# hku-mars/BALM

Hardware: AMD Instinct MI355X
Metric: BA iterations/sec (W poses x F plane features) (higher is better)
Workload: dtype f64

## Files before the change

balm_amd/capi.py:

```python
import ctypes as C
import os

import numpy as np

_HERE = os.path.dirname(os.path.abspath(__file__))
LIB_PATH = os.environ.get("BALM_HIP_LIB") or os.path.join(_HERE, "lib", "libbalm_hip.so")

FORM_LEFT, FORM_RIGHT = 0, 1
OK, ERR_ARG, ERR_HIP, ERR_STATE, ERR_TOO_FEW_PLANES, ERR_NUMERIC = range(6)
ABI_VERSION = 6
FLAG_TIMING = 1
FLAG_LOOPBACK_SHARDS = 2
FLAG_SYRK_INT8 = 4
T_MOMENTS, T_FACTORS, T_SYRK, T_ASSEMBLE, T_SOLVE, T_UPDATE, T_BUILD, T_VOXEL, T_COV, T_COMM, T_UPLOAD, T_COUNT = range(12)
TIMING_NAMES = ["moments", "factors", "syrk", "assemble", "solve", "update", "build", "voxel", "cov", "comm", "upload"]

EXPORTS = ["balm_create", "balm_prewarm", "balm_create_multi", "balm_destroy", "balm_set_features", "balm_set_features_cb", "balm_evaluate", "balm_only_residual",
           "balm_solve_damped", "balm_damping_iter", "balm_build_clusters", "balm_build_clusters_planes", "balm_voxel_defaults", "balm_associate", "balm_associate_scans", "balm_get_features", "balm_get_association", "balm_pose_covariance",
           "balm_window_open", "balm_window_add_scan", "balm_window_add_scan_strided", "balm_window_recut", "balm_window_get_points", "balm_window_features", "balm_window_marginalize", "balm_window_info", "balm_window_close",
           "balm_set_allreduce", "balm_comm_unique_id", "balm_comm_init_rank", "balm_comm_info",
           "balm_get_timing", "balm_get_shard_timing", "balm_get_solve_trace", "balm_chain_macro_plan", "balm_reset_timing", "balm_work_model", "balm_last_error", "balm_version", "balm_abi_version"]


class IterLog(C.Structure):
    _fields_ = [("r1", C.c_double), ("r2", C.c_double), ("u", C.c_double), ("v", C.c_double),
                ("q", C.c_double), ("q1", C.c_double), ("accepted", C.c_int), ("hess_evaluated", C.c_int)]


class LMOpts(C.Structure):
    _fields_ = [("form", C.c_int), ("u0", C.c_double), ("max_iter", C.c_int), ("rel_tol", C.c_double),
                ("min_planes_per_pose", C.c_int), ("force_hess", C.c_int), ("no_stop", C.c_int),
                ("verbose", C.c_int), ("reanchor", C.c_int), ("abs_tol", C.c_double)]


class VoxelOpts(C.Structure):
    _fields_ = [("voxel_size", C.c_double), ("eigen_thr", C.c_float * 3), ("min_ps", C.c_int), ("layer_limit", C.c_int),
                ("min_observers", C.c_int), ("fix_frames", C.c_int), ("max_plane_dist", C.c_double),
                ("max_lambda21", C.c_double), ("max_lambda0", C.c_double), ("want_point_features", C.c_int),
                ("fix_point_limit", C.c_int), ("defer_recut", C.c_int)]


ALLREDUCE_FN = C.CFUNCTYPE(C.c_int, C.c_void_p, C.c_long, C.c_void_p)
FILL_CLUSTERS_FN = C.CFUNCTYPE(None, C.c_void_p, C.c_int, C.c_int, C.POINTER(C.c_double))

_LIB = None


class BalmError(RuntimeError):
    def __init__(self, code, msg):
        super().__init__("balm_hip error %d: %s" % (code, msg))
        self.code = code


def lib():
    global _LIB
    if _LIB is None:
        if not os.path.exists(LIB_PATH):
            raise ImportError("libbalm_hip.so is not built (%s missing): run `python -m balm_amd.build`. "
                              "There is no CPU fallback for the HIP path." % LIB_PATH)
        L = C.CDLL(LIB_PATH)
        abi = getattr(L, "balm_abi_version", None)
        abi = abi() if abi is not None else 0
        if abi != ABI_VERSION:
            raise ImportError("libbalm_hip.so has ABI revision %d, this binding was written for %d: rebuild (python -m balm_amd.build)"
                              % (abi, ABI_VERSION))
        L.balm_create.restype = C.c_void_p
        L.balm_create.argtypes = [C.c_int, C.c_int, C.c_int]
        L.balm_create_multi.restype = C.c_void_p
        L.balm_create_multi.argtypes = [C.c_int, C.c_int, C.c_int, C.c_int]
        L.balm_prewarm.argtypes = [C.c_int]
        L.balm_destroy.restype = None
        L.balm_destroy.argtypes = [C.c_void_p]
        L.balm_set_features.argtypes = [C.c_void_p, C.c_int, C.c_void_p, C.c_void_p, C.c_void_p]
        L.balm_set_features_cb.argtypes = [C.c_void_p, C.c_int, FILL_CLUSTERS_FN, C.c_void_p, C.c_void_p, C.c_void_p]
        L.balm_evaluate.argtypes = [C.c_void_p, C.c_int, C.c_void_p, C.c_int, C.c_int, C.c_void_p, C.c_void_p,
                                    C.POINTER(C.c_double)]
        L.balm_only_residual.argtypes = [C.c_void_p, C.c_void_p, C.POINTER(C.c_double)]
        L.balm_solve_damped.argtypes = [C.c_void_p, C.c_void_p, C.c_void_p, C.c_double, C.c_void_p,
                                        C.POINTER(C.c_double)]
        L.balm_damping_iter.argtypes = [C.c_void_p, C.POINTER(LMOpts), C.c_void_p, C.POINTER(IterLog),
                                        C.POINTER(C.c_int)]
        L.balm_build_clusters.argtypes = [C.c_void_p, C.c_int, C.c_void_p, C.c_void_p, C.c_void_p, C.c_long,
                                          C.c_void_p, C.c_void_p, C.c_void_p]
        L.balm_build_clusters_planes.argtypes = [C.c_void_p, C.c_int, C.c_void_p, C.c_void_p, C.c_size_t, C.c_size_t, C.c_void_p,
                                                 C.c_void_p, C.c_void_p]
        L.balm_associate_scans.argtypes = [C.c_void_p, C.POINTER(VoxelOpts), C.c_int, C.c_void_p, C.c_void_p, C.c_size_t,
                                           C.c_void_p, C.POINTER(C.c_int), C.POINTER(C.c_long)]
        L.balm_window_add_scan_strided.argtypes = [C.c_void_p, C.c_void_p, C.c_long, C.c_size_t, C.c_void_p]
        L.balm_window_open.argtypes = [C.c_void_p, C.POINTER(VoxelOpts)]
        L.balm_window_add_scan.argtypes = [C.c_void_p, C.c_void_p, C.c_long, C.c_void_p]
        L.balm_window_recut.argtypes = [C.c_void_p]
        L.balm_window_get_points.argtypes = [C.c_void_p, C.c_void_p, C.c_void_p, C.c_void_p, C.c_long, C.c_void_p]
        L.balm_window_features.argtypes = [C.c_void_p, C.POINTER(C.c_int)]
        L.balm_window_marginalize.argtypes = [C.c_void_p, C.c_int, C.c_void_p]
        L.balm_window_info.argtypes = [C.c_void_p, C.POINTER(C.c_int), C.POINTER(C.c_long), C.POINTER(C.c_long)]
        L.balm_window_close.argtypes = [C.c_void_p]
        L.balm_associate.argtypes = [C.c_void_p, C.POINTER(VoxelOpts), C.c_void_p, C.c_void_p, C.c_long, C.c_void_p,
                                     C.POINTER(C.c_int), C.POINTER(C.c_long)]
        L.balm_get_features.argtypes = [C.c_void_p, C.c_void_p, C.c_void_p, C.c_void_p]
        L.balm_get_association.argtypes = [C.c_void_p, C.c_void_p, C.c_void_p]
        L.balm_voxel_defaults.restype = None
        L.balm_voxel_defaults.argtypes = [C.POINTER(VoxelOpts)]
        L.balm_pose_covariance.argtypes = [C.c_void_p, C.c_void_p, C.c_void_p, C.c_double, C.c_void_p, C.c_void_p]
        L.balm_set_allreduce.argtypes = [C.c_void_p, ALLREDUCE_FN, C.c_void_p]
        L.balm_comm_unique_id.argtypes = [C.c_void_p]
        L.balm_comm_init_rank.argtypes = [C.c_void_p, C.c_int, C.c_int, C.c_void_p]
        L.balm_comm_info.argtypes = [C.c_void_p, C.c_void_p]
        L.balm_get_timing.argtypes = [C.c_void_p, C.c_void_p, C.c_void_p]
        L.balm_get_shard_timing.argtypes = [C.c_void_p, C.c_int, C.c_void_p, C.c_void_p]
        L.balm_get_solve_trace.argtypes = [C.c_void_p, C.c_void_p, C.c_long, C.c_void_p]
        L.balm_chain_macro_plan.argtypes = [C.c_int, C.c_int, C.c_void_p, C.c_long]
        L.balm_reset_timing.argtypes = [C.c_void_p]
        L.balm_work_model.argtypes = [C.c_void_p, C.c_void_p]
        L.balm_last_error.restype = C.c_char_p
        L.balm_last_error.argtypes = [C.c_void_p]
        L.balm_version.restype = C.c_char_p
        _LIB = L
    return _LIB


def chain_macro_plan(panels, helpers):
    tab = np.empty(helpers * 64, np.int32)
    rc = lib().balm_chain_macro_plan(int(panels), int(helpers), tab.ctypes.data_as(C.c_void_p), tab.size)
    if rc != OK:
        raise BalmError(rc, "balm_chain_macro_plan(%d, %d)" % (panels, helpers))
    tab = tab.reshape(helpers, 64)
    return [[(int(e) & 0xffff, int(e) >> 16) for e in row if e >= 0] for row in tab]


def _p(a):
    return None if a is None else a.ctypes.data_as(C.c_void_p)


def _c(a, dtype=np.float64):
    return None if a is None else np.ascontiguousarray(a, dtype=dtype)


class Context:

    def __init__(self, win_size, device=0, flags=0, n_devices=None):
        self.L = lib()
        self.W = int(win_size)
        self.n = 6 * self.W
        if n_devices is None:
            self.h = self.L.balm_create(self.W, int(device), int(flags))
        else:
            self.h = self.L.balm_create_multi(self.W, int(device), int(n_devices), int(flags))
        if not self.h:
            raise BalmError(ERR_HIP, "balm_create(win_size=%d, device=%d, n_devices=%s) failed (no GPU, bad device, or "
                                     "win_size out of range)" % (win_size, device, n_devices))
        self.F = 0
        self._cb = None

    def close(self):
        if getattr(self, "h", None):
            self.L.balm_destroy(self.h)
            self.h = None

    def __del__(self):
        try:
            self.close()
        except Exception:
            pass

    def _check(self, rc):
        if rc != OK:
            raise BalmError(rc, self.L.balm_last_error(self.h).decode())

    def set_features(self, clusters, fix, coeffs):
        clusters, fix, coeffs = _c(clusters), _c(fix), _c(coeffs)
        F = clusters.shape[0]
        assert clusters.shape == (F, self.W, 10), clusters.shape
        assert coeffs.shape == (F,)
        assert fix is None or fix.shape == (F, 10)
        self._check(self.L.balm_set_features(self.h, F, _p(clusters), _p(fix), _p(coeffs)))
        self.F = F

    def set_features_cb(self, per_feature, fix, coeffs):
        tabs = [_c(t) for t in per_feature]
        F = len(tabs)
        assert all(t.shape == (self.W, 10) for t in tabs)
        fix, coeffs = _c(fix), _c(coeffs)
        row = self.W * 10

        failed = []

        def fill(_user, f0, f1, dst):
            out = np.ctypeslib.as_array(dst, shape=((f1 - f0) * row,))
            try:
                for a in range(f0, f1):
                    out[(a - f0) * row:(a - f0 + 1) * row] = tabs[a].reshape(-1)
            except BaseException as exc:
                out[:] = 0.0
                failed.append(exc)

        cb = FILL_CLUSTERS_FN(fill)
        rc = self.L.balm_set_features_cb(self.h, F, cb, None, _p(fix), _p(coeffs))
        if failed:
            self.F = 0
            raise failed[0]
        self._check(rc)
        self.F = F

    def build_clusters(self, F, xyz, feat_id, pose_id, fix, coeffs, want_clusters=True):
        xyz = _c(xyz, np.float32).reshape(-1, 3)
        feat_id, pose_id = _c(feat_id, np.int32), _c(pose_id, np.int32)
        fix, coeffs = _c(fix), _c(coeffs)
        out = np.zeros((F, self.W, 10)) if want_clusters else None
        self._check(self.L.balm_build_clusters(self.h, F, _p(xyz), _p(feat_id), _p(pose_id), xyz.shape[0],
                                               _p(fix), _p(coeffs), _p(out)))
        self.F = F
        return out

    @staticmethod
    def _containers(arrays):
        keep = [np.ascontiguousarray(a, dtype=np.float32) for a in arrays]
        keep = [a.reshape(-1, 3) if a.ndim == 1 else a for a in keep]
        cols = {a.shape[1] for a in keep}
        assert len(cols) == 1 and min(cols) >= 3, "every container: [n, c] float32 with the same c >= 3"
        ptrs = (C.c_void_p * len(keep))(*[a.ctypes.data if a.shape[0] else None for a in keep])
        cnt = (C.c_long * len(keep))(*[a.shape[0] for a in keep])
        return ptrs, cnt, 4 * cols.pop(), keep

    def build_clusters_planes(self, planes, pose_col, fix, coeffs, want_clusters=True):
        ptrs, cnt, stride, keep = self._containers(planes)
        F = len(keep)
        fix, coeffs = _c(fix), _c(coeffs)
        out = np.zeros((F, self.W, 10)) if want_clusters else None
        self._check(self.L.balm_build_clusters_planes(self.h, F, ptrs, cnt, stride, 4 * int(pose_col), _p(fix), _p(coeffs), _p(out)))
        self.F = F
        return out

    def associate_scans(self, scans, poses, voxel_size=2.0, eigen_thresholds=(1.0 / 16, 1.0 / 16, 1.0 / 9), min_ps=15,
                        want_features=True, layer_limit=2, min_observers=2, fix_frames=0, strict=None, want_points=False):
        ptrs, cnt, stride, keep = self._containers(scans)
        poses = _c(poses)
        assert poses.shape[0] == self.W + fix_frames == len(keep), "one scan and one pose per window slot"
        o = self._voxel_opts(voxel_size, eigen_thresholds, min_ps, layer_limit, min_observers, fix_frames, strict, want_points)
        F, nr = C.c_int(0), C.c_long(0)
        self._check(self.L.balm_associate_scans(self.h, C.byref(o), len(keep), ptrs, cnt, stride, _p(poses), C.byref(F), C.byref(nr)))
        self.F = F.value
        return self.F, nr.value, self._association_result(want_features, fix_frames, want_points, sum(a.shape[0] for a in keep))

    def _voxel_opts(self, voxel_size, eigen_thresholds, min_ps, layer_limit, min_observers, fix_frames, strict, want_points):
        o = VoxelOpts()
        self.L.balm_voxel_defaults(C.byref(o))
        o.voxel_size = voxel_size
        o.eigen_thr = (C.c_float * 3)(*[float(t) for t in eigen_thresholds])
        o.min_ps, o.layer_limit, o.min_observers, o.fix_frames = min_ps, layer_limit, min_observers, fix_frames
        if strict is not None:
            o.max_plane_dist, o.max_lambda21, o.max_lambda0 = strict
        o.want_point_features = int(want_points)
        return o

    def _association_result(self, want_features, fix_frames, want_points, n_pts):
        feats = None
        if want_features and self.F > 0:
            cl, co = np.zeros((self.F, self.W, 10)), np.zeros(self.F)
            layer = np.zeros(self.F, dtype=np.int32)
            self._check(self.L.balm_get_features(self.h, _p(cl), _p(co), _p(layer)))
            feats = (cl, co, layer)
            if fix_frames or want_points:
                fix = np.zeros((self.F, 10))
                pf = np.zeros(n_pts, dtype=np.int32) if want_points else None
                self._check(self.L.balm_get_association(self.h, _p(fix), _p(pf)))
                feats = (cl, co, layer, fix, pf)
        return feats

    def associate(self, xyz, frame_id, poses, voxel_size=2.0, eigen_thresholds=(1.0 / 16, 1.0 / 16, 1.0 / 9),
                  min_ps=15, want_features=True, layer_limit=2, min_observers=2, fix_frames=0, strict=None,
                  want_points=False):
        xyz = _c(xyz, np.float32).reshape(-1, 3)
        frame_id, poses = _c(frame_id, np.int32), _c(poses)
        assert poses.shape[0] == self.W + fix_frames, "poses for the marginalised scans too"
        o = self._voxel_opts(voxel_size, eigen_thresholds, min_ps, layer_limit, min_observers, fix_frames, strict, want_points)
        F, nr = C.c_int(0), C.c_long(0)
        self._check(self.L.balm_associate(self.h, C.byref(o), _p(xyz), _p(frame_id), xyz.shape[0], _p(poses),
                                          C.byref(F), C.byref(nr)))
        self.F = F.value
        return self.F, nr.value, self._association_result(want_features, fix_frames, want_points, xyz.shape[0])

    def window_open(self, voxel_size=2.0, eigen_thresholds=(1.0 / 16, 1.0 / 16, 1.0 / 9), min_ps=15, layer_limit=2,
                    min_observers=2, fix_frames=0, strict=None, fix_point_limit=50, defer_recut=False):
        o = VoxelOpts()
        self.L.balm_voxel_defaults(C.byref(o))
        o.voxel_size = voxel_size
        o.eigen_thr = (C.c_float * 3)(*[float(t) for t in eigen_thresholds])
        o.min_ps, o.layer_limit, o.min_observers = min_ps, layer_limit, min_observers
        o.fix_frames, o.fix_point_limit, o.defer_recut = int(fix_frames), int(fix_point_limit), int(bool(defer_recut))
        if strict is not None:
            o.max_plane_dist, o.max_lambda21, o.max_lambda0 = [float(v) for v in strict]
        self._check(self.L.balm_window_open(self.h, C.byref(o)))

    def window_points(self):
        n = self.window_info()[1]
        xyz, slot, feat = np.zeros((n, 3), np.float32), np.zeros(n, np.int32), np.zeros(n, np.int32)
# ... 154 lines not shown
```

balm_amd/csrc/balm_capi.hip:

```cpp
#include <algorithm>
#include <array>
#include <atomic>
#include <chrono>
#include <cmath>
#include <cstdio>
#include <cstdlib>
#include <cstring>

#include "balm_internal.h"

using namespace balm;

#define HIP_TRY(expr)                                                                              \
  do {                                                                                             \
    hipError_t e_ = (expr);                                                                        \
    if (e_ != hipSuccess) {                                                                        \
      ctx->err = std::string(#expr) + ": " + hipGetErrorString(e_);                                \
      return BALM_ERR_HIP;                                                                         \
    }                                                                                              \
  } while (0)

namespace {

#ifdef BALM_COLD_TRACE
static void cold_mark(const char *what) {
  static const auto t0 = std::chrono::steady_clock::now();
  static double last = 0;
  const double now = std::chrono::duration<double, std::milli>(std::chrono::steady_clock::now() - t0).count();
  fprintf(stderr, "[cold] %9.3f ms (+%8.3f)  %s\n", now, now - last, what);
  last = now;
}
#else
#define cold_mark(what) ((void)0)
#endif

struct DeviceWarm {
  std::mutex mu;
  std::thread th;
  bool started = false;
  PinnedRing ring;
  std::atomic<bool> ring_ready{false};
  ~DeviceWarm() { if (th.joinable()) th.join(); }
};
static DeviceWarm g_warm[64];

static void warm_body(int device) {
  DeviceWarm &w = g_warm[device];
  if (hipSetDevice(device) != hipSuccess) { hipGetLastError(); return; }
  std::thread ring_th([&w, device] {
    if (hipSetDevice(device) == hipSuccess && w.ring.init(device) == hipSuccess) w.ring_ready.store(true, std::memory_order_release);
    else hipGetLastError();
  });
  (void)preload_voxel(); (void)preload_build(); (void)prepare_device_accum(); (void)preload_solve(); (void)prepare_device_cov();
  hipGetLastError();
  ring_th.join();
}

static int warm_start(int device) {
  if (device < 0 || device >= 64) return BALM_ERR_ARG;
  DeviceWarm &w = g_warm[device];
  std::lock_guard<std::mutex> lk(w.mu);
  if (!w.started) { w.started = true; w.th = std::thread(warm_body, device); }
  return BALM_OK;
}

static void adopt_warm_ring(balm_ctx *ctx) {
  if (ctx->ring.buf[0] || ctx->device < 0 || ctx->device >= 64) return;
  DeviceWarm &w = g_warm[ctx->device];
  std::lock_guard<std::mutex> lk(w.mu);
  if (!w.started) return;
  if (w.th.joinable()) w.th.join();
  if (w.ring_ready.load(std::memory_order_acquire)) {
    const int key = ctx->ring.pool_key;
    ctx->ring = w.ring; ctx->ring.pool_key = key;
    w.ring = PinnedRing(); w.ring_ready.store(false);
  }
}

struct Span {
  balm_ctx *c; int slot; hipEvent_t a = nullptr, b = nullptr;
  Span(balm_ctx *ctx, int s) : c(ctx), slot(s) {
    if (!c->timer.on) return;
    a = take(); b = take();
    hipEventRecord(a, c->stream);
  }
  ~Span() {
    if (!c->timer.on) return;
    hipEventRecord(b, c->stream);
    c->timer.pending.push_back({a, b, slot});
  }
  hipEvent_t take() {
    if (!c->timer.pool.empty()) { hipEvent_t e = c->timer.pool.back(); c->timer.pool.pop_back(); return e; }
    hipEvent_t e; hipEventCreate(&e); return e;
  }
};

void collect_timing(balm_ctx *c) {
  for (auto &sp : c->timer.pending) {
    float ms = 0;
    if (hipEventElapsedTime(&ms, sp.a, sp.b) == hipSuccess) { c->timer.ms[sp.slot] += ms; c->timer.cnt[sp.slot]++; }
    c->timer.pool.push_back(sp.a); c->timer.pool.push_back(sp.b);
  }
  c->timer.pending.clear();
}

template <class T>
int dalloc(balm_ctx *ctx, T **p, size_t count) {
  if (*p) { hipFree(*p); *p = nullptr; }
  if (count == 0) count = 1;
  HIP_TRY(hipMalloc((void **)p, count * sizeof(T)));
  return BALM_OK;
}

template <class T>
int keep(balm_ctx *ctx, T **p, size_t *cap, size_t count) {
  if (*p && *cap >= count) return BALM_OK;
  for (int k = 0; k < balm_ctx::LM_GRAPHS; k++)
    if (ctx->lm_graph[k]) { hipGraphExecDestroy(ctx->lm_graph[k]); ctx->lm_graph[k] = nullptr; ctx->lm_graph_form[k] = -1; }
  int rc = dalloc(ctx, p, count + count / 4);
  *cap = rc ? 0 : count + count / 4;
  return rc;
}

template <class T>
int ensure(balm_ctx *ctx, T **p, size_t *cap, size_t count) {
  if (*p && *cap >= count) return BALM_OK;
  for (int k = 0; k < balm_ctx::LM_GRAPHS; k++)
    if (ctx->lm_graph[k]) { hipGraphExecDestroy(ctx->lm_graph[k]); ctx->lm_graph[k] = nullptr; ctx->lm_graph_form[k] = -1; }
  int rc = dalloc(ctx, p, count);
  if (rc) return rc;
  *cap = count;
  return BALM_OK;
}

int stage_begin(balm_ctx *ctx, size_t total_bytes) {
  total_bytes += 16 * 256;
  ctx->stage_off = 0;
  if (ctx->stage_cap >= total_bytes) return BALM_OK;
  if (ctx->d_stage) { hipStreamSynchronize(ctx->stream); hipFree(ctx->d_stage); ctx->d_stage = nullptr; ctx->stage_cap = 0; }
  const size_t want = total_bytes + total_bytes / 8;
  HIP_TRY(hipMalloc((void **)&ctx->d_stage, want));
  ctx->stage_cap = want;
  return BALM_OK;
}

template <class T>
T *stage_take(balm_ctx *ctx, size_t count) {
  const size_t off = (ctx->stage_off + 255) & ~(size_t)255;
  ctx->stage_off = off + count * sizeof(T);
  return reinterpret_cast<T *>(ctx->d_stage + off);
}

int sync_stream(balm_ctx *ctx) {
  HIP_TRY(hipStreamSynchronize(ctx->stream));
  HIP_TRY(hipGetLastError());
  collect_timing(ctx);
  return BALM_OK;
}

long red_dacc_off(const balm_ctx *c) { return (long)c->ntiles * TILE_ELEMS; }
long red_r_off(const balm_ctx *c) { return red_dacc_off(c) + (long)DACC_MAX * c->W; }

bool has_transport(const balm_ctx *ctx) { return ctx->comm || multi_is_loopback(ctx) || ctx->allreduce; }

int hook_allreduce(balm_ctx *ctx, double *buf, long n) {
  if (ctx->comm) { Span sp(ctx, BALM_T_COMM); return comm_allreduce(ctx, buf, n); }
  if (multi_is_loopback(ctx)) { Span sp(ctx, BALM_T_COMM); return loopback_allreduce(ctx, buf, n); }
  if (!ctx->allreduce) return BALM_OK;
  int rc = sync_stream(ctx);
  if (rc) return rc;
  if (ctx->allreduce((void *)buf, n, ctx->allreduce_user) != 0) {
    ctx->err = "all-reduce hook failed";
    return BALM_ERR_STATE;
  }
  return BALM_OK;
}

int set_damping(balm_ctx *ctx, double u) {
  ctx->u_value = u;
  ctx->u_on_device = false;
  return BALM_OK;
}
int push_damping(balm_ctx *ctx) {
  double *slot = ctx->h_scal + 16 + (ctx->u_ring++ & 63);
  *slot = ctx->u_value;
  HIP_TRY(hipMemcpyAsync(ctx->d_scal + SCAL_U, slot, sizeof(double), hipMemcpyHostToDevice, ctx->stream));
  ctx->u_on_device = true;
  return BALM_OK;
}

static void collect_timing_if_idle(balm_ctx *ctx) {
  if (!ctx->timer.on || ctx->timer.pending.empty()) return;
  if (hipStreamSynchronize(ctx->stream) == hipSuccess) collect_timing(ctx);
}

int wait_scalars(balm_ctx *ctx) {
  volatile double *stamp = ctx->h_scal + SCAL_STAMP;
  const double want = (double)ctx->mail_seq;
  const auto t0 = std::chrono::steady_clock::now();
  for (int spin = 0;; spin++) {
    if (*stamp == want) { std::atomic_thread_fence(std::memory_order_acquire); collect_timing_if_idle(ctx); return BALM_OK; }
    if ((spin & 255) == 255 && std::chrono::steady_clock::now() - t0 > std::chrono::microseconds(300)) break;
  }
  int rc = sync_stream(ctx);
  if (rc) return rc;
  if (*stamp != want) { ctx->err = "balm_damping_iter: the iteration's scalars did not arrive"; return BALM_ERR_HIP; }
  return BALM_OK;
}

void drop_lm_graphs(balm_ctx *ctx) {
  for (int k = 0; k < balm_ctx::LM_GRAPHS; k++) {
    if (ctx->lm_graph[k]) hipGraphExecDestroy(ctx->lm_graph[k]);
    ctx->lm_graph[k] = nullptr; ctx->lm_graph_form[k] = -1;
  }
}

int residual_device(balm_ctx *ctx, const double *d_poses, int f0, int f1, int slot, bool defer_sum = false, bool send_mail = false) {
  if (f1 <= f0) {
    HIP_TRY(hipMemsetAsync(ctx->d_scal + slot, 0, sizeof(double), ctx->stream));
    ctx->nr_tmp = 0;
  } else {
    Span sp(ctx, BALM_T_MOMENTS);
    launch_world_moments(ctx->stream, ctx->d_cl, d_poses, ctx->W, f0, f1, ctx->d_C);
    const EigenMail mail{ctx->d_scal, ctx->d_hscal, send_mail ? (double)++ctx->mail_seq : 0.0, slot};
    ctx->nr_tmp = launch_feature_eigen(ctx->stream, ctx->d_C, ctx->has_fix ? ctx->d_fix : nullptr, ctx->d_coe, f0, f1, ctx->d_feat_tmp,
                                       ctx->d_rpart_tmp, send_mail ? &mail : nullptr);
    if (!defer_sum) launch_sum_scalar(ctx->stream, ctx->d_rpart_tmp, ctx->nr_tmp, ctx->d_scal + slot);
  }
  HIP_TRY(hipGetLastError());
  if (defer_sum) return BALM_OK;
  return hook_allreduce(ctx, ctx->d_scal + slot, 1);
}

bool fuse_trial(const balm_ctx *ctx) {
  const char *e = getenv("BALM_FUSE_TRIAL");
  return ctx->W <= 256 && ctx->F > 0 && e && e[0] == '1';
}

static bool syrk_int8_mode(const balm_ctx *ctx) {
  if (ctx->flags & BALM_FLAG_SYRK_INT8) return true;
  const char *m = getenv("BALM_SYRK");
  return m && !strcmp(m, "int8");
}
static bool syrk_int8_for(const balm_ctx *ctx, long K) {
  if (!syrk_int8_mode(ctx)) return false;
  if (const char *m = getenv("BALM_SYRK_INT8_MIN_COLS")) return K >= atol(m);
  return K >= 12288L && ctx->W >= 96;
}

int prepare_evaluate(balm_ctx *ctx, int form, int nf) {
  if (nf <= 0) return BALM_OK;
  const SyrkPlan plan = plan_syrk(ctx->ntiles, 3L * nf);
  int rc;
  size_t gcols = (size_t)plan.Kpad + 64, parts = (size_t)plan.SG * ctx->ntiles;
  if (ctx->sparse && nf == ctx->F) {
    gcols = (size_t)ctx->sp_nchunks * ctx->sp_nsteps * 4 + 64;
    parts = (size_t)ctx->sp_nitems;
  }
  {
    const double *before = ctx->d_Gt;
    if ((rc = ensure(ctx, &ctx->d_Gt, &ctx->cap_Gt, gcols * ctx->npad))) return rc;
    if (ctx->d_Gt != before) ctx->gt_dirty_cols = ~(size_t)0;
  }
  if ((rc = ensure(ctx, &ctx->d_part, &ctx->cap_part, parts * TILE_ELEMS))) return rc;
  if (syrk_int8_for(ctx, 3L * nf) && !(ctx->sparse && nf == ctx->F)) {
    if ((rc = ensure(ctx, &ctx->d_i8, &ctx->cap_i8, syrk_i8_scratch_bytes(ctx->n, 3L * nf, nullptr)))) return rc;
    if (!ctx->d_rowmax) ctx->rowmax_cur_valid = false;
    if (!ctx->d_rowmax2) ctx->rowmax_trial_valid = false;
    if ((rc = ensure(ctx, &ctx->d_rowmax, &ctx->cap_rowmax, (size_t)ctx->npad + 128))) return rc;
    if ((rc = ensure(ctx, &ctx->d_rowmax2, &ctx->cap_rowmax2, (size_t)ctx->npad + 128))) return rc;
    if ((rc = ensure(ctx, &ctx->d_rowmax_part, &ctx->cap_rowmax_part, (size_t)factors_grid(ctx->W, nf, form) * 6 * ctx->W))) return rc;
    HIP_TRY(prepare_device_syrk_i8());
  }
  if ((rc = ensure(ctx, &ctx->d_dpart, &ctx->cap_dpart, (size_t)factors_grid(ctx->W, nf, form) * DACC_MAX * ctx->W))) return rc;
  if (nf == ctx->F && fuse_trial(ctx)) {
    if (ctx->cap_Gt2 < gcols * ctx->npad || ctx->cap_dpart2 < (size_t)factors_grid(ctx->W, nf, form) * DACC_MAX * ctx->W) ctx->gt_trial_valid = false;
    if ((rc = ensure(ctx, &ctx->d_Gt2, &ctx->cap_Gt2, gcols * ctx->npad))) return rc;
    if ((rc = ensure(ctx, &ctx->d_dpart2, &ctx->cap_dpart2, (size_t)factors_grid(ctx->W, nf, form) * DACC_MAX * ctx->W))) return rc;
  }
  return BALM_OK;
}

int evaluate_device(balm_ctx *ctx, int form, const double *d_poses, int f0, int f1, int slot) {
  const int W = ctx->W, nf = f1 - f0;
  const int dacc = form == 0 ? DACC_LEFT : DACC_RIGHT;
  int rc;
  if (nf <= 0) {
    HIP_TRY(hipMemsetAsync(ctx->d_red, 0, ctx->red_len * sizeof(double), ctx->stream));
    if ((rc = hook_allreduce(ctx, ctx->d_red, (long)ctx->red_len))) return rc;
    Span sp(ctx, BALM_T_ASSEMBLE);
    launch_assemble(ctx->stream, form, ctx->d_red, red_dacc_off(ctx), ctx->d_sub, ctx->ntiles, W, ctx->d_H, ctx->d_g,
                    ctx->d_red + red_r_off(ctx), ctx->d_scal + slot);
    return BALM_OK;
  }
  SyrkPlan plan = plan_syrk(ctx->ntiles, 3L * nf);
  if ((rc = prepare_evaluate(ctx, form, nf))) return rc;
  const int nblk = factors_grid(W, nf, form);
  hipStream_t s = ctx->stream;
  if (!(ctx->feat_cur_valid && f0 == 0 && f1 == ctx->F)) {
    Span sp(ctx, BALM_T_MOMENTS);
    launch_world_moments(s, ctx->d_cl, d_poses, W, f0, f1, ctx->d_C);
    ctx->nr_cur = launch_feature_eigen(s, ctx->d_C, ctx->has_fix ? ctx->d_fix : nullptr, ctx->d_coe, f0, f1, ctx->d_feat, ctx->d_rpart);
    ctx->feat_cur_valid = (f0 == 0 && f1 == ctx->F);
  }
  const int nr = ctx->nr_cur;
  const bool sparse = ctx->sparse && f0 == 0 && f1 == ctx->F;
  const size_t kpad = sparse ? (size_t)ctx->sp_nchunks * ctx->sp_nsteps * 4 : (size_t)plan.Kpad;
  if (!(ctx->gt_cur_valid && ctx->feat_cur_valid && f0 == 0 && f1 == ctx->F)) {
    Span sp(ctx, BALM_T_FACTORS);
    const size_t k0 = (size_t)3 * nf, k1 = kpad + 64;
    if (ctx->gt_dirty_cols == ~(size_t)0) {
      HIP_TRY(hipMemsetAsync(ctx->d_Gt, 0, ctx->cap_Gt * sizeof(double), s));
      ctx->gt_dirty_cols = 0;
    } else if (ctx->gt_dirty_cols > k0) {
      HIP_TRY(hipMemsetAsync(ctx->d_Gt + k0 * ctx->npad, 0, (std::max(ctx->gt_dirty_cols, k1) - k0) * ctx->npad * sizeof(double), s));
    }
    ctx->gt_dirty_cols = k0;
    ctx->rowmax_cur_valid = launch_factors(s, form, ctx->d_cl, d_poses, ctx->d_feat, W, ctx->npad, f0, f1, ctx->d_Gt, ctx->d_dpart, nblk,
                                           sparse ? ctx->d_slot : nullptr, (!sparse && syrk_int8_for(ctx, 3L * nf)) ? ctx->d_rowmax : nullptr, ctx->d_rowmax_part);
    ctx->gt_cur_valid = false;
  }
  HIP_TRY(hipGetLastError());
  const bool int8 = !sparse && syrk_int8_for(ctx, 3L * nf);
  {
    Span sp(ctx, BALM_T_SYRK);
    if (sparse) launch_syrk_sparse(s, ctx->d_Gt, ctx->npad, ctx->d_jobs, ctx->d_items, ctx->d_chunk_ids, ctx->sp_nsteps, ctx->sp_nitems, ctx->d_part);
    else if (int8) {
      if (launch_syrk_i8(s, ctx->d_Gt, ctx->npad, ctx->n, 3L * nf, ctx->d_sub, ctx->ntiles, ctx->d_i8, ctx->d_part,
                         ctx->rowmax_cur_valid ? ctx->d_rowmax : nullptr)) { ctx->err = "INT8 SYRK: unsupported size"; return BALM_ERR_ARG; }
      plan.SG = 1;
    }
    else launch_syrk(s, ctx->d_Gt, ctx->npad, ctx->ntiles, ctx->d_jobs, plan, ctx->d_part);
  }
  {
    Span sp(ctx, BALM_T_ASSEMBLE);
    launch_reduce(s, ctx->d_part, plan.SG, (long)ctx->ntiles * TILE_ELEMS, ctx->d_dpart, nblk, dacc * W,
                  ctx->d_rpart, nr, ctx->d_red, red_dacc_off(ctx), red_r_off(ctx), sparse ? ctx->d_csr : nullptr);
  }
  if ((rc = hook_allreduce(ctx, ctx->d_red, (long)ctx->red_len))) return rc;
  {
    Span sp(ctx, BALM_T_ASSEMBLE);
    launch_assemble(s, form, ctx->d_red, red_dacc_off(ctx), ctx->d_sub, ctx->ntiles, W, ctx->d_H, ctx->d_g, ctx->d_red + red_r_off(ctx),
                    ctx->d_scal + slot);
  }
  return BALM_OK;
}

int trial_device(balm_ctx *ctx, int form, const double *d_poses, int slot) {
  const int W = ctx->W, F = ctx->F;
  hipStream_t s = ctx->stream;
  const SyrkPlan plan = plan_syrk(ctx->ntiles, 3L * F);
  const bool sparse = ctx->sparse;
  const size_t kpad = sparse ? (size_t)ctx->sp_nchunks * ctx->sp_nsteps * 4 : (size_t)plan.Kpad;
  const int nblk = factors_grid(W, F, form);
  {
    Span sp(ctx, BALM_T_FACTORS);
    const size_t k0 = (size_t)3 * F, k1 = kpad + 64;
    HIP_TRY(hipMemsetAsync(ctx->d_Gt2 + k0 * ctx->npad, 0, (k1 - k0) * ctx->npad * sizeof(double), s));
    if (ctx->npad > ctx->n)
      HIP_TRY(hipMemset2DAsync(ctx->d_Gt2 + ctx->n, (size_t)ctx->npad * sizeof(double), 0,
                               (size_t)(ctx->npad - ctx->n) * sizeof(double), k0, s));
    ctx->nr_tmp = launch_moments_factors(s, form, ctx->d_cl, d_poses, ctx->has_fix ? ctx->d_fix : nullptr, ctx->d_coe, W, ctx->npad, F,
                                         ctx->d_Gt2, ctx->d_dpart2, nblk, sparse ? ctx->d_slot : nullptr, ctx->d_feat_tmp, ctx->d_rpart_tmp,
                                         (!sparse && syrk_int8_for(ctx, 3L * F) && ctx->d_rowmax2) ? ctx->d_rowmax2 : nullptr, ctx->d_rowmax_part);
    ctx->rowmax_trial_valid = !sparse && syrk_int8_for(ctx, 3L * F) && ctx->d_rowmax2;
  }
  HIP_TRY(hipGetLastError());
  {
    Span sp(ctx, BALM_T_MOMENTS);
    launch_sum_scalar(s, ctx->d_rpart_tmp, ctx->nr_tmp, ctx->d_scal + slot);
  }
  ctx->gt_trial_valid = true;
  return hook_allreduce(ctx, ctx->d_scal + slot, 1);
}

int read_scalars(balm_ctx *ctx) {
  HIP_TRY(hipMemcpyAsync(ctx->h_scal, ctx->d_scal, 16 * sizeof(double), hipMemcpyDeviceToHost, ctx->stream));
  return sync_stream(ctx);
}

std::vector<unsigned char> obs_of(const double *clusters, int F, int W) {
  std::vector<unsigned char> obs((size_t)F * W);
  parallel_ranges(obs.size(), (size_t)1 << 16, [&](size_t lo, size_t hi) {
    for (size_t t = lo; t < hi; t++) obs[t] = clusters[t * 10 + 9] != 0 ? 1 : 0;
  });
  return obs;
}

int feature_bookkeeping(balm_ctx *ctx, int F, const unsigned char *obs, const double *fix, const double *coeffs) {
  const int W = ctx->W;
  ctx->planes_per_pose.assign(W, 0);
  double S = 0, B = 0;
  int bad_a = F, bad_rc = BALM_OK;
  std::mutex mu;
  parallel_ranges((size_t)F, (size_t)(65536 / W + 1), [&](size_t lo, size_t hi) {
    std::vector<int> ppp((size_t)W, 0);
    double s = 0, b = 0;
    int my_bad = F, my_rc = BALM_OK;
    for (size_t a = lo; a < hi; a++) {
      int na = 0;
      const unsigned char *oa = obs + a * W;
      for (int i = 0; i < W; i++)
        if (oa[i]) { ppp[(size_t)i]++; na++; }
      if (my_rc == BALM_OK) {
        if (na == 0 && !(fix && fix[a * 10 + 9] != 0)) { my_bad = (int)a; my_rc = BALM_ERR_NUMERIC; }
        else if (!(coeffs[a] >= 0) || !std::isfinite(coeffs[a])) { my_bad = (int)a; my_rc = BALM_ERR_ARG; }
      }
      s += na; b += 0.5 * na * (na + 1.0);
    }
    std::lock_guard<std::mutex> lk(mu);
    for (int i = 0; i < W; i++) ctx->planes_per_pose[(size_t)i] += ppp[(size_t)i];
    S += s; B += b;
    if (my_rc != BALM_OK && my_bad < bad_a) { bad_a = my_bad; bad_rc = my_rc; }
  });
  if (bad_rc == BALM_ERR_NUMERIC) {
    ctx->err = "feature " + std::to_string(bad_a) + " has no observation and no fix cluster (zero point count)";
    return BALM_ERR_NUMERIC;
  }
  if (bad_rc == BALM_ERR_ARG) {
    ctx->err = "feature " + std::to_string(bad_a) + " has a negative or non-finite weight";
    return BALM_ERR_ARG;
  }
  ctx->work_S = S; ctx->work_B = B;
  return BALM_OK;
}

}

extern "C" {

const char *balm_version(void) { return "balm_hip 0.6.0 (gfx950)"; }
int balm_abi_version(void) { return BALM_ABI_VERSION; }

const char *balm_last_error(balm_ctx *ctx) { return ctx ? ctx->err.c_str() : "null context"; }

static void one_destroy(balm_ctx *ctx);

balm_ctx *balm_create(int win_size, int device, int flags) {
  if (win_size < 1 || win_size > MAX_W) return nullptr;
  cold_mark("balm_create: enter");
  int ndev = 0;
  if (hipGetDeviceCount(&ndev) != hipSuccess || ndev < 1 || device < 0 || device >= ndev) return nullptr;
  if (hipSetDevice(device) != hipSuccess) return nullptr;
  cold_mark("balm_create: hipGetDeviceCount + hipSetDevice");
  warm_start(device);
  if (prepare_device_accum() != hipSuccess || prepare_device_cov() != hipSuccess) return nullptr;
  cold_mark("balm_create: prepare_device (function attributes -> code objects)");
  balm_ctx *ctx = new balm_ctx();
  ctx->W = win_size;
  ctx->n = 6 * win_size;
  ctx->npad = (ctx->n + TILE - 1) / TILE * TILE;
  ctx->T = ctx->npad / TILE;
  ctx->nA = (ctx->n + NB - 1) / NB * NB;
  ctx->device = device;
  ctx->flags = flags;
  ctx->timer.on = (flags & BALM_FLAG_TIMING) != 0;
  auto fail = [&]() -> balm_ctx * { one_destroy(ctx); return nullptr; };
  std::vector<int> jobs, sub;
  {
    const int T = ctx->T, ngroups = T / 5;
    std::vector<std::array<int, 3>> mixed[4];
    std::vector<std::array<int, 2>> pairs;
    for (int r = 0; r < TM; r++) for (int c = r; c < TM; c++) pairs.push_back({r, c});
    for (int k = 0; k < 15; k++) mixed[1].push_back({0, pairs[k][0], pairs[k][1]});
    for (int k = 0; k < 10; k++) mixed[1].push_back({1, pairs[k][0], pairs[k][1]});
    for (int k = 10; k < 15; k++) mixed[2].push_back({1, pairs[k][0], pairs[k][1]});
    for (int k = 0; k < 15; k++) mixed[2].push_back({2, pairs[k][0], pairs[k][1]});
    for (int k = 0; k < 5; k++) mixed[2].push_back({3, pairs[k][0], pairs[k][1]});
    for (int k = 5; k < 15; k++) mixed[3].push_back({3, pairs[k][0], pairs[k][1]});
    for (int k = 0; k < 15; k++) mixed[3].push_back({4, pairs[k][0], pairs[k][1]});
    auto regular = [&](int I, int J) {
      jobs.insert(jobs.end(), {0, I, J, 0});
      for (int t = 0; t < 25; t++) sub.push_back(((TM * I + t / TM) << 16) | (TM * J + t % TM));
    };
    for (int m = 0; m < T; m++) {
      for (int i = 0; i < m; i++) regular(i, m);
      if (m >= TM * ngroups) regular(m, m);
      else if (m % TM == TM - 1) {
        const int b = m - (TM - 1);
        for (int v = 1; v <= 3; v++) {
          jobs.insert(jobs.end(), {v, b, b, 0});
          for (const auto &e : mixed[v]) sub.push_back(((TM * (b + e[0]) + e[1]) << 16) | (TM * (b + e[0]) + e[2]));
        }
      }
    }
  }
  ctx->ntiles = (int)(jobs.size() / 4);
  ctx->h_jobs = jobs;
  if (hipStreamCreateWithFlags(&ctx->stream, hipStreamNonBlocking) != hipSuccess) return fail();
  cold_mark("balm_create: job tables + stream");
  const int W = ctx->W, n = ctx->n, nA = ctx->nA;
  ctx->red_len = (size_t)ctx->ntiles * TILE_ELEMS + (size_t)DACC_MAX * W + 2;
  if (dalloc(ctx, &ctx->d_poses, (size_t)12 * W) || dalloc(ctx, &ctx->d_poses_tmp, (size_t)12 * W) ||
      dalloc(ctx, &ctx->d_red, ctx->red_len) || dalloc(ctx, &ctx->d_jobs, jobs.size()) || dalloc(ctx, &ctx->d_sub, sub.size()) ||
      dalloc(ctx, &ctx->d_H, (size_t)n * n) || dalloc(ctx, &ctx->d_g, (size_t)n) ||
      dalloc(ctx, &ctx->d_A, (size_t)(2 * nA + NB) * nA) || dalloc(ctx, &ctx->d_Wp, (size_t)2 * NB * (2 * nA + NB)) ||
      dalloc(ctx, &ctx->d_dvec, (size_t)nA) || dalloc(ctx, &ctx->d_z, (size_t)nA) || dalloc(ctx, &ctx->d_x, (size_t)16 * nA) ||
      dalloc(ctx, &ctx->d_perm, (size_t)nA) || dalloc(ctx, &ctx->d_flags, (size_t)2 * (2 * (nA / NB) + 1) * (nA / NB) + (nA / NB) + 8) || dalloc(ctx, &ctx->d_minv, (size_t)2 * (nA / NB) * NB * NB) || dalloc(ctx, &ctx->d_dx, (size_t)n) ||
      dalloc(ctx, &ctx->d_scal, (size_t)16) || dalloc(ctx, &ctx->d_pre, (size_t)W + 2))
    return fail();
  if (hipHostMalloc((void **)&ctx->h_scal, (16 + 64 + 8) * sizeof(double), hipHostMallocMapped | hipHostMallocCoherent) != hipSuccess) return fail();
  if (hipHostGetDevicePointer((void **)&ctx->d_hscal, ctx->h_scal, 0) != hipSuccess) return fail();
  ctx->h_scal[SCAL_STAMP] = 0.0;
  if (hipMemcpy(ctx->d_jobs, jobs.data(), jobs.size() * sizeof(int), hipMemcpyHostToDevice) != hipSuccess ||
      hipMemcpy(ctx->d_sub, sub.data(), sub.size() * sizeof(int), hipMemcpyHostToDevice) != hipSuccess)
    return fail();
  if (getenv("BALM_SOLVE_TRACE")) {
    const size_t cnt = (size_t)(2 * (nA / NB) + 1) * (nA / NB) * 6 + (size_t)(nA / NB) * 6;
    if (hipMalloc((void **)&ctx->d_trace, cnt * sizeof(long long)) != hipSuccess) return fail();
    hipMemset(ctx->d_trace, 0, cnt * sizeof(long long));
  }
  {
    std::vector<int> ident(nA);
    for (int i = 0; i < nA; i++) ident[i] = i;
    if (hipMemcpy(ctx->d_perm, ident.data(), (size_t)nA * sizeof(int), hipMemcpyHostToDevice) != hipSuccess) return fail();
  }
  if (hipMemset(ctx->d_scal, 0, 16 * sizeof(double)) != hipSuccess) return fail();
  if (hipMemset(ctx->d_red, 0, ctx->red_len * sizeof(double)) != hipSuccess) return fail();
  if (hipMemset(ctx->d_minv, 0, (size_t)2 * (nA / NB) * NB * NB * sizeof(double)) != hipSuccess) return fail();
  cold_mark("balm_create: device buffers + small copies");
  context_born(device); ctx->counted_live = true;
  return ctx;
}

static void one_destroy(balm_ctx *ctx) {
  if (!ctx) return;
  if (ctx->counted_live) { context_gone(ctx->device); ctx->counted_live = false; }
  comm_destroy(ctx);
  drop_lm_graphs(ctx);
  hipSetDevice(ctx->device);
  if (ctx->stream) hipStreamSynchronize(ctx->stream);
  if (ctx->window) { window_close(ctx->window); ctx->window = nullptr; }
  void *ptrs[] = {ctx->d_cl, ctx->d_fix, ctx->d_coe, ctx->d_poses, ctx->d_poses_tmp, ctx->d_C, ctx->d_feat,
                  ctx->d_Gt, ctx->d_Gt2, ctx->d_dpart2, ctx->d_part, ctx->d_dpart, ctx->d_rpart, ctx->d_feat_tmp, ctx->d_rpart_tmp, ctx->d_red, ctx->d_jobs, ctx->d_sub, ctx->d_H,
                  ctx->d_g, ctx->d_A, ctx->d_Wp, ctx->d_dvec, ctx->d_z, ctx->d_x, ctx->d_perm, ctx->d_dx, ctx->d_scal, ctx->d_arena, ctx->d_pre, ctx->d_flags, ctx->d_minv, ctx->d_macro_tab, ctx->d_trace, ctx->d_slot, ctx->d_items, ctx->d_csr, ctx->d_chunk_ids, ctx->d_stage, ctx->d_i8, ctx->d_rowmax, ctx->d_rowmax2, ctx->d_rowmax_part};
  for (void *p : ptrs) if (p) hipFree(p);
  if (ctx->h_scal) hipHostFree(ctx->h_scal);
  ctx->ring.release();
  if (ctx->amail.host) hipHostFree((void *)ctx->amail.host);
  if (ctx->amail.scan_state) hipFree(ctx->amail.scan_state);
  for (auto &sp : ctx->timer.pending) { hipEventDestroy(sp.a); hipEventDestroy(sp.b); }
  for (auto e : ctx->timer.pool) hipEventDestroy(e);
  if (ctx->stream) hipStreamDestroy(ctx->stream);
  delete ctx;
}

static int build_sparse_plan(balm_ctx *ctx, int F, const unsigned char *obs) {
  ctx->sparse = false;
  const char *mode = getenv("BALM_SYRK");
  if (mode && !strcmp(mode, "dense")) return BALM_OK;
  if (syrk_int8_for(ctx, 3L * F)) return BALM_OK;
  const int W = ctx->W, T = ctx->T, ntiles = ctx->ntiles;
  if (T > 128 || T <= 2 || F < 64) return BALM_OK;
  struct Key { uint64_t hi, lo; int a; };
  std::vector<Key> keys((size_t)F);
  parallel_ranges((size_t)F, (size_t)(65536 / W + 1), [&](size_t a0, size_t a1) {
    for (size_t a = a0; a < a1; a++) {
      uint64_t hi = 0, lo = 0;
      const unsigned char *oa = obs + a * W;
      for (int i = 0; i < W; i++)
        if (oa[i])
          for (int b = (6 * i) / TILE; b <= (6 * i + 5) / TILE; b++) {
            if (b < 64) hi |= 1ull << (63 - b); else lo |= 1ull << (127 - b);
          }
      keys[a] = {hi, lo, (int)a};
    }
  });
  auto first_of = [&](const Key &k) { for (int b = 0; b < T; b++) if (b < 64 ? (k.hi >> (63 - b)) & 1 : (k.lo >> (127 - b)) & 1) return b; return T; };
  auto last_of = [&](const Key &k) { for (int b = T - 1; b >= 0; b--) if (b < 64 ? (k.hi >> (63 - b)) & 1 : (k.lo >> (127 - b)) & 1) return b; return -1; };
  std::vector<int> fb((size_t)F), lb((size_t)F);
  for (int a = 0; a < F; a++) { fb[(size_t)a] = first_of(keys[(size_t)a]); lb[(size_t)a] = last_of(keys[(size_t)a]); }
  std::sort(keys.begin(), keys.end(), [&](const Key &x, const Key &y) {
    if (fb[(size_t)x.a] != fb[(size_t)y.a]) return fb[(size_t)x.a] < fb[(size_t)y.a];
    if (lb[(size_t)x.a] != lb[(size_t)y.a]) return lb[(size_t)x.a] < lb[(size_t)y.a];
    return x.hi != y.hi ? x.hi > y.hi : (x.lo != y.lo ? x.lo > y.lo : x.a < y.a);
  });
  const int C = 16, nsteps = 3 * C / 4, nchunks = (F + C - 1) / C;
  auto touched = [](const Key &k, int b) { return b < 64 ? (k.hi >> (63 - b)) & 1 : (k.lo >> (127 - b)) & 1; };
  std::vector<int> slot((size_t)F);
  std::vector<std::vector<int>> chunks_of((size_t)ntiles);
  long total = 0;
  for (int c = 0; c < nchunks; c++) {
    Key cm{0, 0, 0};
    for (int k = c * C; k < F && k < (c + 1) * C; k++) { cm.hi |= keys[(size_t)k].hi; cm.lo |= keys[(size_t)k].lo; slot[(size_t)keys[(size_t)k].a] = k; }
    for (int j = 0; j < ntiles; j++) {
      const int type = ctx->h_jobs[(size_t)4 * j], I = ctx->h_jobs[(size_t)4 * j + 1], J = ctx->h_jobs[(size_t)4 * j + 2];
      bool need;
      if (type == 0) need = touched(cm, I) && touched(cm, J);
      else if (type == 1) need = touched(cm, I) || touched(cm, I + 1);
      else if (type == 2) need = touched(cm, I + 1) || touched(cm, I + 2) || touched(cm, I + 3);
      else need = touched(cm, I + 3) || touched(cm, I + 4);
      if (need) { chunks_of[(size_t)j].push_back(c); total++; }
    }
  }
  const double dense_steps = (double)ntiles * ((3.0 * F + 3) / 4), sparse_steps = (double)total * nsteps;
  const bool forced = mode && !strcmp(mode, "sparse");
  if (total == 0 || (!forced && !(sparse_steps < 0.8 * dense_steps))) return BALM_OK;
  long per = total / 2048;
  if (per < 8) per = 8;
  std::vector<int> items, chunk_ids, csr((size_t)ntiles + 1, 0);
  struct Order { int first_chunk, item; };
  std::vector<Order> order;
  int run = 0;
  for (int j = 0; j < ntiles; j++) {
    csr[(size_t)j] = run;
    const std::vector<int> &L = chunks_of[(size_t)j];
    const long pieces = ((long)L.size() + per - 1) / per;
    for (long q = 0; q < pieces; q++) {
      const size_t b = (size_t)((long)L.size() * q / pieces), e = (size_t)((long)L.size() * (q + 1) / pieces);
      order.push_back({L[b], (int)(items.size() / 4)});
      items.insert(items.end(), {j, (int)chunk_ids.size(), (int)(e - b), run++});
      chunk_ids.insert(chunk_ids.end(), L.begin() + (long)b, L.begin() + (long)e);
    }
  }
  csr[(size_t)ntiles] = run;
  std::stable_sort(order.begin(), order.end(), [](const Order &x, const Order &y) { return x.first_chunk < y.first_chunk; });
  std::vector<int> sorted_items;
  sorted_items.reserve(items.size());
  for (const Order &o : order) sorted_items.insert(sorted_items.end(), items.begin() + 4L * o.item, items.begin() + 4L * o.item + 4);
  if (chunk_ids.empty()) chunk_ids.push_back(0);
  int rc;
  if ((rc = keep(ctx, &ctx->d_slot, &ctx->cap_slot, (size_t)F)) || (rc = keep(ctx, &ctx->d_items, &ctx->cap_items, sorted_items.size())) ||
      (rc = keep(ctx, &ctx->d_chunk_ids, &ctx->cap_chunk_ids, chunk_ids.size())) || (rc = keep(ctx, &ctx->d_csr, &ctx->cap_csr, csr.size())))
    return rc;
  HIP_TRY(hipMemcpy(ctx->d_slot, slot.data(), slot.size() * sizeof(int), hipMemcpyHostToDevice));
  HIP_TRY(hipMemcpy(ctx->d_items, sorted_items.data(), sorted_items.size() * sizeof(int), hipMemcpyHostToDevice));
  HIP_TRY(hipMemcpy(ctx->d_chunk_ids, chunk_ids.data(), chunk_ids.size() * sizeof(int), hipMemcpyHostToDevice));
  HIP_TRY(hipMemcpy(ctx->d_csr, csr.data(), csr.size() * sizeof(int), hipMemcpyHostToDevice));
  ctx->sparse = true; ctx->sp_nsteps = nsteps; ctx->sp_nchunks = nchunks; ctx->sp_nitems = run; ctx->sp_steps = sparse_steps;
  return BALM_OK;
}

static int install_feature_buffers(balm_ctx *ctx, int F, const double *fix, const double *coeffs,
                                   hipMemcpyKind kind = hipMemcpyHostToDevice) {
  int rc;
  drop_lm_graphs(ctx);
  ctx->has_fix = fix != nullptr;
  if (fix) {
    if ((rc = keep(ctx, &ctx->d_fix, &ctx->cap_fix, (size_t)F * 10))) return rc;
    HIP_TRY(hipMemcpyAsync(ctx->d_fix, fix, (size_t)F * 10 * sizeof(double), kind, ctx->stream));
  }
  if ((rc = keep(ctx, &ctx->d_coe, &ctx->cap_coe, (size_t)F))) return rc;
  HIP_TRY(hipMemcpyAsync(ctx->d_coe, coeffs, (size_t)F * sizeof(double), kind, ctx->stream));
  if ((rc = keep(ctx, &ctx->d_C, &ctx->cap_C, (size_t)F * 10))) return rc;
  if ((rc = keep(ctx, &ctx->d_feat, &ctx->cap_feat, (size_t)F * FEAT_STRIDE))) return rc;
  if ((rc = keep(ctx, &ctx->d_feat_tmp, &ctx->cap_feat_tmp, (size_t)F * FEAT_STRIDE))) return rc;
  if ((rc = keep(ctx, &ctx->d_rpart, &ctx->cap_rpart, (size_t)(F + 255) / 256 + 1024 + 1))) return rc;
  if ((rc = keep(ctx, &ctx->d_rpart_tmp, &ctx->cap_rpart_tmp, (size_t)(F + 255) / 256 + 1024 + 1))) return rc;
  ctx->feat_cur_valid = false; ctx->gt_cur_valid = false;
  ctx->F = F;
  return BALM_OK;
}

static int assoc_clusters_host(balm_ctx *ctx);

using FillClusters = std::function<void(int, int, double *, unsigned char *)>;

static int one_set_features_fn(balm_ctx *ctx, int F, const FillClusters &fill, const double *fix, const double *coeffs, bool shard_books = false) {
  if (!ctx) return BALM_ERR_ARG;
  if (ctx->multi && F == 0) { ctx->F = 0; ctx->feat_cur_valid = false; ctx->gt_cur_valid = false; ctx->planes_per_pose.clear(); ctx->work_S = ctx->work_B = 0; return BALM_OK; }
  if (F < 1 || !fill || !coeffs) { ctx->err = "balm_set_features: bad argument"; return BALM_ERR_ARG; }
  HIP_TRY(hipSetDevice(ctx->device));
  const int W = ctx->W;
  const size_t count = (size_t)F * W * 10;
  int rc;
  if ((rc = assoc_clusters_host(ctx))) return rc;
  ctx->F = 0;
  adopt_warm_ring(ctx);
  if ((rc = keep(ctx, &ctx->d_cl, &ctx->cap_cl, count))) return rc;
  if ((rc = stage_begin(ctx, count * sizeof(double)))) return rc;
  double *d_aos = stage_take<double>(ctx, count);
  std::vector<unsigned char> obs((size_t)F * W);
  const size_t unit = (size_t)W * 10 * sizeof(double);
  hipError_t e;
  {
    Span sp(ctx, BALM_T_UPLOAD);
    e = staged_upload(ctx->ring, ctx->device, ctx->stream, d_aos, count * sizeof(double), unit, [&](char *dst, size_t off, size_t len) {
      const int f0 = (int)(off / unit), f1 = f0 + (int)(len / unit);
      fill(f0, f1, reinterpret_cast<double *>(dst), obs.data() + (size_t)f0 * W);
    });
  }
  if (e == hipSuccess) launch_transpose_clusters(ctx->stream, d_aos, ctx->d_cl, F, W);
  HIP_TRY(e);
  if ((!ctx->multi || shard_books) && (rc = feature_bookkeeping(ctx, F, obs.data(), fix, coeffs))) { hipStreamSynchronize(ctx->stream); return rc; }
  if ((rc = build_sparse_plan(ctx, F, obs.data()))) { hipStreamSynchronize(ctx->stream); return rc; }
  if ((rc = install_feature_buffers(ctx, F, fix, coeffs))) { hipStreamSynchronize(ctx->stream); return rc; }
  return sync_stream(ctx);
}

static int one_set_features(balm_ctx *ctx, int F, const double *clusters, const double *fix, const double *coeffs) {
  if (ctx && !(ctx->multi && F == 0) && !clusters) { ctx->err = "balm_set_features: bad argument"; return BALM_ERR_ARG; }
  const size_t row = ctx ? (size_t)ctx->W * 10 : 0;
  return one_set_features_fn(ctx, F, [clusters, row](int f0, int f1, double *dst, unsigned char *o) {
    const double *src = clusters + (size_t)f0 * row;
// ... 416 lines not shown
  const int nblk = cov_factors_grid(W, F > 0 ? F : 1);
  if ((rc = ensure(ctx, &ctx->d_dpart, &ctx->cap_dpart, (size_t)nblk * DACC_MAX * W))) return rc;
  const bool int8 = F > 0 && syrk_int8_for(ctx, 3L * F);
  if (int8) {
    if ((rc = ensure(ctx, &ctx->d_i8, &ctx->cap_i8, syrk_i8_scratch_bytes(ctx->n, 3L * F, nullptr)))) return rc;
    HIP_TRY(prepare_device_syrk_i8());
  }
  const size_t pay = 2 * tiles + (size_t)21 * W, nn = (size_t)n * n;
  const size_t ncc = (cluster_cov && F > 0) ? (size_t)F * W * 81 : 0;
  if ((rc = stage_begin(ctx, (pay + 2 * nn + 2 * (size_t)nA * nA + ncc) * sizeof(double)))) return rc;
  double *buf = stage_take<double>(ctx, pay + 2 * nn + 2 * (size_t)nA * nA), *d_cc = nullptr;
  double *redx = buf, *redy = buf + tiles, *sdiag = buf + 2 * tiles, *Rraw = buf + pay, *Rc = Rraw + nn,
         *T0 = Rc + nn, *T1 = T0 + (size_t)nA * nA;
  hipError_t e = hipSuccess;
  if (ncc) {
    d_cc = stage_take<double>(ctx, ncc);
    adopt_warm_ring(ctx);
    if (e == hipSuccess) { Span sp(ctx, BALM_T_UPLOAD); e = staged_copy(ctx->ring, ctx->device, s, d_cc, cluster_cov, (size_t)F * W * 81 * sizeof(double)); }
  }
  double *Gx = ctx->d_Gt, *Gy = ctx->d_Gt + gcols * ctx->npad;
  if (e == hipSuccess && F == 0) e = hipMemsetAsync(buf, 0, pay * sizeof(double), s);
  if (e == hipSuccess && F > 0) {
    Span sp(ctx, BALM_T_COV);
    const size_t k0 = (size_t)3 * F;
    hipMemsetAsync(Gx + k0 * ctx->npad, 0, (gcols - k0) * ctx->npad * sizeof(double), s);
    hipMemsetAsync(Gy + k0 * ctx->npad, 0, (gcols - k0) * ctx->npad * sizeof(double), s);
    launch_cov_factors(s, ctx->d_cl, d_cc, point_sigma * point_sigma, ctx->d_poses, ctx->d_feat, W, ctx->npad, F, Gx, Gy,
                       ctx->d_dpart, nblk);
    e = hipGetLastError();
    if (int8) {
      if (launch_syrk_i8(s, Gx, ctx->npad, ctx->n, 3L * F, ctx->d_sub, ctx->ntiles, ctx->d_i8, ctx->d_part)) e = hipErrorInvalidValue;
      launch_cov_reduce_tiles(s, ctx->d_part, 1, (long)tiles, redx);
      if (launch_syrk_i8(s, Gy, ctx->npad, ctx->n, 3L * F, ctx->d_sub, ctx->ntiles, ctx->d_i8, ctx->d_part)) e = hipErrorInvalidValue;
      launch_cov_reduce_tiles(s, ctx->d_part, 1, (long)tiles, redy);
    } else {
      launch_syrk(s, Gx, ctx->npad, ctx->ntiles, ctx->d_jobs, plan, ctx->d_part);
      launch_cov_reduce_tiles(s, ctx->d_part, plan.SG, (long)tiles, redx);
      launch_syrk(s, Gy, ctx->npad, ctx->ntiles, ctx->d_jobs, plan, ctx->d_part);
      launch_cov_reduce_tiles(s, ctx->d_part, plan.SG, (long)tiles, redy);
    }
    launch_cov_reduce_dacc(s, ctx->d_dpart, nblk, W, sdiag);
  }
  if (e == hipSuccess) rc = hook_allreduce(ctx, buf, (long)pay);
  if (e == hipSuccess && !rc) {
    Span sp(ctx, BALM_T_COV);
    launch_cov_assemble(s, redx, redy, sdiag, ctx->d_sub, ctx->ntiles, W, Rraw);
    hipMemsetAsync(ctx->d_g, 0, (size_t)n * sizeof(double), s);
    set_damping(ctx, 0.0);
    ctx->need_minv = true;
    launch_solve(ctx, true);
    ctx->need_minv = false;
    launch_congruence_inverse(ctx, Rraw, T0, T1, Rc);
    if (Rcov) e = hipMemcpyAsync(Rcov, Rc, nn * sizeof(double), hipMemcpyDeviceToHost, s);
    if (e == hipSuccess && Rcov_raw) e = hipMemcpyAsync(Rcov_raw, Rraw, nn * sizeof(double), hipMemcpyDeviceToHost, s);
  }
  if (e == hipSuccess) e = hipStreamSynchronize(s);
  if (e == hipSuccess) e = hipGetLastError();
  if (rc) return rc;
  HIP_TRY(e);
  collect_timing(ctx);
  return BALM_OK;
}

int balm_comm_info(balm_ctx *ctx, long *out4) {
  if (!ctx || !out4) return BALM_ERR_ARG;
  out4[0] = 1; out4[1] = 0; out4[2] = (long)ctx->red_len; out4[3] = 0;
  if (ctx->comm) {
    int cnt = -1, rk = -1;
    comm_query(ctx, &cnt, &rk);
    out4[0] = cnt; out4[1] = rk; out4[3] = 1;
  } else if (multi_is_loopback(ctx)) {
    out4[0] = ctx->multi->n; out4[1] = ctx->rank; out4[3] = 2;
  } else if (ctx->allreduce) {
    out4[0] = -1; out4[3] = 3;
  }
  return BALM_OK;
}

int balm_set_allreduce(balm_ctx *ctx, balm_allreduce_fn fn, void *user) {
  if (!ctx) return BALM_ERR_ARG;
  if (fn && (ctx->multi || ctx->comm)) { ctx->err = "balm_set_allreduce: the context already has a collective transport"; return BALM_ERR_STATE; }
  ctx->allreduce = fn;
  ctx->allreduce_user = user;
  return BALM_OK;
}

static int one_evaluate(balm_ctx *ctx, int form, const double *poses, int head, int end, double *Hess, double *JacT,
                  double *residual) {
  if (!ctx) return BALM_ERR_ARG;
  if (!ctx->multi) {
    if (ctx->F < 1) { ctx->err = "balm_evaluate: no features installed"; return BALM_ERR_STATE; }
    if ((form != 0 && form != 1) || !poses || head < 0 || end > ctx->F || head >= end) {
      ctx->err = "balm_evaluate: bad argument"; return BALM_ERR_ARG;
    }
  }
  HIP_TRY(hipSetDevice(ctx->device));
  const int n = ctx->n;
  HIP_TRY(hipMemcpyAsync(ctx->d_poses, poses, (size_t)12 * ctx->W * sizeof(double), hipMemcpyHostToDevice, ctx->stream));
  ctx->feat_cur_valid = false; ctx->gt_cur_valid = false;
  int rc = evaluate_device(ctx, form, ctx->d_poses, head, end, 0);
  ctx->feat_cur_valid = false; ctx->gt_cur_valid = false;
  if (rc) return rc;
  if (Hess) HIP_TRY(hipMemcpyAsync(Hess, ctx->d_H, (size_t)n * n * sizeof(double), hipMemcpyDeviceToHost, ctx->stream));
  if (JacT) HIP_TRY(hipMemcpyAsync(JacT, ctx->d_g, (size_t)n * sizeof(double), hipMemcpyDeviceToHost, ctx->stream));
  if ((rc = read_scalars(ctx))) return rc;
  if (residual) *residual = ctx->h_scal[0];
  if (!std::isfinite(ctx->h_scal[0])) { ctx->err = "balm_evaluate: non-finite residual"; return BALM_ERR_NUMERIC; }
  return BALM_OK;
}

static int one_only_residual(balm_ctx *ctx, const double *poses, double *residual) {
  if (!ctx) return BALM_ERR_ARG;
  if (!ctx->multi && ctx->F < 1) { ctx->err = "balm_only_residual: no features installed"; return BALM_ERR_STATE; }
  if (!poses || !residual) { ctx->err = "balm_only_residual: bad argument"; return BALM_ERR_ARG; }
  HIP_TRY(hipSetDevice(ctx->device));
  HIP_TRY(hipMemcpyAsync(ctx->d_poses_tmp, poses, (size_t)12 * ctx->W * sizeof(double), hipMemcpyHostToDevice, ctx->stream));
  int rc = residual_device(ctx, ctx->d_poses_tmp, 0, ctx->F, 1);
  if (rc) return rc;
  if ((rc = read_scalars(ctx))) return rc;
  *residual = ctx->h_scal[1];
  if (!std::isfinite(ctx->h_scal[1])) { ctx->err = "balm_only_residual: non-finite residual"; return BALM_ERR_NUMERIC; }
  return BALM_OK;
}

int balm_solve_damped(balm_ctx *ctx, const double *Hess, const double *JacT, double u, double *dxi, double *q1) {
  if (!ctx) return BALM_ERR_ARG;
  if (!Hess || !JacT || !dxi) { ctx->err = "balm_solve_damped: bad argument"; return BALM_ERR_ARG; }
  HIP_TRY(hipSetDevice(ctx->device));
  const int n = ctx->n;
  HIP_TRY(hipMemcpyAsync(ctx->d_H, Hess, (size_t)n * n * sizeof(double), hipMemcpyHostToDevice, ctx->stream));
  HIP_TRY(hipMemcpyAsync(ctx->d_g, JacT, (size_t)n * sizeof(double), hipMemcpyHostToDevice, ctx->stream));
  {
    Span sp(ctx, BALM_T_SOLVE);
    int rcu = set_damping(ctx, u);
    if (rcu) return rcu;
    launch_solve(ctx, true);
  }
  HIP_TRY(hipMemcpyAsync(dxi, ctx->d_dx, (size_t)n * sizeof(double), hipMemcpyDeviceToHost, ctx->stream));
  int rc = read_scalars(ctx);
  if (rc) return rc;
  if (!std::isfinite(ctx->h_scal[2]) && !ctx->persistent_off && solve_timed_out(ctx)) {
    ctx->persistent_off = true;
    {
      Span sp(ctx, BALM_T_SOLVE);
      launch_solve(ctx, true);
    }
    HIP_TRY(hipMemcpyAsync(dxi, ctx->d_dx, (size_t)n * sizeof(double), hipMemcpyDeviceToHost, ctx->stream));
    if ((rc = read_scalars(ctx))) return rc;
  }
  if (q1) *q1 = ctx->h_scal[2];
  return BALM_OK;
}

static int lm_enqueue(balm_ctx *ctx, int form, bool evaluated, bool mail) {
  int rc;
  if (evaluated && (rc = evaluate_device(ctx, form, ctx->d_poses, 0, ctx->F, 0))) return rc;
  {
    Span sp(ctx, BALM_T_SOLVE);
    launch_solve(ctx, evaluated, form, ctx->d_poses, ctx->d_poses_tmp);
  }
  ctx->gt_trial_valid = false;
  bool sum_in_mail = false;
  if (fuse_trial(ctx) && ctx->d_Gt2 && ctx->d_dpart2) {
    if ((rc = trial_device(ctx, form, ctx->d_poses_tmp, 1))) return rc;
  } else {
    sum_in_mail = mail && !has_transport(ctx) && ctx->F > 0;
    const bool eigen_mails = sum_in_mail && ctx->F <= 256;
    if ((rc = residual_device(ctx, ctx->d_poses_tmp, 0, ctx->F, 1, sum_in_mail, eigen_mails))) return rc;
    if (eigen_mails) return BALM_OK;
  }
  if (mail) launch_scalars_mail(ctx->stream, ctx->d_scal, ctx->d_hscal, (double)++ctx->mail_seq, sum_in_mail ? ctx->d_rpart_tmp : nullptr,
                                ctx->nr_tmp, 1);
  else HIP_TRY(hipMemcpyAsync(ctx->h_scal, ctx->d_scal, 16 * sizeof(double), hipMemcpyDeviceToHost, ctx->stream));
  return BALM_OK;
}

static int lm_iteration(balm_ctx *ctx, int form, bool evaluated, int it) {
  const char *genv = getenv("BALM_GRAPH");
  const bool disabled = !(genv && (!strcmp(genv, "1") || !strcmp(genv, "debug")));
  const bool graphable = !disabled && ctx->graphs_ok && it >= 1 && !ctx->timer.on && !has_transport(ctx) && !ctx->multi &&
                         ctx->feat_cur_valid && ctx->F > 0 && !solve_is_persistent(ctx);
  if (graphable) {
    const bool fused = fuse_trial(ctx) && ctx->d_Gt2 && ctx->d_dpart2;
    const int slot = (ctx->gt_parity ? 16 : 0) | (fused ? 8 : 0) | (ctx->gt_cur_valid ? 4 : 0) | (evaluated ? 2 : 0) | ctx->parity;
    if (ctx->lm_graph[slot] && ctx->lm_graph_form[slot] != form) {
      hipGraphExecDestroy(ctx->lm_graph[slot]); ctx->lm_graph[slot] = nullptr;
    }
    if (!ctx->lm_graph[slot]) {
      hipGraph_t g = nullptr;
      ctx->u_on_device = true;
      bool ok = hipStreamBeginCapture(ctx->stream, hipStreamCaptureModeThreadLocal) == hipSuccess;
      if (ok) {
        const int rc = lm_enqueue(ctx, form, evaluated, false);
        const hipError_t e = hipStreamEndCapture(ctx->stream, &g);
        ok = rc == BALM_OK && e == hipSuccess && g != nullptr;
      }
      if (ok) ok = hipGraphInstantiate(&ctx->lm_graph[slot], g, nullptr, nullptr, 0) == hipSuccess;
      if (g) hipGraphDestroy(g);
      if (genv && !strcmp(genv, "debug")) fprintf(stderr, "balm_hip: LM graph slot %d capture %s\n", slot, ok ? "ok" : "FAILED");
      if (!ok) {
        hipGetLastError();
        ctx->lm_graph[slot] = nullptr;
        ctx->graphs_ok = false;
      } else {
        ctx->lm_graph_form[slot] = form;
      }
    }
    if (ctx->lm_graph[slot]) {
      int rcu = push_damping(ctx);
      if (rcu) return rcu;
      HIP_TRY(hipGraphLaunch(ctx->lm_graph[slot], ctx->stream));
      return sync_stream(ctx);
    }
    ctx->u_on_device = false;
  }
  int rc = lm_enqueue(ctx, form, evaluated, true);
  if (rc) return rc;
  return wait_scalars(ctx);
}

static int one_damping_iter(balm_ctx *ctx, const balm_lm_opts *o, double *poses, balm_iter_log *log, int *n_iters) {
  if (!ctx) return BALM_ERR_ARG;
  if (!ctx->multi && ctx->F < 1) { ctx->err = "balm_damping_iter: no features installed"; return BALM_ERR_STATE; }
  if (!o || !poses || (o->form != 0 && o->form != 1) || o->max_iter < 1) {
    ctx->err = "balm_damping_iter: bad argument"; return BALM_ERR_ARG;
  }
  if (n_iters) *n_iters = 0;
  HIP_TRY(hipSetDevice(ctx->device));
  const int W = ctx->W, F = ctx->F;
  hipStream_t s = ctx->stream;
  cold_mark("damping_iter: enter");
  int rc = prepare_evaluate(ctx, o->form, F);
  cold_mark("damping_iter: prepare_evaluate (scratch allocations)");
  std::vector<double> pre((size_t)W + 2, 0.0);
  for (size_t i = 0; i < ctx->planes_per_pose.size() && i < (size_t)W; i++) pre[i] = ctx->planes_per_pose[i];
  pre[(size_t)W] = rc ? 1.0 : 0.0;
  if (has_transport(ctx)) {
    int rc2;
    if (hipMemcpyAsync(ctx->d_pre, pre.data(), pre.size() * sizeof(double), hipMemcpyHostToDevice, s) != hipSuccess) return BALM_ERR_HIP;
    if ((rc2 = hook_allreduce(ctx, ctx->d_pre, (long)pre.size()))) return rc2;
    if (hipMemcpyAsync(pre.data(), ctx->d_pre, pre.size() * sizeof(double), hipMemcpyDeviceToHost, s) != hipSuccess) return BALM_ERR_HIP;
    if ((rc2 = sync_stream(ctx))) return rc2;
    if (pre[(size_t)W] != 0.0 && !rc) { ctx->err = "balm_damping_iter: another rank failed before the loop"; rc = BALM_ERR_STATE; }
  }
  if (rc) return rc;
  if (o->min_planes_per_pose > 0) {
    double mn = pre[0];
    for (int i = 1; i < W; i++) mn = pre[(size_t)i] < mn ? pre[(size_t)i] : mn;
    if (mn < o->min_planes_per_pose) {
      ctx->err = "Initial error too large. Please loose plane determination criteria for more planes. "
                 "The optimization is terminated.";
      return BALM_ERR_TOO_FEW_PLANES;
    }
  }
  HIP_TRY(hipMemcpyAsync(ctx->d_poses, poses, (size_t)12 * W * sizeof(double), hipMemcpyHostToDevice, s));
  ctx->feat_cur_valid = false; ctx->gt_cur_valid = false;
  double u = o->u0, v = 2, r1 = 0, r2 = 0;
  bool calc = true;
  int it = 0;
  int fault_rank = -1, fault_it = -1, timeout_it = -1;
  if (const char *fi = getenv("BALM_FAULT_INJECT")) {
    if (!strncmp(fi, "timeout,", 8)) timeout_it = atoi(fi + 8);
    else if (ctx->multi) sscanf(fi, "%d,%d", &fault_rank, &fault_it);
  }
  while (it < o->max_iter) {
    const bool evaluated = calc || o->force_hess;
    if (ctx->rank == fault_rank && it == fault_it) { ctx->err = "balm_damping_iter: injected fault"; return BALM_ERR_HIP; }
    if (it == timeout_it) { ctx->inject_solve_timeout = true; timeout_it = -1; }
    if ((rc = set_damping(ctx, u))) return rc;
    if ((rc = lm_iteration(ctx, o->form, evaluated, it))) return rc;
    double sc[3] = {ctx->h_scal[0], ctx->h_scal[1], ctx->h_scal[2]};
    if ((rc = multi_share_scalars(ctx, it, sc, 3))) return rc;
    r1 = sc[0]; r2 = sc[1];
    const double q1 = sc[2];
    double q = r1 - r2;
    if (!ctx->multi && !ctx->persistent_off && !(std::isfinite(r2) && std::isfinite(q1)) && std::isfinite(r1) && solve_timed_out(ctx)) {
      ctx->persistent_off = true;
      drop_lm_graphs(ctx);
      ctx->feat_cur_valid = false; ctx->gt_cur_valid = false;
      calc = true;
      continue;
    }
    if (!(std::isfinite(r1) && std::isfinite(r2))) {
      ctx->err = "balm_damping_iter: non-finite residual";
      return BALM_ERR_NUMERIC;
    }
    if (log) { log[it].r1 = r1; log[it].r2 = r2; log[it].u = u; log[it].v = v; log[it].q = q; log[it].q1 = q1;
               log[it].accepted = q > 0; log[it].hess_evaluated = evaluated; }
    if (o->verbose)
    {
      printf("iter%d: (%lf %lf) u: %lf v: %.1lf q: %.3lf %lf %lf\n", it, r1, r2, u, v, q / q1, q1, q);
      fflush(stdout);
    }
    if (q > 0) {
      double *t = ctx->d_poses; ctx->d_poses = ctx->d_poses_tmp; ctx->d_poses_tmp = t;
      t = ctx->d_feat; ctx->d_feat = ctx->d_feat_tmp; ctx->d_feat_tmp = t;
      t = ctx->d_rpart; ctx->d_rpart = ctx->d_rpart_tmp; ctx->d_rpart_tmp = t;
      ctx->nr_cur = ctx->nr_tmp;
      ctx->feat_cur_valid = true;
      ctx->gt_cur_valid = ctx->gt_trial_valid;
      if (ctx->gt_trial_valid) {
        std::swap(ctx->d_Gt, ctx->d_Gt2); std::swap(ctx->cap_Gt, ctx->cap_Gt2);
        std::swap(ctx->d_rowmax, ctx->d_rowmax2); std::swap(ctx->cap_rowmax, ctx->cap_rowmax2);
        ctx->rowmax_cur_valid = ctx->rowmax_trial_valid;
        ctx->gt_dirty_cols = ~(size_t)0;
        std::swap(ctx->d_dpart, ctx->d_dpart2); std::swap(ctx->cap_dpart, ctx->cap_dpart2);
        ctx->gt_parity ^= 1;
      }
      ctx->parity ^= 1;
      q = q / q1; v = 2; q = 1 - std::pow(2 * q - 1, 3);
      u *= (q < 1.0 / 3.0 ? 1.0 / 3.0 : q);
      calc = true;
    } else {
      u = u * v; v = 2 * v; calc = false;
    }
    it++;
    if (!o->no_stop && std::fabs(r1 - r2) / r1 < o->rel_tol) break;
    if (!o->no_stop && o->abs_tol > 0 && std::fabs(r1 - r2) < o->abs_tol) break;
  }
  ctx->feat_cur_valid = false; ctx->gt_cur_valid = false;
  if (o->reanchor) launch_reanchor(s, W, ctx->d_poses);
  HIP_TRY(hipMemcpyAsync(poses, ctx->d_poses, (size_t)12 * W * sizeof(double), hipMemcpyDeviceToHost, s));
  if ((rc = sync_stream(ctx))) return rc;
  if (n_iters) *n_iters = it;
  cold_mark("damping_iter: done");
  return BALM_OK;
}

static balm_multi *leader_of(balm_ctx *ctx) { return (ctx && ctx->multi && ctx->rank == 0) ? ctx->multi : nullptr; }

int balm_prewarm(int device) {
  int ndev = 0;
  if (hipGetDeviceCount(&ndev) != hipSuccess || device < 0 || device >= ndev) { hipGetLastError(); return BALM_ERR_ARG; }
  return warm_start(device);
}

balm_ctx *balm_create_multi(int win_size, int first_device, int n_devices, int flags) {
  if (n_devices < 1 || n_devices > MAX_SHARDS) return nullptr;
  const bool loopback = (flags & BALM_FLAG_LOOPBACK_SHARDS) != 0;
  HostPool::shard_pool_threads() = n_devices > 4 ? 8 : 0;
  std::vector<balm_ctx *> subs;
  for (int k = 0; k < n_devices; k++) {
    balm_ctx *c = balm_create(win_size, loopback ? first_device : first_device + k, flags);
    if (!c) { for (auto *q : subs) one_destroy(q); return nullptr; }
    c->ring.pool_key = k;
    subs.push_back(c);
  }
  std::string err;
  balm_multi *m = multi_new(subs, loopback, &err);
  if (!m) {
    fprintf(stderr, "balm_create_multi: %s\n", err.c_str());
    for (auto *q : subs) one_destroy(q);
    return nullptr;
  }
  return subs[0];
}

void balm_destroy(balm_ctx *ctx) {
  if (!ctx) return;
  if (balm_multi *m = ctx->multi) {
    std::vector<balm_ctx *> subs = m->sub;
    for (auto *q : subs) { hipSetDevice(q->device); if (q->stream) hipStreamSynchronize(q->stream); }
    multi_delete(m);
    for (auto *q : subs) { q->multi = nullptr; one_destroy(q); }
    return;
  }
  one_destroy(ctx);
}

int balm_comm_unique_id(void *id128) {
  if (!id128) return BALM_ERR_ARG;
  return comm_unique_id(id128);
}

int balm_comm_init_rank(balm_ctx *ctx, int n_ranks, int rank, const void *id128) {
  if (!ctx) return BALM_ERR_ARG;
  if (!id128 || n_ranks < 1 || rank < 0 || rank >= n_ranks) { ctx->err = "balm_comm_init_rank: bad argument"; return BALM_ERR_ARG; }
  if (ctx->multi || ctx->comm) { ctx->err = "balm_comm_init_rank: the context already has a collective transport"; return BALM_ERR_STATE; }
  HIP_TRY(hipSetDevice(ctx->device));
  return comm_init_rank(ctx, n_ranks, rank, id128);
}

static int multi_set_features(balm_ctx *ctx, balm_multi *m, int F, const double *clusters, const double *fix, const double *coeffs) {
  if (F < 1 || !clusters || !coeffs) { ctx->err = "balm_set_features: bad argument"; return BALM_ERR_ARG; }
  m->F = 0;
  m->books_per_shard = false;
  for (size_t k = 1; k < m->sub.size(); k++) { m->sub[k]->planes_per_pose.clear(); m->sub[k]->work_S = m->sub[k]->work_B = 0; }
  const std::vector<unsigned char> obs = obs_of(clusters, F, ctx->W);
  int rc = feature_bookkeeping(ctx, F, obs.data(), fix, coeffs);
  if (rc) return rc;
  {
    const int W = ctx->W;
    std::vector<double> cum((size_t)F + 1, 0.0);
    parallel_ranges((size_t)F, (size_t)(65536 / W + 1), [&](size_t lo, size_t hi) {
      for (size_t a = lo; a < hi; a++) {
        int na = 0;
        const unsigned char *oa = obs.data() + a * W;
        for (int i = 0; i < W; i++) na += oa[i];
        cum[a + 1] = 0.5 * na * (na + 1.0) + 4.0 * na + 1.0;
      }
    });
    for (int a = 0; a < F; a++) cum[(size_t)a + 1] += cum[(size_t)a];
    m->fbeg[0] = 0;
    for (int k = 1; k < m->n; k++) {
      const double target = cum[(size_t)F] * k / m->n;
      int f = (int)(std::lower_bound(cum.begin(), cum.end(), target) - cum.begin());
      if (f < m->fbeg[(size_t)k - 1]) f = m->fbeg[(size_t)k - 1];
      if (f > F) f = F;
      m->fbeg[(size_t)k] = f;
    }
    m->fbeg[(size_t)m->n] = F;
  }
  const size_t W = (size_t)ctx->W;
  rc = multi_run(m, [&](int k) {
    const int f0 = m->fbeg[(size_t)k], nf = m->fbeg[(size_t)k + 1] - f0;
    return one_set_features(m->sub[(size_t)k], nf, clusters + (size_t)f0 * W * 10, fix ? fix + (size_t)f0 * 10 : nullptr, coeffs + f0);
  });
  if (rc) { if (ctx->err.empty()) ctx->err = "balm_set_features: a device failed"; return rc; }
  m->F = F;
  return BALM_OK;
}

int balm_set_features(balm_ctx *ctx, int F, const double *clusters, const double *fix, const double *coeffs) {
  if (balm_multi *m = leader_of(ctx)) return multi_set_features(ctx, m, F, clusters, fix, coeffs);
  return one_set_features(ctx, F, clusters, fix, coeffs);
}

static void multi_cut(balm_multi *m, int F, const std::vector<double> &cum ) {
  m->fbeg[0] = 0;
  for (int k = 1; k < m->n; k++) {
    const double target = cum[(size_t)F] * k / m->n;
    int f = (int)(std::lower_bound(cum.begin(), cum.end(), target) - cum.begin());
    if (f < m->fbeg[(size_t)k - 1]) f = m->fbeg[(size_t)k - 1];
    if (f > F) f = F;
    m->fbeg[(size_t)k] = f;
  }
  m->fbeg[(size_t)m->n] = F;
}

static int multi_done(balm_ctx *ctx, balm_multi *m, int F, int rc, const char *who) {
  if (rc) { if (ctx->err.empty()) ctx->err = std::string(who) + ": a device failed"; for (auto *q : m->sub) if (!q->err.empty()) { ctx->err = q->err; break; } return rc; }
  m->F = F;
  m->books_per_shard = true;
  return BALM_OK;
}

int balm_set_features_cb(balm_ctx *ctx, int F, balm_fill_clusters_fn fill, void *user, const double *fix, const double *coeffs) {
  if (!ctx) return BALM_ERR_ARG;
  if (F < 1 || !fill || !coeffs) { ctx->err = "balm_set_features_cb: bad argument"; return BALM_ERR_ARG; }
  if (balm_multi *m = leader_of(ctx)) {
    const size_t Wc = (size_t)ctx->W, row = Wc * 10;
    m->F = 0;
    std::vector<double> cum((size_t)F + 1, 0.0);
    parallel_ranges((size_t)F, (size_t)(32768 / row + 1), [&](size_t lo, size_t hi) {
      const size_t blk = std::max<size_t>(1, (size_t)65536 / (row * sizeof(double)));
      std::vector<double> scratch(blk * row);
      for (size_t a0 = lo; a0 < hi; a0 += blk) {
        const size_t a1 = std::min(hi, a0 + blk);
        fill(user, (int)a0, (int)a1, scratch.data());
        for (size_t a = a0; a < a1; a++) {
          int na = 0;
          const double *r = scratch.data() + (a - a0) * row;
          for (size_t i = 0; i < Wc; i++) na += r[i * 10 + 9] != 0 ? 1 : 0;
          cum[a + 1] = 0.5 * na * (na + 1.0) + 4.0 * na + 1.0;
        }
      }
    });
    for (int a = 0; a < F; a++) cum[(size_t)a + 1] += cum[(size_t)a];
    multi_cut(m, F, cum);
    int rc = multi_run(m, [&](int k) {
      const int f0 = m->fbeg[(size_t)k], nf = m->fbeg[(size_t)k + 1] - f0;
      return one_set_features_fn(m->sub[(size_t)k], nf, [fill, user, Wc, f0](int a0, int a1, double *dst, unsigned char *o) {
        fill(user, f0 + a0, f0 + a1, dst);
// ... 292 lines not shown
```

balm_amd/csrc/balm_internal.h:

```cpp
#pragma once
#include <hip/hip_runtime.h>
#include <atomic>
#include <condition_variable>
#include <cstddef>
#include <cstdint>
#include <functional>
#include <mutex>
#include <string>
#include <thread>
#include <vector>

#include "../../include/balm_hip.h"
#include "host_stage.h"

namespace balm {

constexpr int TILE = 80;
constexpr int TM = 5;
constexpr int TILE_ELEMS = TILE * TILE;
constexpr int FEAT_STRIDE = 24;
constexpr int DACC_LEFT = 27;
constexpr int DACC_RIGHT = 30;
constexpr int DACC_MAX = 30;
constexpr int NB = 48;
constexpr int MAX_W_LDS = 480;
constexpr int MAX_W = 1024;
constexpr int MAX_SHARDS = 16;

enum { FT_NN = 0, FT_VBAR = 1, FT_LAM = 4, FT_U0 = 7, FT_U1 = 10, FT_U2 = 13, FT_C0 = 16, FT_C1 = 17,
       FT_C2 = 18, FT_COE = 19 };

struct Timer {
  bool on = false;
  struct Span { hipEvent_t a, b; int slot; };
  std::vector<Span> pending;
  std::vector<hipEvent_t> pool;
  double ms[BALM_T_COUNT] = {0};
  long cnt[BALM_T_COUNT] = {0};
};

}

namespace balm {
struct WindowSession;
struct AssocMail {
  volatile unsigned int *host = nullptr; unsigned int *dev = nullptr; unsigned int seq = 0;
  unsigned long long *scan_state = nullptr; unsigned int scan_gen = 0;
};
constexpr long SCAN_TILES_CAP = 8192;
}

struct balm_ctx {
  int W = 0, n = 0, npad = 0, T = 0, ntiles = 0, device = 0, flags = 0;
  int nA = 0;
  int F = 0;
  hipStream_t stream = nullptr;
  std::string err;

  double *d_cl = nullptr;
  double *d_fix = nullptr;
  double *d_coe = nullptr;
  double *d_poses = nullptr;
  double *d_poses_tmp = nullptr;
  double *d_C = nullptr;
  double *d_feat = nullptr;
  double *d_feat_tmp = nullptr;
  double *d_rpart_tmp = nullptr;
  int nr_cur = 0, nr_tmp = 0;
  bool feat_cur_valid = false;
  double *d_Gt = nullptr;
  double *d_Gt2 = nullptr, *d_dpart2 = nullptr;
  size_t cap_Gt2 = 0, cap_dpart2 = 0;
  size_t gt_dirty_cols = ~(size_t)0;
  bool gt_cur_valid = false;
  int gt_parity = 0;
  bool gt_trial_valid = false;
  size_t cap_cl = 0, cap_fix = 0, cap_coe = 0, cap_C = 0, cap_feat = 0, cap_feat_tmp = 0, cap_rpart = 0, cap_rpart_tmp = 0;
  size_t cap_slot = 0, cap_items = 0, cap_chunk_ids = 0, cap_csr = 0;
  bool has_fix = false;
  size_t cap_Gt = 0;
  double *d_part = nullptr;
  size_t cap_part = 0;
  double *d_dpart = nullptr;
  size_t cap_dpart = 0;
  double *d_rpart = nullptr;
  double *d_red = nullptr;
  size_t red_len = 0;
  std::vector<int> h_jobs;
  bool sparse = false;
  int sp_nsteps = 0, sp_nchunks = 0, sp_nitems = 0;
  int *d_slot = nullptr;
  int *d_items = nullptr;
  int *d_chunk_ids = nullptr;
  double sp_steps = 0;
  int *d_csr = nullptr;
  int *d_jobs = nullptr;
  int *d_sub = nullptr;
  double *d_H = nullptr;
  double *d_g = nullptr;
  double *d_A = nullptr;
  double *d_Wp = nullptr;
  double *d_dvec = nullptr;
  double *d_z = nullptr;
  double *d_x = nullptr;
  int *d_perm = nullptr;
  int *d_flags = nullptr;
  long long *d_trace = nullptr;
  int fused_cap = -1;
  int chain_cap = -1;
  double *d_minv = nullptr;
  int *d_macro_tab = nullptr;
  int macro_tab_P = 0, macro_tab_NH = 0;
  double *d_dx = nullptr;
  double *d_scal = nullptr;
  double *h_scal = nullptr;
  double *d_hscal = nullptr;
  unsigned long long mail_seq = 0;
  bool need_minv = false;
  bool solve_tiled = false;
  int chain_refused_P[2] = {-1, -1};
  bool solve_backsub = false;
  bool counted_live = false;
  bool persistent_off = false;
  bool inject_solve_timeout = false;
  bool small_ready = false, small_refused = false;
  double u_value = 0.0;
  bool u_on_device = false;
  int u_ring = 0;
  static constexpr int LM_GRAPHS = 32;
  hipGraphExec_t lm_graph[LM_GRAPHS] = {};
  int lm_graph_form[LM_GRAPHS] = {};
  bool graphs_ok = true;
  int parity = 0;
  std::vector<int> planes_per_pose;
  double work_S = 0, work_B = 0;
  std::vector<double> assoc_clusters, assoc_coeffs;
  bool assoc_cl_on_device = false;
  std::vector<int> assoc_layer, assoc_point_feat;
  std::vector<double> assoc_fix;
  balm::WindowSession *window = nullptr;
  bool window_dead = false;
  balm::AssocMail amail;
  void *d_arena = nullptr;
  size_t arena_cap = 0;
  char *d_stage = nullptr;
  size_t stage_cap = 0, stage_off = 0;
  balm::PinnedRing ring;
  balm_allreduce_fn allreduce = nullptr;
  void *allreduce_user = nullptr;
  balm::Timer timer;
  void *comm = nullptr;
  std::atomic<bool> comm_dead{false};
  bool comm_aborted = false;
  std::timed_mutex comm_mu;
  int rank = 0, nranks = 1;
  unsigned long long *d_rowmax = nullptr, *d_rowmax2 = nullptr; size_t cap_rowmax = 0, cap_rowmax2 = 0;
  double *d_rowmax_part = nullptr; size_t cap_rowmax_part = 0;
  bool rowmax_cur_valid = false, rowmax_trial_valid = false;
  unsigned char *d_i8 = nullptr; size_t cap_i8 = 0;
  struct balm_multi *multi = nullptr;
  double *d_pre = nullptr;
};

namespace balm {

hipError_t prepare_device_accum();
hipError_t prepare_device_cov();
hipError_t preload_solve();
hipError_t preload_build();
hipError_t preload_voxel();
void launch_transpose_clusters(hipStream_t s, const double *aos, double *soa, int F, int W);
void launch_world_moments(hipStream_t s, const double *cl, const double *poses, int W, int f0, int f1, double *C);
struct EigenMail { double *scal; double *host; double stamp; int slot; };
int launch_feature_eigen(hipStream_t s, const double *C, const double *fix, const double *coe, int f0, int f1,
                         double *feat, double *rpart, const EigenMail *mail = nullptr);
int factors_grid(int W, int nfeat, int form);
int factors_chunk(int W);
bool launch_factors(hipStream_t s, int form, const double *cl, const double *poses, const double *feat, int W,
                    int npad, int f0, int f1, double *Gt, double *dpart, int nblk, const int *slot = nullptr,
                    unsigned long long *rowmax = nullptr, double *rowmax_part = nullptr);
int launch_moments_factors(hipStream_t s, int form, const double *cl, const double *poses, const double *fix, const double *coe, int W,
                           int npad, int F, double *Gt, double *dpart, int nblk, const int *slot, double *feat, double *rpart,
                           unsigned long long *rowmax = nullptr, double *rowmax_part = nullptr);
struct SyrkPlan { int SG; int nsteps; int Kpad; long nblocks; };
SyrkPlan plan_syrk(int ntiles, long K);
void launch_syrk(hipStream_t s, const double *Gt, int npad, int ntiles, const int *tileIJ, const SyrkPlan &p,
                 double *part);
void launch_syrk_sparse(hipStream_t s, const double *Gt, int npad, const int *jobs, const int *items, const int *chunk_ids,
                        int nsteps, long nitems, double *part);
void launch_reduce(hipStream_t s, const double *part, int SG, long tile_elems_total, const double *dpart, int nblk,
                   int dacc_len, const double *rpart, int nr, double *red, long red_dacc_off, long red_r_off,
                   const int *csr_ptr = nullptr);
void launch_assemble(hipStream_t s, int form, const double *red, long red_dacc_off, const int *tileIJ, int ntiles,
                     int W, double *H, double *g, const double *r_in = nullptr, double *r_out = nullptr);
void launch_sum_scalar(hipStream_t s, const double *rpart, int nr, double *out);
struct I8Layout { int T, rows_p, NT, M; long Kp; size_t off_digits, off_rowmax, off_scale, off_part; };
size_t syrk_i8_scratch_bytes(int n, long K, I8Layout *lay);
hipError_t prepare_device_syrk_i8();
int launch_syrk_i8(hipStream_t s, const double *Gt, int npad, int n, long K, const int *tileIJ, int ntiles, unsigned char *scratch, double *part,
                   const unsigned long long *rowmax_known = nullptr);

struct Barrier;
}

struct balm_multi {
  int n = 0;
  bool loopback = false;
  std::vector<balm_ctx *> sub;
  std::vector<int> fbeg;
  int F = 0;
  bool books_per_shard = false;
  std::vector<std::thread> th;
  std::mutex mu;
  std::condition_variable cv_go, cv_done;
  uint64_t gen = 0;
  int pending = 0;
  bool quit = false;
  const std::function<int(int)> *job = nullptr;
  std::vector<int> rc;
  balm::Barrier *bar = nullptr;
  std::atomic<int> abort_rc{0};
  std::atomic<bool> dead{false};
  std::atomic<uint64_t> lm_seq{0};
  uint64_t lm_epoch = 0;
  double lm_vals[2][8] = {{0}};
  std::vector<hipEvent_t> ev1, ev2;
  std::vector<double *> lb_tmp, lb_buf;
  std::vector<size_t> lb_cap;
};

namespace balm {
balm_multi *multi_new(const std::vector<balm_ctx *> &subs, bool loopback, std::string *err);
void multi_delete(balm_multi *m);
int multi_run(balm_multi *m, const std::function<int(int)> &f);
int comm_unique_id(void *out128);
int comm_init_rank(balm_ctx *ctx, int nranks, int rank, const void *id128);
void comm_destroy(balm_ctx *ctx);
const char *rccl_load_error();
int comm_allreduce(balm_ctx *ctx, double *buf, long n);
void comm_query(const balm_ctx *ctx, int *count, int *rank);
int loopback_allreduce(balm_ctx *ctx, double *buf, long n);
bool multi_is_loopback(const balm_ctx *ctx);
int multi_share_scalars(balm_ctx *ctx, int it, double *vals, int count);
void multi_abort(balm_multi *m, int rc);
int multi_host_barrier_rc(balm_ctx *ctx, int rc);

constexpr int SCAL_U = 5;
constexpr int SCAL_STAMP = 16 + 64;
bool chain_macro_plan(int P, int NH, std::vector<int> &tab);
void context_born(int device);
void context_gone(int device);
bool solve_timed_out(balm_ctx *c);
bool solve_is_persistent(const balm_ctx *c);
void launch_solve(balm_ctx *c, bool new_hessian, int upd_form = 0, const double *upd_poses = nullptr, double *upd_out = nullptr);
void launch_update_poses(hipStream_t s, int form, int W, const double *poses, const double *dx, double *out);
void launch_scalars_mail(hipStream_t s, double *d_scal, double *d_hscal, double stamp, const double *rpart = nullptr, int nr = 0,
                         int slot = 0);
void launch_reanchor(hipStream_t s, int W, double *poses);

struct AssocOpts {
  int W;
  double voxel_size;
  float thr[3];
  int min_ps, layer_limit, min_observers, fix_frames;
  double max_dis, ratio21_max, lam0_max;
  int fix_limit = 50;
  int defer_recut = 0;
};
int associate_device(hipStream_t s, const float *d_xyz, const int *d_frame, const long *d_first, const double *d_poses, long n, const AssocOpts &o,
                     void *arena, size_t arena_cap, size_t *arena_need, int *F_out, double **d_out, double **d_coe,
                     double **d_fix, int **d_layer, int **d_point_feat, long *n_roots, AssocMail *mail, bool *outputs_owned);

WindowSession *window_open(hipStream_t s, const AssocOpts &o);
void window_close(WindowSession *w);
int window_add_scan(WindowSession *w, const float *xyz_new, long n_new, const double *pose12, bool xyz_on_host);
int window_recut(WindowSession *w);
int window_marginalize(WindowSession *w, int mg, const double *poses);
int window_features(WindowSession *w, int min_observers, int *F_out, double **d_out, double **d_coe, double **d_fix, int **d_layer);
long window_get_points(WindowSession *w, float *xyz, int *slot, int *feature, long cap);
int window_count(const WindowSession *w);
int window_min_observers(const WindowSession *w);
long window_points(const WindowSession *w);
long window_nodes(const WindowSession *w);

int cov_factors_grid(int W, int F);
void launch_cov_factors(hipStream_t s, const double *cl, const double *ccov, double sigma2, const double *poses,
                        const double *feat, int W, int npad, int F, double *Gx, double *Gy, double *dpart, int nblk);
void launch_cov_reduce_tiles(hipStream_t s, const double *part, int SG, long tile_total, double *red);
void launch_cov_reduce_dacc(hipStream_t s, const double *dpart, int nblk, int W, double *out);
void launch_cov_assemble(hipStream_t s, const double *redx, const double *redy, const double *sdiag, const int *tileIJ,
                         int ntiles, int W, double *Rout);
void launch_congruence_inverse(balm_ctx *c, const double *Rraw, double *T0, double *T1, double *Rcov);

void launch_build_clusters(hipStream_t s, const float *xyz, const int *feat_id, const int *pose_id, long n_pts,
                           int F, int W, double *soa, int *unsorted_flag);
void launch_build_clusters_any(hipStream_t s, const float *xyz, const int *feat_id, const int *pose_id, long n_pts,
                               int F, int W, double *soa);
void launch_soa_to_aos(hipStream_t s, const double *soa, double *aos, int F, int W);
void launch_rebase_ids(hipStream_t s, int *d_id, long n, int base);
void launch_expand_ids(hipStream_t s, const long *d_first, int m, long n, int *d_id);
void launch_unpack_xyzw(hipStream_t s, const float *d_rec, long n, float *d_xyz, int *d_aux);
void launch_obs_mask(hipStream_t s, const double *soa, int F, int W, unsigned char *mask);

}
```

balm_amd/csrc/kernels_accum.hip:

```cpp
#include "balm_internal.h"

namespace balm {

typedef double d4 __attribute__((ext_vector_type(4)));
typedef double d2 __attribute__((ext_vector_type(2)));

__device__ __forceinline__ double wave_sum(double v) {
#pragma unroll
  for (int off = 32; off > 0; off >>= 1) v += __shfl_xor(v, off, 64);
  return v;
}

struct Obs {
  double N;
  double Rv[3];
  double b[3];
  double Pw[6];
};

__device__ __forceinline__ void to_world(const double P[6], const double v[3], double N, const double R[9],
                                         const double p[3], Obs &o) {
  o.N = N;
#pragma unroll
  for (int r = 0; r < 3; r++) o.Rv[r] = R[r] * v[0] + R[3 + r] * v[1] + R[6 + r] * v[2];
// ... 53 lines not shown
__global__ __launch_bounds__(256) void k_world_moments(const double *__restrict__ cl,
                                                       const double *__restrict__ poses, int W, int f0, int f1,
                                                       double *__restrict__ Cout) {
  extern __shared__ __attribute__((aligned(16))) double sp[];
  for (int t0 = 0; t0 < 12 * W; t0 += 10 * (int)blockDim.x) {
    double pv[10];
#pragma unroll
    for (int j = 0; j < 10; j++) {
      const int t = t0 + j * (int)blockDim.x + (int)threadIdx.x;
      pv[j] = t < 12 * W ? poses[t] : 0.0;
    }
#pragma unroll
    for (int j = 0; j < 10; j++) {
      const int t = t0 + j * (int)blockDim.x + (int)threadIdx.x;
      if (t < 12 * W) { const int i = t / 12, c = t - 12 * i; sp[c * W + i] = pv[j]; }
    }
  }
  __syncthreads();
  const int lane = threadIdx.x & 63, wv = threadIdx.x >> 6, nw = blockDim.x >> 6;
  for (int a = f0 + blockIdx.x * nw + wv; a < f1; a += gridDim.x * nw) {
    const double *ca = cl + (size_t)a * 10 * W;
    double acc[10];
#pragma unroll
    for (int c = 0; c < 10; c++) acc[c] = 0.0;
    for (int i = lane; i < W; i += 64) {
      double P[6], v[3];
      const double N = ca[(size_t)9 * W + i];
#pragma unroll
      for (int c = 0; c < 6; c++) P[c] = ca[(size_t)c * W + i];
#pragma unroll
      for (int c = 0; c < 3; c++) v[c] = ca[(size_t)(6 + c) * W + i];
      if ((int)N > 0) {
        double R[9], p[3];
#pragma unroll
        for (int c = 0; c < 9; c++) R[c] = sp[c * W + i];
#pragma unroll
        for (int c = 0; c < 3; c++) p[c] = sp[(9 + c) * W + i];
        Obs o;
        to_world(P, v, N, R, p, o);
#pragma unroll
        for (int c = 0; c < 6; c++) acc[c] += o.Pw[c];
#pragma unroll
        for (int c = 0; c < 3; c++) acc[6 + c] += o.b[c];
        acc[9] += N;
      }
    }
#pragma unroll
    for (int c = 0; c < 10; c++) acc[c] = wave_sum(acc[c]);
    if (lane == 0) {
#pragma unroll
      for (int c = 0; c < 10; c++) Cout[(size_t)a * 10 + c] = acc[c];
    }
  }
}

void launch_world_moments(hipStream_t s, const double *cl, const double *poses, int W, int f0, int f1, double *C) {
  int nf = f1 - f0;
  if (nf <= 0) return;
  int grid = (nf + 3) / 4;
  if (grid > 2048) grid = 2048;
  size_t lds = (size_t)12 * W * sizeof(double);
  hipLaunchKernelGGL(k_world_moments, dim3(grid), dim3(256), lds, s, cl, poses, W, f0, f1, C);
}

__device__ __forceinline__ void jrot(double &app, double &aqq, double &apq, double &arp, double &arq, double &v0p,
                                     double &v0q, double &v1p, double &v1q, double &v2p, double &v2q) {
  if (apq == 0.0) return;
  const double theta = (aqq - app) / (2.0 * apq);
  const double t = (theta >= 0.0 ? 1.0 : -1.0) / (fabs(theta) + sqrt(theta * theta + 1.0));
  const double c = 1.0 / sqrt(t * t + 1.0), s = t * c;
  app -= t * apq;
  aqq += t * apq;
  apq = 0.0;
  const double rp = c * arp - s * arq, rq = s * arp + c * arq;
  arp = rp; arq = rq;
  double x, y;
  x = c * v0p - s * v0q; y = s * v0p + c * v0q; v0p = x; v0q = y;
  x = c * v1p - s * v1q; y = s * v1p + c * v1q; v1p = x; v1q = y;
  x = c * v2p - s * v2q; y = s * v2p + c * v2q; v2p = x; v2q = y;
}

__device__ __forceinline__ void eig3_jacobi(double a00, double a01, double a02, double a11, double a12, double a22,
                                            double lam[3], double U[3][3]) {
  double v00 = 1, v01 = 0, v02 = 0, v10 = 0, v11 = 1, v12 = 0, v20 = 0, v21 = 0, v22 = 1;
  for (int sweep = 0; sweep < 30; sweep++) {
    const double off = a01 * a01 + a02 * a02 + a12 * a12;
    const double dia = a00 * a00 + a11 * a11 + a22 * a22;
    if (off <= 1e-300 || off <= 1e-34 * dia) break;
    jrot(a00, a11, a01, a02, a12, v00, v01, v10, v11, v20, v21);
    jrot(a00, a22, a02, a01, a12, v00, v02, v10, v12, v20, v22);
    jrot(a11, a22, a12, a01, a02, v01, v02, v11, v12, v21, v22);
  }
  double l0 = a00, l1 = a11, l2 = a22;
  double c0[3] = {v00, v10, v20}, c1[3] = {v01, v11, v21}, c2[3] = {v02, v12, v22};
#define BALM_CSWAP(la, lb, ca, cb)                                                         \
  if (la > lb) {                                                                            \
    double t_ = la; la = lb; lb = t_;                                                       \
    for (int k_ = 0; k_ < 3; k_++) { double s_ = ca[k_]; ca[k_] = cb[k_]; cb[k_] = s_; }    \
  }
  BALM_CSWAP(l0, l1, c0, c1)
  BALM_CSWAP(l1, l2, c1, c2)
  BALM_CSWAP(l0, l1, c0, c1)
#undef BALM_CSWAP
  lam[0] = l0; lam[1] = l1; lam[2] = l2;
  for (int k = 0; k < 3; k++) { U[k][0] = c0[k]; U[k][1] = c1[k]; U[k][2] = c2[k]; }
}

__global__ __launch_bounds__(256) void k_feature_eigen(const double *__restrict__ C, const double *__restrict__ fix,
                                                       const double *__restrict__ coe, int f0, int f1,
                                                       double *__restrict__ feat, double *__restrict__ rpart, EigenMail mail) {
  __shared__ double sred[256];
  const int a = f0 + blockIdx.x * blockDim.x + threadIdx.x;
  double res = 0.0;
  if (a < f1) {
    double c[10];
#pragma unroll
    for (int k = 0; k < 10; k++) c[k] = C[(size_t)a * 10 + k];
    if (fix) {
#pragma unroll
      for (int k = 0; k < 10; k++) c[k] += fix[(size_t)a * 10 + k];
    }
    const double NN = c[9];
    const double inv = 1.0 / NN;
    const double vb0 = c[6] * inv, vb1 = c[7] * inv, vb2 = c[8] * inv;
    double lam[3], U[3][3];
    eig3_jacobi(c[0] * inv - vb0 * vb0, c[1] * inv - vb0 * vb1, c[2] * inv - vb0 * vb2, c[3] * inv - vb1 * vb1,
                c[4] * inv - vb1 * vb2, c[5] * inv - vb2 * vb2, lam, U);
    const double w = coe[a];
    res = w * lam[0];
    double *f = feat + (size_t)a * FEAT_STRIDE;
    f[FT_NN] = NN;
    f[FT_VBAR] = vb0; f[FT_VBAR + 1] = vb1; f[FT_VBAR + 2] = vb2;
    f[FT_LAM] = lam[0]; f[FT_LAM + 1] = lam[1]; f[FT_LAM + 2] = lam[2];
#pragma unroll
    for (int k = 0; k < 3; k++) {
      f[FT_U0 + k] = U[k][0]; f[FT_U1 + k] = U[k][1]; f[FT_U2 + k] = U[k][2];
    }
    f[FT_C0] = sqrt(2.0 * w) * inv;
    f[FT_C1] = sqrt(2.0 * w / (lam[1] - lam[0])) * inv;
    f[FT_C2] = sqrt(2.0 * w / (lam[2] - lam[0])) * inv;
    f[FT_COE] = w;
  }
  sred[threadIdx.x] = res;
  __syncthreads();
  for (int s = 128; s > 0; s >>= 1) {
    if (threadIdx.x < s) sred[threadIdx.x] += sred[threadIdx.x + s];
    __syncthreads();
  }
  if (threadIdx.x == 0) rpart[blockIdx.x] = sred[0];
  if (!mail.host) return;
  if (threadIdx.x == 0) mail.scal[mail.slot] = sred[0];
  __syncthreads();
  volatile double *host = mail.host;
  if (threadIdx.x < 16) host[threadIdx.x] = ((int)threadIdx.x == mail.slot) ? sred[0] : mail.scal[threadIdx.x];
  __threadfence_system();
  __syncthreads();
  if (threadIdx.x == 0) { host[SCAL_STAMP] = mail.stamp; __threadfence_system(); }
}

int launch_feature_eigen(hipStream_t s, const double *C, const double *fix, const double *coe, int f0, int f1,
                         double *feat, double *rpart, const EigenMail *mail) {
  int nf = f1 - f0;
  if (nf <= 0) return 0;
  int grid = (nf + 255) / 256;
  const EigenMail none{nullptr, nullptr, 0.0, 0};
  hipLaunchKernelGGL(k_feature_eigen, dim3(grid), dim3(256), 0, s, C, fix, coe, f0, f1, feat, rpart, (mail && grid == 1) ? *mail : none);
  return grid;
}

__global__ __launch_bounds__(256) void k_sum_scalar(const double *__restrict__ part, int nr, double *__restrict__ out) {
  __shared__ double sred[256];
  double s = 0.0;
  for (int t = threadIdx.x; t < nr; t += 256) s += part[t];
  sred[threadIdx.x] = s;
  __syncthreads();
  for (int k = 128; k > 0; k >>= 1) {
    if (threadIdx.x < k) sred[threadIdx.x] += sred[threadIdx.x + k];
    __syncthreads();
  }
  if (threadIdx.x == 0) out[0] = sred[0];
}

void launch_sum_scalar(hipStream_t s, const double *rpart, int nr, double *out) {
  hipLaunchKernelGGL(k_sum_scalar, dim3(1), dim3(256), 0, s, rpart, nr, out);
}

__device__ __forceinline__ void cross3(const double a[3], const double b[3], double o[3]) {
  o[0] = a[1] * b[2] - a[2] * b[1];
  o[1] = a[2] * b[0] - a[0] * b[2];
  o[2] = a[0] * b[1] - a[1] * b[0];
}

__device__ __forceinline__ void store6(double *dst, const double x[6]) {
  d2 *q = reinterpret_cast<d2 *>(dst);
  d2 t0 = {x[0], x[1]}, t1 = {x[2], x[3]}, t2 = {x[4], x[5]};
  q[0] = t0; q[1] = t1; q[2] = t2;
}

struct FeatRec { double NN, iNN, vbar[3], u0[3], u1[3], u2[3], c0, c1, c2, coe; };

template <int FORM>
__device__ __forceinline__ void obs_factors(const FeatRec &fr, const double P[6], const double v[3], const double N,
                                            const double *__restrict__ sp, double *__restrict__ sacc, const int Wc, const int il,
                                            double col0[6], double col1[6], double col2[6]) {
  const double NN = fr.NN, iNN = fr.iNN, c0 = fr.c0, c1 = fr.c1, c2 = fr.c2, coe = fr.coe;
  const double *vbar = fr.vbar, *u0 = fr.u0, *u1 = fr.u1, *u2 = fr.u2;
  if ((int)N > 0) {
    double R[9], p[3];
#pragma unroll
    for (int c = 0; c < 9; c++) R[c] = sp[c * Wc + il];
#pragma unroll
    for (int c = 0; c < 3; c++) p[c] = sp[(9 + c) * Wc + il];

    if (FORM == 0) {
      Obs o;
      to_world(P, v, N, R, p, o);
      const double Pw[3][3] = {{o.Pw[0], o.Pw[1], o.Pw[2]}, {o.Pw[1], o.Pw[3], o.Pw[4]}, {o.Pw[2], o.Pw[4], o.Pw[5]}};
      double cvec[3];
#pragma unroll
      for (int r = 0; r < 3; r++) cvec[r] = o.b[r] - N * vbar[r];
      double m0[3], m1[3], m2[3];
      const double vu0 = vbar[0] * u0[0] + vbar[1] * u0[1] + vbar[2] * u0[2];
      const double vu1 = vbar[0] * u1[0] + vbar[1] * u1[1] + vbar[2] * u1[2];
      const double vu2 = vbar[0] * u2[0] + vbar[1] * u2[1] + vbar[2] * u2[2];
#pragma unroll
      for (int r = 0; r < 3; r++) {
        m0[r] = Pw[r][0] * u0[0] + Pw[r][1] * u0[1] + Pw[r][2] * u0[2] - o.b[r] * vu0;
        m1[r] = Pw[r][0] * u1[0] + Pw[r][1] * u1[1] + Pw[r][2] * u1[2] - o.b[r] * vu1;
        m2[r] = Pw[r][0] * u2[0] + Pw[r][1] * u2[1] + Pw[r][2] * u2[2] - o.b[r] * vu2;
      }
      const double s0 = cvec[0] * u0[0] + cvec[1] * u0[1] + cvec[2] * u0[2];
      const double s1 = cvec[0] * u1[0] + cvec[1] * u1[1] + cvec[2] * u1[2];
      const double s2 = cvec[0] * u2[0] + cvec[1] * u2[1] + cvec[2] * u2[2];
      double x00[3], x01[3], x10[3], x02[3], x20[3], bxu[3];
      cross3(m0, u0, x00);
      cross3(m0, u1, x01); cross3(m1, u0, x10);
      cross3(m0, u2, x02); cross3(m2, u0, x20);
      cross3(o.b, u0, bxu);
      double grad[6];
#pragma unroll
      for (int r = 0; r < 3; r++) {
        grad[r] = 2.0 * coe * iNN * x00[r];
        grad[3 + r] = 2.0 * coe * iNN * s0 * u0[r];
        col0[r] = c0 * bxu[r];
        col0[3 + r] = c0 * N * u0[r];
        col1[r] = c1 * (x01[r] + x10[r]);
        col1[3 + r] = c1 * (s0 * u1[r] + s1 * u0[r]);
        col2[r] = c2 * (x02[r] + x20[r]);
        col2[3 + r] = c2 * (s0 * u2[r] + s2 * u0[r]);
      }
      const double K[3][3] = {{0, -u0[2], u0[1]}, {u0[2], 0, -u0[0]}, {-u0[1], u0[0], 0}};
      double KP[3][3];
#pragma unroll
      for (int r = 0; r < 3; r++)
#pragma unroll
        for (int c = 0; c < 3; c++) KP[r][c] = K[r][0] * Pw[0][c] + K[r][1] * Pw[1][c] + K[r][2] * Pw[2][c];
      const double m0u0 = m0[0] * u0[0] + m0[1] * u0[1] + m0[2] * u0[2];
      const double k1 = coe * iNN, k2 = 2.0 * coe * iNN;
      double bd[21];
      int q = 0;
#pragma unroll
      for (int r = 0; r < 3; r++)
#pragma unroll
        for (int c = r; c < 3; c++) {
          double kpk = KP[r][0] * K[c][0] + KP[r][1] * K[c][1] + KP[r][2] * K[c][2];
          double ell = u0[r] * m0[c] + m0[r] * u0[c] - (r == c ? 2.0 * m0u0 : 0.0);
          bd[q++] = k1 * ell + k2 * kpk;
        }
#pragma unroll
      for (int r = 0; r < 3; r++)
#pragma unroll
        for (int c = 0; c < 3; c++) bd[q++] = k2 * bxu[r] * u0[c];
#pragma unroll
      for (int r = 0; r < 3; r++)
#pragma unroll
        for (int c = r; c < 3; c++) bd[q++] = k2 * N * u0[r] * u0[c];
#pragma unroll
      for (int k = 0; k < 6; k++) sacc[k * Wc + il] += grad[k];
#pragma unroll
      for (int k = 0; k < 21; k++) sacc[(6 + k) * Wc + il] += bd[k];
    } else {
      const double Pf[3][3] = {{P[0], P[1], P[2]}, {P[1], P[3], P[4]}, {P[2], P[4], P[5]}};
      const double NNi = (double)(int)NN;
      const double jNN = 1.0 / NNi;
      double r3[3];
#pragma unroll
      for (int c = 0; c < 3; c++) r3[c] = R[3 * c] * u0[0] + R[3 * c + 1] * u0[1] + R[3 * c + 2] * u0[2];
      double ai[3];
      cross3(v, r3, ai);
      double ti[3];
#pragma unroll
      for (int r = 0; r < 3; r++) ti[r] = p[r] - vbar[r];
      const double s = u0[0] * ti[0] + u0[1] * ti[1] + u0[2] * ti[2];
      double Pr[3];
#pragma unroll
      for (int r = 0; r < 3; r++) Pr[r] = Pf[r][0] * r3[0] + Pf[r][1] * r3[1] + Pf[r][2] * r3[2];
      const double h1[3] = {Pr[0] + v[0] * s, Pr[1] + v[1] * s, Pr[2] + v[2] * s};
      const double C1[3][3] = {{0, -h1[2], h1[1]}, {h1[2], 0, -h1[0]}, {-h1[1], h1[0], 0}};
      const double rh[3][3] = {{0, -r3[2], r3[1]}, {r3[2], 0, -r3[0]}, {-r3[1], r3[0], 0}};
      double Rv[3], combo2[3];
#pragma unroll
      for (int r = 0; r < 3; r++) {
        Rv[r] = R[r] * v[0] + R[3 + r] * v[1] + R[6 + r] * v[2];
        combo2[r] = Rv[r] + N * ti[r];
      }
      double E[3][3];
#pragma unroll
      for (int r = 0; r < 3; r++)
#pragma unroll
        for (int c = 0; c < 3; c++)
          E[r][c] = R[r] * Pf[0][c] + R[3 + r] * Pf[1][c] + R[6 + r] * Pf[2][c] + ti[r] * v[c];
      double Auk[3][6];
      const double c2u = combo2[0] * u0[0] + combo2[1] * u0[1] + combo2[2] * u0[2];
#pragma unroll
      for (int r = 0; r < 3; r++)
#pragma unroll
        for (int c = 0; c < 3; c++) {
          double erh = E[r][0] * rh[0][c] + E[r][1] * rh[1][c] + E[r][2] * rh[2][c];
          double rc1 = R[r] * C1[0][c] + R[3 + r] * C1[1][c] + R[6 + r] * C1[2][c];
          Auk[r][c] = (erh - rc1) * jNN;
          Auk[r][3 + c] = (combo2[r] * u0[c] + (r == c ? c2u : 0.0)) * jNN;
        }
      double jjt[6], a1[6], a2[6];
#pragma unroll
      for (int c = 0; c < 6; c++) {
        jjt[c] = Auk[0][c] * u0[0] + Auk[1][c] * u0[1] + Auk[2][c] * u0[2];
        a1[c] = Auk[0][c] * u1[0] + Auk[1][c] * u1[1] + Auk[2][c] * u1[2];
        a2[c] = Auk[0][c] * u2[0] + Auk[1][c] * u2[1] + Auk[2][c] * u2[2];
      }
      const double r0 = c0 * NN * jNN, r1 = c1 * NN, r2 = c2 * NN;
#pragma unroll
      for (int r = 0; r < 3; r++) {
        col0[r] = r0 * ai[r];
        col0[3 + r] = r0 * N * u0[r];
      }
#pragma unroll
      for (int c = 0; c < 6; c++) { col1[c] = r1 * a1[c]; col2[c] = r2 * a2[c]; }
      double D1[3][3];
#pragma unroll
      for (int r = 0; r < 3; r++)
#pragma unroll
        for (int c = 0; c < 3; c++)
          D1[r][c] = C1[r][c] - (rh[r][0] * Pf[0][c] + rh[r][1] * Pf[1][c] + rh[r][2] * Pf[2][c]);
      const double hj[3][3] = {{0, -jjt[2], jjt[1]}, {jjt[2], 0, -jjt[0]}, {-jjt[1], jjt[0], 0}};
      const double k2 = 2.0 * coe * jNN;
      double bd[24];
      int q = 0;
#pragma unroll
      for (int r = 0; r < 3; r++)
#pragma unroll
        for (int c = 0; c < 3; c++) {
          double d1rh = D1[r][0] * rh[0][c] + D1[r][1] * rh[1][c] + D1[r][2] * rh[2][c];
          bd[q++] = k2 * d1rh - 0.5 * coe * hj[r][c];
        }
#pragma unroll
      for (int r = 0; r < 3; r++)
#pragma unroll
        for (int c = 0; c < 3; c++) bd[q++] = k2 * ai[r] * u0[c];
#pragma unroll
      for (int r = 0; r < 3; r++)
#pragma unroll
        for (int c = r; c < 3; c++) bd[q++] = k2 * N * u0[r] * u0[c];
#pragma unroll
      for (int k = 0; k < 6; k++) sacc[k * Wc + il] += coe * jjt[k];
#pragma unroll
      for (int k = 0; k < 24; k++) sacc[(6 + k) * Wc + il] += bd[k];
    }
  } else {
#pragma unroll
    for (int k = 0; k < 6; k++) col0[k] = col1[k] = col2[k] = 0.0;
  }
}

__device__ __forceinline__ void track_rowmax(double rm[6], double &bad, const double col0[6], const double col1[6], const double col2[6]) {
#pragma unroll
  for (int k = 0; k < 6; k++) {
    rm[k] = fmax(rm[k], fmax(fabs(col0[k]), fmax(fabs(col1[k]), fabs(col2[k]))));
    bad = fma(col0[k] + col1[k] + col2[k], 0.0, bad);
  }
}
__device__ __forceinline__ void publish_rowmax(double *__restrict__ part, int W, int pose, const double rm[6], double bad) {
#pragma unroll
  for (int k = 0; k < 6; k++) part[(size_t)(blockIdx.x * 6 + k) * W + pose] = bad != bad ? bad : rm[k];
}
__device__ __forceinline__ double nanmax(double a, double b) { return (a != a || b != b) ? __longlong_as_double(0x7ff8000000000000ll) : fmax(a, b); }
__global__ __launch_bounds__(1024) void k_rowmax_reduce(const double *__restrict__ part, int nblk, int W, int npad, unsigned long long *__restrict__ rowmax) {
  __shared__ double sm[16][64];
  const int tx = threadIdx.x & 63, ty = threadIdx.x >> 6, t = blockIdx.x * 64 + tx;
  double m[4] = {0.0, 0.0, 0.0, 0.0};
  if (t < 6 * W) {
    int b = ty;
    for (; b + 48 < nblk; b += 64) {
#pragma unroll
      for (int u = 0; u < 4; u++) m[u] = nanmax(m[u], part[(size_t)(b + 16 * u) * 6 * W + t]);
    }
    for (; b < nblk; b += 16) m[0] = nanmax(m[0], part[(size_t)b * 6 * W + t]);
  }
  sm[ty][tx] = nanmax(nanmax(m[0], m[1]), nanmax(m[2], m[3]));
  __syncthreads();
  if (ty == 0) {
    double v = sm[0][tx];
#pragma unroll
    for (int k = 1; k < 16; k++) v = nanmax(v, sm[k][tx]);
    if (t < 6 * W) {
      const int r = t / W, pose = t - r * W;
      rowmax[6 * pose + r] = (unsigned long long)__double_as_longlong(v);
    } else if (t < npad) {
      rowmax[t] = 0ull;
    }
  }
}

template <int FORM, bool REGS, bool MAXR = false>
__global__ __launch_bounds__(256) void k_feature_factors(const double *__restrict__ cl,
                                                         const double *__restrict__ poses,
                                                         const double *__restrict__ feat, int W, int Wc, int npad, int f0,
                                                         int f1, double *__restrict__ Gt,
                                                         double *__restrict__ dpart, const int *__restrict__ slot, int staged,
                                                         double *__restrict__ rowmax_part = nullptr) {
  static_assert(!MAXR || REGS, "the row maxima live in the lane that owns the pose");
  double rm[6] = {0.0, 0.0, 0.0, 0.0, 0.0, 0.0}, bad = 0.0;
  constexpr int DACC = FORM == 0 ? DACC_LEFT : DACC_RIGHT;
  extern __shared__ __attribute__((aligned(16))) double sm[];
  const int p0 = blockIdx.y * Wc, wc = min(Wc, W - p0);
  double *sp = sm;
  double *sacc = sm + 12 * Wc;
  double preg[12], racc[DACC];
  if (REGS) {
    const double *q = poses + 12 * (p0 + (threadIdx.x < (unsigned)wc ? (int)threadIdx.x : 0));
#pragma unroll
    for (int c = 0; c < 12; c++) preg[c] = q[c];
#pragma unroll
    for (int k = 0; k < DACC; k++) racc[k] = 0.0;
  }
  if (!REGS)
  for (int t0 = 0; t0 < 12 * wc; t0 += 10 * (int)blockDim.x) {
    double pv[10];
#pragma unroll
    for (int j = 0; j < 10; j++) {
      const int t = t0 + j * (int)blockDim.x + (int)threadIdx.x;
      pv[j] = t < 12 * wc ? poses[12 * p0 + t] : 0.0;
    }
#pragma unroll
    for (int j = 0; j < 10; j++) {
      const int t = t0 + j * (int)blockDim.x + (int)threadIdx.x;
      if (t < 12 * wc) { const int il = t / 12, c = t - 12 * il; sp[c * Wc + il] = pv[j]; }
    }
  }
  if (!REGS) {
    for (int t = threadIdx.x; t < DACC * Wc; t += blockDim.x) sacc[t] = 0.0;
    __syncthreads();
  }

  double nxt[10];
  auto fetch = [&](int a, int i) {
    const double *ca = cl + (size_t)a * 10 * W + i;
#pragma unroll
    for (int c = 0; c < 10; c++) nxt[c] = ca[(size_t)c * W];
  };
  const int i_first = p0 + (threadIdx.x < (unsigned)wc ? (int)threadIdx.x : 0);
  const int a_begin = f0 + (int)blockIdx.x, a_end = f1, a_step = (int)gridDim.x;
  const int lane = threadIdx.x & 63;
  double *stg = sm + (12 + DACC) * Wc + (threadIdx.x >> 6) * 384;
  if (a_begin < a_end) fetch(a_begin, i_first);

  for (int a = a_begin; a < a_end; a += a_step) {
    const double *f = feat + (size_t)a * FEAT_STRIDE;
    const FeatRec fr = {f[FT_NN], 1.0 / f[FT_NN], {f[FT_VBAR], f[FT_VBAR + 1], f[FT_VBAR + 2]}, {f[FT_U0], f[FT_U0 + 1], f[FT_U0 + 2]},
                        {f[FT_U1], f[FT_U1 + 1], f[FT_U1 + 2]}, {f[FT_U2], f[FT_U2 + 1], f[FT_U2 + 2]}, f[FT_C0], f[FT_C1], f[FT_C2], f[FT_COE]};
    const double *ca = cl + (size_t)a * 10 * W;
    double *g0 = Gt + (size_t)(3 * (slot ? slot[a] : a - f0)) * npad;

    for (int ilb = 0; ilb < wc; ilb += blockDim.x) {
      const int il = ilb + (int)threadIdx.x;
      if (il - lane >= wc) break;
      const bool act = il < wc;
      const int i = p0 + (act ? il : wc - 1);
      double col0[6], col1[6], col2[6];
      double P[6], v[3];
      if (!act) {
#pragma unroll
        for (int c = 0; c < 6; c++) P[c] = 0.0;
        v[0] = v[1] = v[2] = 0.0;
      } else if (il == (int)threadIdx.x) {
#pragma unroll
        for (int c = 0; c < 6; c++) P[c] = nxt[c];
#pragma unroll
        for (int c = 0; c < 3; c++) v[c] = nxt[6 + c];
      } else {
#pragma unroll
        for (int c = 0; c < 6; c++) P[c] = ca[(size_t)c * W + i];
#pragma unroll
        for (int c = 0; c < 3; c++) v[c] = ca[(size_t)(6 + c) * W + i];
      }
      const double N = !act ? 0.0 : (il == (int)threadIdx.x ? nxt[9] : ca[(size_t)9 * W + i]);
      if (il == (int)threadIdx.x && a + a_step < a_end) fetch(a + a_step, i_first);
      if (REGS) obs_factors<FORM>(fr, P, v, N, preg, racc, 1, 0, col0, col1, col2);
      else obs_factors<FORM>(fr, P, v, N, sp, sacc, Wc, act ? il : wc - 1, col0, col1, col2);
      if (MAXR) track_rowmax(rm, bad, col0, col1, col2);
      if (!staged) {
        if (act) {
          store6(g0 + 6 * i, col0);
          store6(g0 + (size_t)npad + 6 * i, col1);
          store6(g0 + (size_t)2 * npad + 6 * i, col2);
        }
      } else {
        const int nval = 6 * min(64, wc - (il - lane));
        double *gw = g0 + 6 * (size_t)(p0 + il - lane);
        auto flush = [&](const double col[6], double *gcol) {
          d2 *q = reinterpret_cast<d2 *>(stg + 6 * lane);
          d2 t0 = {col[0], col[1]}, t1 = {col[2], col[3]}, t2 = {col[4], col[5]};
          q[0] = t0; q[1] = t1; q[2] = t2;
          asm volatile("" ::: "memory");
#pragma unroll
          for (int j = 0; j < 3; j++) {
            const int idx = 2 * (64 * j + lane);
            const d2 w = *reinterpret_cast<const d2 *>(stg + idx);
            if (idx < nval) *reinterpret_cast<d2 *>(gcol + idx) = w;
          }
          asm volatile("" ::: "memory");
        };
        flush(col0, gw);
        flush(col1, gw + (size_t)npad);
        flush(col2, gw + (size_t)2 * npad);
      }
    }
  }
  double *dp = dpart + (size_t)blockIdx.x * DACC * W + p0;
  if (REGS) {
    if (threadIdx.x < (unsigned)wc) {
#pragma unroll
      for (int k = 0; k < DACC; k++) dp[(size_t)k * W + threadIdx.x] = racc[k];
      if (MAXR) publish_rowmax(rowmax_part, W, p0 + (int)threadIdx.x, rm, bad);
    }
    return;
  }
  __syncthreads();
  for (int t = threadIdx.x; t < DACC * wc; t += blockDim.x) {
    const int k = t / wc, il = t - k * wc;
    dp[(size_t)k * W + il] = sacc[k * Wc + il];
  }
}

template <int FORM, bool MAXR = false>
__global__ __launch_bounds__(320, 3) void k_moments_factors(const double *__restrict__ cl, const double *__restrict__ poses,
                                                         const double *__restrict__ fix, const double *__restrict__ coe_in, int W, int npad,
                                                         int F, double *__restrict__ Gt, double *__restrict__ dpart,
                                                         const int *__restrict__ slot, double *__restrict__ feat_out,
                                                         double *__restrict__ rpart, double *__restrict__ rowmax_part = nullptr) {
  constexpr int DACC = FORM == 0 ? DACC_LEFT : DACC_RIGHT;
  double rm[6] = {0.0, 0.0, 0.0, 0.0, 0.0, 0.0}, bad = 0.0;
  extern __shared__ __attribute__((aligned(16))) double sm[];
  const int npl = (int)blockDim.x - 64, npw = npl >> 6;
  double *sp = sm;
  double *sacc = sm + 12 * W;
  double *mom = sacc + DACC * W;
  double *eig = mom + 80;
  const int tid = threadIdx.x, lane = tid & 63, wv = tid >> 6;
  const bool is_pose = tid < npl;
  for (int t = tid; t < 12 * W; t += blockDim.x) {
    const int i = t / 12, c = t - 12 * i;
    sp[c * W + i] = poses[t];
  }
  for (int t = tid; t < DACC * W; t += blockDim.x) sacc[t] = 0.0;
  __syncthreads();
  const int il = tid, G = gridDim.x, a0 = blockIdx.x;
  const bool has_pose = is_pose && il < W;
  double cur[10], nxt[10];
#pragma unroll
  for (int c = 0; c < 10; c++) cur[c] = nxt[c] = 0.0;
  auto fetch = [&](int a, double (&dst)[10]) {
    const double *ca = cl + (size_t)a * 10 * W + il;
#pragma unroll
// ... 11 lines not shown
      for (int c = 0; c < 3; c++) p[c] = sp[(9 + c) * W + il];
      Obs o;
      to_world(c10, c10 + 6, c10[9], R, p, o);
#pragma unroll
      for (int c = 0; c < 6; c++) m[c] = o.Pw[c];
#pragma unroll
      for (int c = 0; c < 3; c++) m[6 + c] = o.b[c];
      m[9] = c10[9];
    }
#pragma unroll
    for (int c = 0; c < 10; c++) m[c] = wave_sum(m[c]);
    if (lane == 0) {
#pragma unroll
      for (int c = 0; c < 10; c++) mom[(buf * 4 + wv) * 10 + c] = m[c];
    }
  };
  double res = 0.0;
  auto eigen_step = [&](int a, int buf) {
    double c[10];
#pragma unroll
    for (int k = 0; k < 10; k++) {
      double t = mom[(buf * 4) * 10 + k];
      for (int w = 1; w < npw; w++) t += mom[(buf * 4 + w) * 10 + k];
      c[k] = t;
    }
    if (fix) {
#pragma unroll
      for (int k = 0; k < 10; k++) c[k] += fix[(size_t)a * 10 + k];
    }
    const double NN = c[9], inv = 1.0 / NN;
    const double vb0 = c[6] * inv, vb1 = c[7] * inv, vb2 = c[8] * inv;
    double lam[3], U[3][3];
    eig3_jacobi(c[0] * inv - vb0 * vb0, c[1] * inv - vb0 * vb1, c[2] * inv - vb0 * vb2, c[3] * inv - vb1 * vb1,
                c[4] * inv - vb1 * vb2, c[5] * inv - vb2 * vb2, lam, U);
    const double w = coe_in[a];
    res += w * lam[0];
    double rec[FEAT_STRIDE];
#pragma unroll
    for (int k = 0; k < FEAT_STRIDE; k++) rec[k] = 0.0;
    rec[FT_NN] = NN;
    rec[FT_VBAR] = vb0; rec[FT_VBAR + 1] = vb1; rec[FT_VBAR + 2] = vb2;
    rec[FT_LAM] = lam[0]; rec[FT_LAM + 1] = lam[1]; rec[FT_LAM + 2] = lam[2];
#pragma unroll
    for (int k = 0; k < 3; k++) { rec[FT_U0 + k] = U[k][0]; rec[FT_U1 + k] = U[k][1]; rec[FT_U2 + k] = U[k][2]; }
    rec[FT_C0] = sqrt(2.0 * w) * inv;
    rec[FT_C1] = sqrt(2.0 * w / (lam[1] - lam[0])) * inv;
    rec[FT_C2] = sqrt(2.0 * w / (lam[2] - lam[0])) * inv;
    rec[FT_COE] = w;
    if (lane == 0) {
#pragma unroll
      for (int k = 0; k < FEAT_STRIDE; k++) { eig[buf * FEAT_STRIDE + k] = rec[k]; feat_out[(size_t)a * FEAT_STRIDE + k] = rec[k]; }
    }
  };

  if (a0 < F) {
    if (has_pose) fetch(a0, cur);
    if (is_pose) partial_moments(cur, 0);
    if (has_pose && a0 + G < F) fetch(a0 + G, nxt);
  }
  __syncthreads();
  if (!is_pose && a0 < F) eigen_step(a0, 0);
  __syncthreads();
  int b = 0;
  for (int a = a0; a < F; a += G, b ^= 1) {
    const bool has_next = a + G < F;
    if (is_pose && has_next) partial_moments(nxt, b ^ 1);
    __syncthreads();
    if (!is_pose) {
      if (has_next) eigen_step(a + G, b ^ 1);
    } else {
      const double *f = eig + b * FEAT_STRIDE;
      const FeatRec fr = {f[FT_NN], 1.0 / f[FT_NN], {f[FT_VBAR], f[FT_VBAR + 1], f[FT_VBAR + 2]}, {f[FT_U0], f[FT_U0 + 1], f[FT_U0 + 2]},
                          {f[FT_U1], f[FT_U1 + 1], f[FT_U1 + 2]}, {f[FT_U2], f[FT_U2 + 1], f[FT_U2 + 2]}, f[FT_C0], f[FT_C1], f[FT_C2], f[FT_COE]};
      if (has_pose) {
        double col0[6], col1[6], col2[6];
        obs_factors<FORM>(fr, cur, cur + 6, cur[9], sp, sacc, W, il, col0, col1, col2);
        if (MAXR) track_rowmax(rm, bad, col0, col1, col2);
        double *g0 = Gt + (size_t)(3 * (slot ? slot[a] : a)) * npad;
        store6(g0 + 6 * il, col0);
        store6(g0 + (size_t)npad + 6 * il, col1);
        store6(g0 + (size_t)2 * npad + 6 * il, col2);
#pragma unroll
        for (int c = 0; c < 10; c++) cur[c] = nxt[c];
        if (a + 2 * G < F) fetch(a + 2 * G, nxt);
      }
    }
    __syncthreads();
  }
  double *dp = dpart + (size_t)blockIdx.x * DACC * W;
  for (int t = tid; t < DACC * W; t += blockDim.x) dp[t] = sacc[t];
  if (MAXR && has_pose) publish_rowmax(rowmax_part, W, il, rm, bad);
  if (!is_pose && lane == 0) rpart[blockIdx.x] = res;
}

int factors_chunk(int W) { return W <= MAX_W_LDS ? W : 256; }

static size_t factors_lds(int W, int form) {
  const int dacc = form == 0 ? DACC_LEFT : DACC_RIGHT;
  return (size_t)(12 + dacc) * factors_chunk(W) * sizeof(double);
}
constexpr size_t FACTORS_STAGE_BYTES = 4 * 384 * sizeof(double);
static bool factors_staged(int W, int nfeat, int form) {
  if (factors_lds(W, form) + FACTORS_STAGE_BYTES > 160 * 1024) return false;
  if (const char *es = getenv("BALM_FACTORS_STAGE")) return es[0] != '0';
  return (long)nfeat * W >= 1000000;
}

int factors_grid(int W, int nfeat, int form) {
  size_t lds = factors_lds(W, form) + (factors_staged(W, nfeat, form) ? FACTORS_STAGE_BYTES : 0);
  int per_cu = (int)(160 * 1024 / lds);
  if (per_cu < 1) per_cu = 1;
  if (per_cu > 4) per_cu = 4;
  int grid = 256 * per_cu;
  if (grid > nfeat) grid = nfeat;
  if (grid < 1) grid = 1;
  return grid;
}

hipError_t prepare_device_accum() {
  hipError_t e = hipFuncSetAttribute((const void *)k_world_moments, hipFuncAttributeMaxDynamicSharedMemorySize, 160 * 1024);
  if (e == hipSuccess) e = hipFuncSetAttribute((const void *)k_feature_factors<0, false>, hipFuncAttributeMaxDynamicSharedMemorySize, 160 * 1024);
  if (e == hipSuccess) e = hipFuncSetAttribute((const void *)k_feature_factors<1, false>, hipFuncAttributeMaxDynamicSharedMemorySize, 160 * 1024);
  if (e == hipSuccess) e = hipFuncSetAttribute((const void *)k_feature_factors<0, true>, hipFuncAttributeMaxDynamicSharedMemorySize, 160 * 1024);
  if (e == hipSuccess) e = hipFuncSetAttribute((const void *)k_feature_factors<0, true, true>, hipFuncAttributeMaxDynamicSharedMemorySize, 160 * 1024);
  if (e == hipSuccess) e = hipFuncSetAttribute((const void *)k_moments_factors<0, false>, hipFuncAttributeMaxDynamicSharedMemorySize, 160 * 1024);
  if (e == hipSuccess) e = hipFuncSetAttribute((const void *)k_moments_factors<1, false>, hipFuncAttributeMaxDynamicSharedMemorySize, 160 * 1024);
  if (e == hipSuccess) e = hipFuncSetAttribute((const void *)k_moments_factors<0, true>, hipFuncAttributeMaxDynamicSharedMemorySize, 160 * 1024);
  if (e == hipSuccess) e = hipFuncSetAttribute((const void *)k_moments_factors<1, true>, hipFuncAttributeMaxDynamicSharedMemorySize, 160 * 1024);
  return e;
}

int launch_moments_factors(hipStream_t s, int form, const double *cl, const double *poses, const double *fix, const double *coe, int W,
                           int npad, int F, double *Gt, double *dpart, int nblk, const int *slot, double *feat, double *rpart,
                           unsigned long long *rowmax, double *rowmax_part) {
  const int dacc = form == 0 ? DACC_LEFT : DACC_RIGHT;
  const size_t lds = (size_t)((12 + dacc) * W + 80 + 2 * FEAT_STRIDE) * sizeof(double);
  const int bs = (W <= 64 ? 64 : (W <= 128 ? 128 : 256)) + 64;
  if (rowmax) {
    if (form == 0)
      hipLaunchKernelGGL((k_moments_factors<0, true>), dim3(nblk), dim3(bs), lds, s, cl, poses, fix, coe, W, npad, F, Gt, dpart, slot, feat, rpart, rowmax_part);
    else
      hipLaunchKernelGGL((k_moments_factors<1, true>), dim3(nblk), dim3(bs), lds, s, cl, poses, fix, coe, W, npad, F, Gt, dpart, slot, feat, rpart, rowmax_part);
    hipLaunchKernelGGL(k_rowmax_reduce, dim3((npad + 63) / 64), dim3(1024), 0, s, rowmax_part, nblk, W, npad, rowmax);
    return nblk;
  }
  if (form == 0)
    hipLaunchKernelGGL((k_moments_factors<0, false>), dim3(nblk), dim3(bs), lds, s, cl, poses, fix, coe, W, npad, F, Gt, dpart, slot, feat, rpart, nullptr);
  else
    hipLaunchKernelGGL((k_moments_factors<1, false>), dim3(nblk), dim3(bs), lds, s, cl, poses, fix, coe, W, npad, F, Gt, dpart, slot, feat, rpart, nullptr);
  return nblk;
}

bool launch_factors(hipStream_t s, int form, const double *cl, const double *poses, const double *feat, int W,
                    int npad, int f0, int f1, double *Gt, double *dpart, int nblk, const int *slot, unsigned long long *rowmax, double *rowmax_part) {
  const int Wc = factors_chunk(W), chunks = (W + Wc - 1) / Wc;
  size_t lds = factors_lds(W, form);
  int bs = W <= 64 ? 64 : (W <= 128 ? 128 : 256);
  const int staged = factors_staged(W, f1 - f0, form);
  if (staged) lds += FACTORS_STAGE_BYTES;
  const char *er = getenv("BALM_FACTORS_REGS");
  const bool regs = form == 0 && chunks == 1 && W <= bs && !(er && er[0] == '0');
  if (rowmax && regs) {
    hipLaunchKernelGGL((k_feature_factors<0, true, true>), dim3(nblk, chunks), dim3(bs), lds, s, cl, poses, feat, W, Wc, npad, f0, f1, Gt, dpart, slot, staged, rowmax_part);
    hipLaunchKernelGGL(k_rowmax_reduce, dim3((npad + 63) / 64), dim3(1024), 0, s, rowmax_part, nblk, W, npad, rowmax);
    return true;
  }
#define BALM_FACTORS(F, R) hipLaunchKernelGGL((k_feature_factors<F, R, false>), dim3(nblk, chunks), dim3(bs), lds, s, cl, poses, feat, W, Wc, npad, f0, f1, Gt, dpart, slot, staged, nullptr)
  if (form == 0) { if (regs) BALM_FACTORS(0, true); else BALM_FACTORS(0, false); }
  else BALM_FACTORS(1, false);
#undef BALM_FACTORS
  return false;
}

#include "syrk_mfma_asm.inc"

__device__ __forceinline__ void load5(const double *__restrict__ p, double (&x)[TM]) {
#pragma unroll
  for (int r = 0; r < TM; r++) x[r] = p[16 * r];
}

constexpr int SYRK_NBUF = 4;

__device__ __forceinline__ void syrk_sweep(const double *__restrict__ pa, const double *__restrict__ pb, size_t step,
                                           int nsteps) {
  double a[SYRK_NBUF][TM], b[SYRK_NBUF][TM];
#pragma unroll
  for (int i = 0; i < SYRK_NBUF - 1; i++) {
    load5(pa + i * step, a[i]);
    load5(pb + i * step, b[i]);
  }
  pa += (SYRK_NBUF - 1) * step;
  pb += (SYRK_NBUF - 1) * step;
  for (int s = 0; s < nsteps; s += SYRK_NBUF) {
#pragma unroll
    for (int j = 0; j < SYRK_NBUF; j++) {
      const int nb = (j + SYRK_NBUF - 1) % SYRK_NBUF;
      load5(pa, a[nb]);
      load5(pb, b[nb]);
      pa += step; pb += step;
      BALM_SYRK_MFMA_FULL(a[j], b[j])
    }
  }
}

#define BALM_DEFINE_MIXED_SWEEP(V)                                                                                  \
  __device__ __forceinline__ void syrk_sweep_mixed##V(const double *__restrict__ p, size_t step, int nsteps) {    \
    double x[SYRK_NBUF][BALM_SYRK_MIX##V##_NLOAD];                                                                  \
    _Pragma("unroll") for (int i = 0; i < SYRK_NBUF - 1; i++) {                                                    \
      const double *q = p + i * step;                                                                               \
      BALM_SYRK_MIX##V##_LOAD(q, x[i])                                                                              \
    }                                                                                                               \
    p += (SYRK_NBUF - 1) * step;                                                                                    \
    for (int s = 0; s < nsteps; s += SYRK_NBUF) {                                                                   \
      _Pragma("unroll") for (int j = 0; j < SYRK_NBUF; j++) {                                                      \
        const int nb = (j + SYRK_NBUF - 1) % SYRK_NBUF;                                                             \
        BALM_SYRK_MIX##V##_LOAD(p, x[nb])                                                                           \
        p += step;                                                                                                  \
        BALM_SYRK_MIX##V##_MFMA(x[j])                                                                               \
      }                                                                                                             \
    }                                                                                                               \
  }
BALM_DEFINE_MIXED_SWEEP(1)
BALM_DEFINE_MIXED_SWEEP(2)
BALM_DEFINE_MIXED_SWEEP(3)
#undef BALM_DEFINE_MIXED_SWEEP

__device__ __forceinline__ void syrk_accumulate(const double *__restrict__ Gt, int npad, int type, int I, int J,
                                                size_t k_begin, int nsteps) {
  const int lane = threadIdx.x;
  const double *base = Gt + (k_begin + (lane >> 4)) * (size_t)npad + (lane & 15);
  const double *pa = base + I * TILE;
  const double *pb = base + J * TILE;
  const size_t step = (size_t)4 * npad;
  if (type == 0) syrk_sweep(pa, pb, step, nsteps);
  else if (type == 1) syrk_sweep_mixed1(pa, step, nsteps);
  else if (type == 2) syrk_sweep_mixed2(pa, step, nsteps);
  else syrk_sweep_mixed3(pa, step, nsteps);
}

__device__ __forceinline__ void syrk_write_out(double *__restrict__ out) {
  asm volatile("s_nop 15\n\ts_nop 15\n\ts_nop 15" ::: "memory");
  out += threadIdx.x;
#define BALM_X(T)                                                                             \
  {                                                                                           \
    unsigned U[8];                                                                            \
    BALM_SYRK_READ_##T(U);                                                                    \
    _Pragma("unroll") for (int e = 0; e < 4; e++) out[(T * 4 + e) * 64] = __hiloint2double(U[2 * e + 1], U[2 * e]); \
  }
  BALM_SYRK_FOR_TILES(BALM_X)
#undef BALM_X
}

__device__ __forceinline__ long xcd_remap(long bid, long nblocks) {
  const long q = nblocks >> 3, r = nblocks & 7, x = bid & 7;
  return x * q + (x < r ? x : r) + (bid >> 3);
}

__global__ __launch_bounds__(64) void k_hessian_syrk(const double *__restrict__ Gt, int npad, int njobs,
                                                     const int *__restrict__ jobs, int nsteps, long nblocks,
                                                     double *__restrict__ part) {
  const long bid = xcd_remap(blockIdx.x, nblocks);
  const int tile = (int)(bid % njobs);
  const int sg = (int)(bid / njobs);
  BALM_SYRK_ZERO_ACC();
  syrk_accumulate(Gt, npad, jobs[4 * tile], jobs[4 * tile + 1], jobs[4 * tile + 2], (size_t)sg * nsteps * 4, nsteps);
  syrk_write_out(part + ((size_t)sg * njobs + tile) * TILE_ELEMS);
}

__global__ __launch_bounds__(64) void k_hessian_syrk_sparse(const double *__restrict__ Gt, int npad,
                                                            const int *__restrict__ jobs, const int *__restrict__ items,
                                                            const int *__restrict__ chunk_ids, int nsteps, long nitems,
                                                            double *__restrict__ part) {
  const long bid = xcd_remap(blockIdx.x, nitems);
  const int tile = items[4 * bid], first = items[4 * bid + 1], count = items[4 * bid + 2], slot = items[4 * bid + 3];
  const int type = jobs[4 * tile], I = jobs[4 * tile + 1], J = jobs[4 * tile + 2];
  BALM_SYRK_ZERO_ACC();
  for (int c = 0; c < count; c++)
    syrk_accumulate(Gt, npad, type, I, J, (size_t)chunk_ids[first + c] * nsteps * 4, nsteps);
  syrk_write_out(part + (size_t)slot * TILE_ELEMS);
}

SyrkPlan plan_syrk(int ntiles, long K) {
  SyrkPlan p;
  long steps = (K + 3) / 4;
  if (steps < 1) steps = 1;
  long max_sg = steps / 64;
  if (max_sg < 1) max_sg = 1;
  {
    const long one_round = 1024 / ntiles > 1 ? 1024 / ntiles : 1;
    if (max_sg < one_round) {
      long nst = SYRK_NBUF;
      while ((steps + nst - 1) / nst > one_round) nst += SYRK_NBUF;
      p.SG = (int)((steps + nst - 1) / nst);
      p.nsteps = (int)nst;
      p.Kpad = (int)(p.SG * nst * 4);
      p.nblocks = (long)p.SG * ntiles;
      return p;
    }
  }
  long base = (4096 + ntiles - 1) / ntiles, sg = base;
  double best = -1.0;
  for (long c = (base > 6 ? base - 6 : 1); c <= base + 6; c++) {
    const double per_xcd = (double)ntiles * c / 8.0;
    const double rounds = (double)(long)((per_xcd + 127.0) / 128.0);
    const double eff = per_xcd / (rounds * 128.0);
    if (eff > best + 1e-9) { best = eff; sg = c; }
  }
  if (sg > max_sg) sg = max_sg;
  if (steps / sg < 128 && sg > 1) {
    long one_round = 1024 / ntiles;
    if (one_round < 1) one_round = 1;
    if (one_round < sg) sg = one_round;
  }
  long nst = (steps + sg - 1) / sg;
  nst = (nst + SYRK_NBUF - 1) / SYRK_NBUF * SYRK_NBUF;
  p.SG = (int)sg;
  p.nsteps = (int)nst;
  p.Kpad = (int)(sg * nst * 4);
  p.nblocks = sg * ntiles;
  return p;
}

void launch_syrk_sparse(hipStream_t s, const double *Gt, int npad, const int *jobs, const int *items, const int *chunk_ids,
                        int nsteps, long nitems, double *part) {
  hipLaunchKernelGGL(k_hessian_syrk_sparse, dim3((unsigned)nitems), dim3(64), 0, s, Gt, npad, jobs, items, chunk_ids, nsteps,
                     nitems, part);
}

void launch_syrk(hipStream_t s, const double *Gt, int npad, int ntiles, const int *tileIJ, const SyrkPlan &p,
                 double *part) {
  hipLaunchKernelGGL(k_hessian_syrk, dim3((unsigned)p.nblocks), dim3(64), 0, s, Gt, npad, ntiles, tileIJ,
                     p.nsteps, p.nblocks, part);
}

template <class Sink>
__device__ __forceinline__ void reduce_tiles(const double *__restrict__ part, int SG, long tile_total, Sink sink,
                                             int bid, int nb) {
  for (long t = (long)bid * blockDim.x + threadIdx.x; t < tile_total; t += (long)nb * blockDim.x) {
    double s0 = 0.0, s1 = 0.0, s2 = 0.0, s3 = 0.0;
    const double *pp = part + t;
    int g = 0;
    for (; g + 3 < SG; g += 4) {
      s0 += pp[(size_t)g * tile_total];
      s1 += pp[(size_t)(g + 1) * tile_total];
      s2 += pp[(size_t)(g + 2) * tile_total];
      s3 += pp[(size_t)(g + 3) * tile_total];
    }
    for (; g < SG; g++) s0 += pp[(size_t)g * tile_total];
    sink(t, (s0 + s1) + (s2 + s3));
  }
}

template <class Sink>
__device__ __forceinline__ void reduce_tiles_quads(const double *__restrict__ part, int SG, long tile_total, Sink sink, int bid, int nb) {
  const int c = threadIdx.x & 3;
  const int full = SG / 4;
  for (long t = ((long)bid * blockDim.x + threadIdx.x) >> 2; t < tile_total; t += ((long)nb * blockDim.x) >> 2) {
    const double *pp = part + t + (size_t)c * tile_total;
    double s = 0.0;
    int m = 0;
    for (; m + 3 < full; m += 4) {
      const double v0 = pp[(size_t)(4 * m) * tile_total], v1 = pp[(size_t)(4 * m + 4) * tile_total],
                   v2 = pp[(size_t)(4 * m + 8) * tile_total], v3 = pp[(size_t)(4 * m + 12) * tile_total];
      s += v0;
      s += v1;
      s += v2;
      s += v3;
    }
    for (; m < full; m++) s += pp[(size_t)(4 * m) * tile_total];
    if (c == 0)
      for (int g = 4 * full; g < SG; g++) s += part[(size_t)g * tile_total + t];
    s += __shfl_xor(s, 1, 64);
    s += __shfl_xor(s, 2, 64);
    if (c == 0) sink(t, s);
  }
}

template <class Sink>
__device__ __forceinline__ void reduce_tiles_csr(const double *__restrict__ part, const int *__restrict__ ptr, long tile_total,
                                                 Sink sink, int bid, int nb) {
  for (long t = (long)bid * blockDim.x + threadIdx.x; t < tile_total; t += (long)nb * blockDim.x) {
    const int job = (int)(t / TILE_ELEMS);
    const long e = t - (long)job * TILE_ELEMS;
    const int s0 = ptr[job], s1 = ptr[job + 1];
    double a0 = 0.0, a1 = 0.0, a2 = 0.0, a3 = 0.0;
    int g = s0;
    for (; g + 3 < s1; g += 4) {
      a0 += part[(size_t)g * TILE_ELEMS + e];
      a1 += part[(size_t)(g + 1) * TILE_ELEMS + e];
      a2 += part[(size_t)(g + 2) * TILE_ELEMS + e];
      a3 += part[(size_t)(g + 3) * TILE_ELEMS + e];
    }
    for (; g < s1; g++) a0 += part[(size_t)g * TILE_ELEMS + e];
    sink(t, (a0 + a1) + (a2 + a3));
  }
}

__device__ __forceinline__ void reduce_dacc(const double *__restrict__ dpart, int nblk, int dacc_len, int dacc_cap,
                                            const double *__restrict__ rpart, int nr, double *__restrict__ red_dacc,
                                            double *__restrict__ red_r, int bid) {
  __shared__ double sq[256];
  const int jl = threadIdx.x & 63, q = threadIdx.x >> 6;
  const int j = bid * 64 + jl;
  double s = 0.0;
  if (j < dacc_len) {
    const int chunk = (nblk + 3) / 4;
    const int b0 = q * chunk, b1 = min(nblk, b0 + chunk);
    double a[8];
#pragma unroll
    for (int k = 0; k < 8; k++) a[k] = 0.0;
    int b = b0;
    for (; b + 7 < b1; b += 8) {
#pragma unroll
      for (int k = 0; k < 8; k++) a[k] += dpart[(size_t)(b + k) * dacc_len + j];
    }
    for (; b < b1; b++) a[0] += dpart[(size_t)b * dacc_len + j];
    s = ((a[0] + a[1]) + (a[2] + a[3])) + ((a[4] + a[5]) + (a[6] + a[7]));
  }
  sq[threadIdx.x] = s;
  __syncthreads();
  if (q == 0 && j < dacc_len) red_dacc[j] = (sq[jl] + sq[64 + jl]) + (sq[128 + jl] + sq[192 + jl]);
  if (q == 0 && j >= dacc_len && j < dacc_cap) red_dacc[j] = 0.0;
  if (bid == 0) {
    __syncthreads();
    double r = 0.0;
    for (int t = threadIdx.x; t < nr; t += 256) r += rpart[t];
    sq[threadIdx.x] = r;
    __syncthreads();
    for (int k = 128; k > 0; k >>= 1) {
      if (threadIdx.x < k) sq[threadIdx.x] += sq[threadIdx.x + k];
      __syncthreads();
    }
    if (threadIdx.x == 0) { red_r[0] = sq[0]; red_r[1] = 0.0; }
  }
}

__global__ __launch_bounds__(256) void k_reduce_all(const double *__restrict__ part, int SG, const int *__restrict__ csr_ptr, long tile_total,
                                                    int tile_blocks, const double *__restrict__ dpart, int nblk, int dacc_len, int dacc_cap,
                                                    const double *__restrict__ rpart, int nr, double *__restrict__ red, long dacc_off, long r_off, int quads) {
  if ((int)blockIdx.x < tile_blocks) {
    auto to_payload = [&](long t, double v) { red[t] = v; };
    if (csr_ptr) reduce_tiles_csr(part, csr_ptr, tile_total, to_payload, blockIdx.x, tile_blocks);
    else if (quads) reduce_tiles_quads(part, SG, tile_total, to_payload, blockIdx.x, tile_blocks);
    else reduce_tiles(part, SG, tile_total, to_payload, blockIdx.x, tile_blocks);
  } else {
    reduce_dacc(dpart, nblk, dacc_len, dacc_cap, rpart, nr, red + dacc_off, red + r_off, (int)blockIdx.x - tile_blocks);
  }
}

void launch_reduce(hipStream_t s, const double *part, int SG, long tile_total, const double *dpart, int nblk,
                   int dacc_len, const double *rpart, int nr, double *red, long dacc_off, long r_off, const int *csr_ptr) {
  const int dacc_cap = (int)(r_off - dacc_off);
  static const bool no_quads = getenv("BALM_REDUCE_QUADS") && getenv("BALM_REDUCE_QUADS")[0] == '0';
  const int quads = !csr_ptr && !no_quads && tile_total <= 32768 && SG >= 8;
  int grid = (int)(((quads ? 4 : 1) * tile_total + 255) / 256);
  if (grid > 8192) grid = 8192;
  hipLaunchKernelGGL(k_reduce_all, dim3(grid + (dacc_cap + 63) / 64), dim3(256), 0, s, part, SG, csr_ptr, tile_total, grid, dpart, nblk, dacc_len,
                     dacc_cap, rpart, nr, red, dacc_off, r_off, quads);
}

__device__ __forceinline__ int sym3(int r, int c) {
  if (r > c) { int t = r; r = c; c = t; }
  return r == 0 ? c : (r == 1 ? 2 + c : 5);
}

template <int FORM>
__device__ __forceinline__ double blockdiag_at(const double *__restrict__ dacc, int W, int i, int r, int c) {
  const double *d = dacc + i;
  if (FORM == 0) {
    if (r < 3 && c < 3) return d[(size_t)(6 + sym3(r, c)) * W];
    if (r < 3 && c >= 3) return d[(size_t)(12 + 3 * r + (c - 3)) * W];
    if (r >= 3 && c < 3) return d[(size_t)(12 + 3 * c + (r - 3)) * W];
    return d[(size_t)(21 + sym3(r - 3, c - 3)) * W];
  } else {
    if (r < 3 && c < 3) return d[(size_t)(6 + 3 * r + c) * W];
    if (r < 3 && c >= 3) return d[(size_t)(15 + 3 * r + (c - 3)) * W];
    if (r >= 3 && c < 3) return d[(size_t)(15 + 3 * c + (r - 3)) * W];
    return d[(size_t)(24 + sym3(r - 3, c - 3)) * W];
  }
}

template <int FORM>
__global__ __launch_bounds__(256) void k_assemble(const double *__restrict__ red, long dacc_off,
                                                  const int *__restrict__ tileIJ, int ntiles, int W,
                                                  double *__restrict__ H, double *__restrict__ g, const double *__restrict__ r_in,
                                                  double *__restrict__ r_out) {
  const int n = 6 * W;
  if (r_out && blockIdx.x == 0 && threadIdx.x == 0) *r_out = *r_in;
  const long total = (long)ntiles * TILE_ELEMS;
  const double *dacc = red + dacc_off;
  for (long t = (long)blockIdx.x * blockDim.x + threadIdx.x; t < total; t += (long)gridDim.x * blockDim.x) {
    const int tile = (int)(t / TILE_ELEMS);
    const int e = (int)(t - (long)tile * TILE_ELEMS);
    const int lane = e & 63, slot = e >> 6;
    const int reg = slot & 3, mt = slot >> 2;
    const int rc = tileIJ[tile * 25 + mt];
    const int row = (rc >> 16) * 16 + (lane >> 4) + 4 * reg;
    const int col = (rc & 0xffff) * 16 + (lane & 15);
    if (row >= n || col >= n || row > col) continue;
    double val = -red[t];
    const int pi = row / 6, pj = col / 6;
    if (pi == pj) {
      const int r = row - 6 * pi, c = col - 6 * pi;
      val += blockdiag_at<FORM>(dacc, W, pi, r, c);
      if (FORM == 1 && r != c) {
        H[(size_t)row * n + col] = -red[t] + blockdiag_at<FORM>(dacc, W, pi, c, r);
        H[(size_t)col * n + row] = val;
        continue;
      }
    }
    H[(size_t)col * n + row] = val;
    H[(size_t)row * n + col] = val;
  }
  for (long t = (long)blockIdx.x * blockDim.x + threadIdx.x; t < n; t += (long)gridDim.x * blockDim.x) {
    const int i = (int)(t / 6), k = (int)(t - 6 * (t / 6));
    g[t] = dacc[(size_t)k * W + i];
  }
}

void launch_assemble(hipStream_t s, int form, const double *red, long dacc_off, const int *tileIJ, int ntiles, int W,
                     double *H, double *g, const double *r_in, double *r_out) {
  long total = (long)ntiles * TILE_ELEMS;
  int grid = (int)((total + 255) / 256);
  if (grid > 4096) grid = 4096;
  if (form == 0)
    hipLaunchKernelGGL(k_assemble<0>, dim3(grid), dim3(256), 0, s, red, dacc_off, tileIJ, ntiles, W, H, g, r_in, r_out);
  else
    hipLaunchKernelGGL(k_assemble<1>, dim3(grid), dim3(256), 0, s, red, dacc_off, tileIJ, ntiles, W, H, g, r_in, r_out);
}


}
```

balm_amd/csrc/kernels_solve.hip:

```cpp
#include <algorithm>
#include <cfloat>
#include <cstdlib>
#include <cstring>

#include "balm_internal.h"

namespace balm {

typedef double d4 __attribute__((ext_vector_type(4)));

template <int MAXI>
__global__ __launch_bounds__(256) void k_rank_diag(const double *__restrict__ H, int n, int nA, int *__restrict__ perm) {
  extern __shared__ __attribute__((aligned(16))) double dabs[];
  int *part = reinterpret_cast<int *>(dabs + nA);
  double dv[MAXI];
#pragma unroll
  for (int it = 0; it < MAXI; it++) {
    const int i = threadIdx.x + 256 * it;
    dv[it] = i < n ? fabs(H[(size_t)i * n + i]) : -1.0;
  }
#pragma unroll
  for (int it = 0; it < MAXI; it++) {
    const int i = threadIdx.x + 256 * it;
    if (i < nA) dabs[i] = dv[it] == dv[it] ? dv[it] : -0.5;
// ... 707 lines not shown
}

static void launch_build_A(balm_ctx *c) {
  const int n = c->n, nA = c->nA, P = nA / NB;
  const double *pu = c->u_on_device ? c->d_scal + SCAL_U : nullptr;
  const int tiled = c->solve_tiled ? 1 : 0;
  const int nflags = 2 * (2 * P + 1) * P + P + 8;
  const size_t lds = (size_t)n * sizeof(double);
#define BALM_BUILD_A(M) hipLaunchKernelGGL(k_build_A<M>, dim3(nA), dim3(256), lds, c->stream, c->d_H, c->d_g, n, nA, c->d_perm, pu, c->u_value, \
                                           c->d_A, c->d_flags, nflags, c->d_x + nA, c->d_minv + (size_t)P * NB * NB, tiled)
  if (nA <= 256 * 5) BALM_BUILD_A(5);
  else if (nA <= 256 * 10) BALM_BUILD_A(10);
  else if (nA <= 256 * 16) BALM_BUILD_A(16);
  else BALM_BUILD_A(25);
#undef BALM_BUILD_A
}

static void launch_factor(balm_ctx *c) {
  hipStream_t s = c->stream;
  const int nA = c->nA, P = nA / NB;
  const bool backsub = c->solve_tiled;
  bool want_fused = backsub || solve_is_persistent(c);
  c->solve_backsub = false;
  static const bool dbg = getenv("BALM_SOLVE_DEBUG") != nullptr;
  if (dbg) fprintf(stderr, "balm_hip: solve P=%d persistent=%d backsub=%d chain_cap=%d fused_cap=%d multi=%d\n", P, (int)want_fused,
                   (int)backsub, c->chain_cap, c->fused_cap, c->multi ? c->multi->n : 0);
  if (backsub) {
    if (launch_factor_chain(c, false, c->solve_tiled)) { c->solve_backsub = true; return; }
    if (P > FUSED_MAX_P) want_fused = false;
    if (c->solve_tiled) { c->solve_tiled = false; launch_build_A(c); }
  } else {
    if (want_fused && solve_wants_chain(c, solve_mode()) && launch_factor_chain(c, true, false)) return;
  }
  if (want_fused) {
    const size_t lds = (size_t)(12 * FLR + 2 * NB * NB + NB) * sizeof(double);
    if (c->fused_cap < 0) c->fused_cap = fused_capacity(lds);
    const int RB = 2 * P + 1;
    int NH = persistent_slots(c, c->fused_cap) - RB;
    const int most = (P - 2) * P;
    if (NH > most) NH = most;
    if (P == 2) NH = 0;
    if (NH >= (P > 2 ? 1 : 0)) {
      FusedArgs fa{c->d_A, c->d_dvec, c->d_z, c->d_flags, c->d_flags + (size_t)RB * P, nA, P, RB, NH > 0 ? NH : 1, c->d_trace};
      if (persistent_launch(c, k_ldl_fused, dim3(RB + (P > 2 ? NH : 0)), dim3(FT), fa, lds, s) == hipSuccess)
        return;
      hipGetLastError();
      c->fused_cap = 0;
    }
  }
  const char *la = getenv("BALM_LOOKAHEAD");
  const bool lookahead = la ? !strcmp(la, "1") : true;
  const size_t wp_stride = (size_t)NB * (2 * nA + NB);
  for (int p = 0; p < P; p++) {
    const int c0 = p * NB;
    const int m = nA - c0 - NB;
    const int nR = nA + NB + NB * (p + 1);
    const int rows = nR - (c0 + NB);
    const int npb = (rows + PANEL_ROWS - 1) / PANEL_ROWS;
    const int mt = m / NB;
    double *Wp = c->d_Wp + (lookahead ? (size_t)(p & 1) * wp_stride : 0);
    const int mt_prev = mt + 1;
    if (lookahead && p > 0 && mt_prev > 1) {
      const int gx = (3 * (mt_prev - 1) + 3) / 4, gy = mt_prev + 1 + p;
      hipLaunchKernelGGL(k_ldl_panel_trail, dim3(npb + gx * gy), dim3(256), 0, s, c->d_A, nA, c0, nR, c->d_dvec, Wp, c->d_z, npb,
                         c0 - NB, c->d_Wp + (size_t)((p - 1) & 1) * wp_stride, mt_prev, gx);
    } else {
      hipLaunchKernelGGL(k_ldl_panel, dim3(npb), dim3(256), 0, s, c->d_A, nA, c0, nR, c->d_dvec, Wp, c->d_z);
    }
    if (m <= 0) continue;
    const int gy = mt + 1 + (p + 1);
    if (lookahead) hipLaunchKernelGGL(k_ldl_trail, dim3(1, gy), dim3(256), 0, s, c->d_A, nA, c0, Wp, mt, 0, 3);
    else hipLaunchKernelGGL(k_ldl_trail, dim3((3 * mt + 3) / 4, gy), dim3(256), 0, s, c->d_A, nA, c0, Wp, mt, 0, 3 * mt);
  }
}

#include "kernels_small.inc"

void launch_solve(balm_ctx *c, bool new_hessian, int upd_form, const double *upd_poses, double *upd_out) {
  hipStream_t s = c->stream;
  const int n = c->n, nA = c->nA;
  if (solve_wants_small(c)) {
    c->solve_backsub = false; c->solve_tiled = false;
    if (launch_solve_small(c, upd_form, upd_poses, upd_out)) return;
  }
  const double *pu = c->u_on_device ? c->d_scal + SCAL_U : nullptr;
  if (new_hessian) {
    const size_t lds = (size_t)nA * sizeof(double) + 256 * sizeof(int);
    const dim3 grid((nA + 15) / 16);
    if (nA <= 256 * 5) hipLaunchKernelGGL(k_rank_diag<5>, grid, dim3(256), lds, s, c->d_H, n, nA, c->d_perm);
    else if (nA <= 256 * 10) hipLaunchKernelGGL(k_rank_diag<10>, grid, dim3(256), lds, s, c->d_H, n, nA, c->d_perm);
    else if (nA <= 256 * 16) hipLaunchKernelGGL(k_rank_diag<16>, grid, dim3(256), lds, s, c->d_H, n, nA, c->d_perm);
    else hipLaunchKernelGGL(k_rank_diag<25>, grid, dim3(256), lds, s, c->d_H, n, nA, c->d_perm);
  }
  c->solve_tiled = solve_wants_backsub(c);
  launch_build_A(c);
  if (c->inject_solve_timeout) {
    const int P = nA / NB;
    hipMemsetAsync(c->d_flags + (size_t)2 * (2 * P + 1) * P + P, 1, sizeof(int), s);
    c->inject_solve_timeout = false;
  }
  launch_factor(c);
  if (c->solve_backsub) {
    const int P = nA / NB;
    hipLaunchKernelGGL(k_ldl_backsolve, dim3(P), dim3(256), 0, s, c->d_A, nA, P, c->solve_tiled ? 1 : 0, c->d_minv, c->d_dvec, c->d_z, c->d_x + nA, c->d_x,
                       c->d_flags + (size_t)2 * (2 * P + 1) * P + P);
  } else {
    hipLaunchKernelGGL(k_ldl_apply, dim3((nA + 63) / 64, APPLY_CHUNKS), dim3(256), 0, s, c->d_A, nA, c->d_dvec, c->d_z, c->d_x);
  }
  {
    const int P = nA / NB;
    int *abortf = c->d_flags + (size_t)2 * (2 * P + 1) * P + P;
    const int nch = c->solve_backsub ? 1 : APPLY_CHUNKS;
    hipLaunchKernelGGL(k_ldl_finish, dim3(1), dim3(1024), 0, s, c->d_x, nA, n, c->d_perm, c->d_H, c->d_g, pu, c->u_value, c->d_dx,
                       c->d_scal, abortf, upd_form, c->W, upd_poses, upd_out, nch);
  }
}

__global__ void k_update_poses(int form, int W, const double *__restrict__ poses, const double *__restrict__ dx,
                               double *__restrict__ out) {
  const int j = blockIdx.x * blockDim.x + threadIdx.x;
  if (j < W) update_pose(form, j, poses, dx, out);
}

void launch_update_poses(hipStream_t s, int form, int W, const double *poses, const double *dx, double *out) {
  hipLaunchKernelGGL(k_update_poses, dim3((W + 127) / 128), dim3(128), 0, s, form, W, poses, dx, out);
}

__global__ __launch_bounds__(256) void k_reanchor(int W, double *__restrict__ poses) {
  __shared__ double e0[12];
  if (threadIdx.x < 12) e0[threadIdx.x] = poses[threadIdx.x];
  __syncthreads();
  for (int j = threadIdx.x; j < W; j += blockDim.x) {
    double *q = poses + 12 * j;
    double R[3][3], p[3] = {q[9] - e0[9], q[10] - e0[10], q[11] - e0[11]};
#pragma unroll
    for (int c = 0; c < 3; c++)
#pragma unroll
      for (int r = 0; r < 3; r++) R[r][c] = q[3 * c + r];
#pragma unroll
    for (int r = 0; r < 3; r++) {
#pragma unroll
      for (int c = 0; c < 3; c++)
        q[3 * c + r] = e0[3 * r] * R[0][c] + e0[3 * r + 1] * R[1][c] + e0[3 * r + 2] * R[2][c];
      q[9 + r] = e0[3 * r] * p[0] + e0[3 * r + 1] * p[1] + e0[3 * r + 2] * p[2];
    }
  }
}

void launch_reanchor(hipStream_t s, int W, double *poses) {
  hipLaunchKernelGGL(k_reanchor, dim3(1), dim3(256), 0, s, W, poses);
}

__global__ __launch_bounds__(256) void k_scalars_mail(double *__restrict__ scal, volatile double *__restrict__ host, double stamp,
                                                      const double *__restrict__ rpart, int nr, int slot) {
  __shared__ double sred[256];
  if (rpart) {
    double s = 0.0;
    for (int t = threadIdx.x; t < nr; t += 256) s += rpart[t];
    sred[threadIdx.x] = s;
    __syncthreads();
    for (int k = 128; k > 0; k >>= 1) {
      if (threadIdx.x < k) sred[threadIdx.x] += sred[threadIdx.x + k];
      __syncthreads();
    }
    if (threadIdx.x == 0) scal[slot] = sred[0];
    __syncthreads();
  }
  if (threadIdx.x < 16) host[threadIdx.x] = (rpart && (int)threadIdx.x == slot) ? sred[0] : scal[threadIdx.x];
  __threadfence_system();
  __syncthreads();
  if (threadIdx.x == 0) { host[SCAL_STAMP] = stamp; __threadfence_system(); }
}

void launch_scalars_mail(hipStream_t s, double *d_scal, double *d_hscal, double stamp, const double *rpart, int nr, int slot) {
  hipLaunchKernelGGL(k_scalars_mail, dim3(1), dim3(256), 0, s, d_scal, d_hscal, stamp, rpart, nr, slot);
}

hipError_t preload_solve() {
  hipFuncAttributes a;
  return hipFuncGetAttributes(&a, (const void *)k_ldl_apply);
}

}
```

include/balm_hip.h:

```cpp
#ifndef BALM_HIP_H
#define BALM_HIP_H

#include <stddef.h>

#ifdef __cplusplus
extern "C" {
#endif

typedef struct balm_ctx balm_ctx;

enum { BALM_FORM_LEFT = 0, BALM_FORM_RIGHT = 1 };

enum {
  BALM_OK = 0,
  BALM_ERR_ARG = 1,
  BALM_ERR_HIP = 2,
  BALM_ERR_STATE = 3,
  BALM_ERR_TOO_FEW_PLANES = 4,
  BALM_ERR_NUMERIC = 5
};

enum {
  BALM_FLAG_TIMING = 1,
  BALM_FLAG_LOOPBACK_SHARDS = 2,
  BALM_FLAG_SYRK_INT8 = 4
};

typedef struct balm_iter_log {
  double r1, r2, u, v, q, q1;
  int accepted;
  int hess_evaluated;
} balm_iter_log;

typedef struct balm_lm_opts {
  int form;
  double u0;
  int max_iter;
  double rel_tol;
  int min_planes_per_pose;
  int force_hess;
  int no_stop;
  int verbose;
  int reanchor;
  double abs_tol;
} balm_lm_opts;

balm_ctx *balm_create(int win_size, int device, int flags);
void balm_destroy(balm_ctx *ctx);

int balm_prewarm(int device);

balm_ctx *balm_create_multi(int win_size, int first_device, int n_devices, int flags);

int balm_comm_unique_id(void *id128);
int balm_comm_init_rank(balm_ctx *ctx, int n_ranks, int rank, const void *id128);
int balm_comm_info(balm_ctx *ctx, long *out4);

int balm_set_features(balm_ctx *ctx, int F, const double *clusters, const double *fix,
                      const double *coeffs);

typedef void (*balm_fill_clusters_fn)(void *user, int f0, int f1, double *dst);
int balm_set_features_cb(balm_ctx *ctx, int F, balm_fill_clusters_fn fill, void *user, const double *fix,
                         const double *coeffs);

int balm_evaluate(balm_ctx *ctx, int form, const double *poses, int head, int end, double *Hess,
                  double *JacT, double *residual);

int balm_only_residual(balm_ctx *ctx, const double *poses, double *residual);

int balm_solve_damped(balm_ctx *ctx, const double *Hess, const double *JacT, double u, double *dxi,
                      double *q1);

int balm_damping_iter(balm_ctx *ctx, const balm_lm_opts *opts, double *poses_inout,
                      balm_iter_log *log, int *n_iters);

int balm_build_clusters(balm_ctx *ctx, int F, const float *xyz, const int *feat_id,
                        const int *pose_id, long n_pts, const double *fix, const double *coeffs,
                        double *clusters_out);

int balm_build_clusters_planes(balm_ctx *ctx, int F, const void *const *plane_points, const long *plane_count,
                               size_t stride_bytes, size_t pose_offset_bytes, const double *fix, const double *coeffs,
                               double *clusters_out);

typedef struct balm_voxel_opts {
  double voxel_size;
  float eigen_thr[3];
  int min_ps;
  int layer_limit;
  int min_observers;
  int fix_frames;
  double max_plane_dist;
  double max_lambda21;
  double max_lambda0;
  int want_point_features;
  int fix_point_limit;
  int defer_recut;
} balm_voxel_opts;
void balm_voxel_defaults(balm_voxel_opts *opts);
int balm_associate(balm_ctx *ctx, const balm_voxel_opts *opts, const float *xyz, const int *frame_id,
                   long n_pts, const double *poses, int *F_out, long *n_root_voxels);

int balm_associate_scans(balm_ctx *ctx, const balm_voxel_opts *opts, int n_scans, const void *const *scan_points,
                         const long *scan_count, size_t stride_bytes, const double *poses, int *F_out,
                         long *n_root_voxels);

int balm_window_open(balm_ctx *ctx, const balm_voxel_opts *opts);
int balm_window_recut(balm_ctx *ctx);
int balm_window_add_scan(balm_ctx *ctx, const float *xyz, long n_pts, const double *pose12);
int balm_window_add_scan_strided(balm_ctx *ctx, const void *points, long n_pts, size_t stride_bytes, const double *pose12);
int balm_window_features(balm_ctx *ctx, int *F_out);
int balm_window_marginalize(balm_ctx *ctx, int mg_size, const double *poses);
int balm_window_info(balm_ctx *ctx, int *scans_in_window, long *points, long *nodes);
int balm_window_get_points(balm_ctx *ctx, float *xyz, int *slot, int *feature, long capacity, long *n_out);
int balm_window_close(balm_ctx *ctx);

int balm_get_features(balm_ctx *ctx, double *clusters, double *coeffs, int *layer);

int balm_get_association(balm_ctx *ctx, double *fix, int *point_feature);

int balm_pose_covariance(balm_ctx *ctx, const double *poses, const double *cluster_cov, double point_sigma,
                         double *Rcov, double *Rcov_raw);

typedef int (*balm_allreduce_fn)(void *dev_buf, long n_doubles, void *user);
int balm_set_allreduce(balm_ctx *ctx, balm_allreduce_fn fn, void *user);

enum {
  BALM_T_MOMENTS = 0,
  BALM_T_FACTORS = 1,
  BALM_T_SYRK = 2,
  BALM_T_ASSEMBLE = 3,
  BALM_T_SOLVE = 4,
  BALM_T_UPDATE = 5,
  BALM_T_BUILD = 6,
  BALM_T_VOXEL = 7,
  BALM_T_COV = 8,
  BALM_T_COMM = 9,
  BALM_T_UPLOAD = 10,
  BALM_T_COUNT = 11
};
int balm_get_timing(balm_ctx *ctx, double *ms, long *count);
int balm_get_shard_timing(balm_ctx *ctx, int shard, double *ms, long *count);

int balm_get_solve_trace(balm_ctx *ctx, long long *ticks, long capacity, int *dims3);
int balm_reset_timing(balm_ctx *ctx);

int balm_chain_macro_plan(int panels, int helpers, int *table, long capacity);

int balm_work_model(balm_ctx *ctx, double *out4);

const char *balm_last_error(balm_ctx *ctx);
const char *balm_version(void);

#define BALM_ABI_VERSION 6
int balm_abi_version(void);

#ifdef __cplusplus
}
#endif
#endif
```

Baseline: 246.7.

## Speculatively enqueue next LM Hessian behind trial residual with device-side go flag

After the trial residual, the next iteration's Hessian build (factors, SYRK, reduce, assemble) is enqueued before the host sees the accept/reject decision. A device-computed go flag in the mail kernel picks the trial or current inputs, or skips the work, so the GPU stays busy while the host reads scalars. Timing spans and the scalar wait are reworked to cope with the extra queued work. The cost is wasted GPU work when the speculation is not needed, more complex state handling, and wrong results if the device-side decision ever disagrees with the host's.

Result: no change. 248.3 (median of 3 runs) (+0.6%).

```diff
diff --git a/balm_amd/capi.py b/balm_amd/capi.py
--- a/balm_amd/capi.py
+++ b/balm_amd/capi.py
@@ -12,6 +12,7 @@
 FLAG_TIMING = 1
 FLAG_LOOPBACK_SHARDS = 2
 FLAG_SYRK_INT8 = 4
+FLAG_NO_LM_AHEAD = 8
 T_MOMENTS, T_FACTORS, T_SYRK, T_ASSEMBLE, T_SOLVE, T_UPDATE, T_BUILD, T_VOXEL, T_COV, T_COMM, T_UPLOAD, T_COUNT = range(12)
 TIMING_NAMES = ["moments", "factors", "syrk", "assemble", "solve", "update", "build", "voxel", "cov", "comm", "upload"]
 
@@ -142,6 +143,8 @@
         self.L = lib()
         self.W = int(win_size)
         self.n = 6 * self.W
+        if os.environ.get("BALM_LM_AHEAD", "")[:1] == "0":
+            flags = int(flags) | FLAG_NO_LM_AHEAD
         if n_devices is None:
             self.h = self.L.balm_create(self.W, int(device), int(flags))
         else:
diff --git a/balm_amd/csrc/balm_capi.hip b/balm_amd/csrc/balm_capi.hip
--- a/balm_amd/csrc/balm_capi.hip
+++ b/balm_amd/csrc/balm_capi.hip
@@ -78,8 +78,8 @@
 }
 
 struct Span {
-  balm_ctx *c; int slot; hipEvent_t a = nullptr, b = nullptr;
-  Span(balm_ctx *ctx, int s) : c(ctx), slot(s) {
+  balm_ctx *c; int slot; bool ahead; hipEvent_t a = nullptr, b = nullptr;
+  Span(balm_ctx *ctx, int s, bool ahead_ = false) : c(ctx), slot(s), ahead(ahead_) {
     if (!c->timer.on) return;
     a = take(); b = take();
     hipEventRecord(a, c->stream);
@@ -87,7 +87,7 @@
   ~Span() {
     if (!c->timer.on) return;
     hipEventRecord(b, c->stream);
-    c->timer.pending.push_back({a, b, slot});
+    (ahead ? c->timer.ahead : c->timer.pending).push_back({a, b, slot});
   }
   hipEvent_t take() {
     if (!c->timer.pool.empty()) { hipEvent_t e = c->timer.pool.back(); c->timer.pool.pop_back(); return e; }
@@ -102,6 +102,30 @@
     c->timer.pool.push_back(sp.a); c->timer.pool.push_back(sp.b);
   }
   c->timer.pending.clear();
+  c->timer.mail_mark = c->timer.ready = 0;
+}
+
+void collect_timing_ready(balm_ctx *c) {
+  size_t k = 0;
+  for (; k < c->timer.ready && k < c->timer.pending.size(); k++) {
+    auto &sp = c->timer.pending[k];
+    float ms = 0;
+    const hipError_t e = hipEventElapsedTime(&ms, sp.a, sp.b);
+    if (e == hipErrorNotReady) { hipGetLastError(); break; }
+    if (e == hipSuccess) { c->timer.ms[sp.slot] += ms; c->timer.cnt[sp.slot]++; }
+    c->timer.pool.push_back(sp.a); c->timer.pool.push_back(sp.b);
+  }
+  c->timer.pending.erase(c->timer.pending.begin(), c->timer.pending.begin() + (long)k);
+  c->timer.ready -= k;
+  c->timer.mail_mark -= std::min(k, c->timer.mail_mark);
+}
+
+void ahead_settle(balm_ctx *c, bool ran) {
+  for (auto &sp : c->timer.ahead) {
+    if (ran) c->timer.pending.push_back(sp);
+    else { c->timer.pool.push_back(sp.a); c->timer.pool.push_back(sp.b); }
+  }
+  c->timer.ahead.clear();
 }
 
 template <class T>
@@ -198,6 +222,22 @@
   volatile double *stamp = ctx->h_scal + SCAL_STAMP;
   const double want = (double)ctx->mail_seq;
   const auto t0 = std::chrono::steady_clock::now();
+  if (ctx->ahead_queued) {
+    if (ctx->timer.on) collect_timing_ready(ctx);
+    auto t_query = t0 + std::chrono::milliseconds(50);
+    for (int spin = 0;; spin++) {
+      if (*stamp == want) { std::atomic_thread_fence(std::memory_order_acquire); ctx->timer.ready = ctx->timer.mail_mark; return BALM_OK; }
+      if ((spin & 255) != 255) continue;
+      const auto now = std::chrono::steady_clock::now();
+      if (now < t_query) continue;
+      t_query = now + std::chrono::milliseconds(50);
+      const hipError_t e = hipStreamQuery(ctx->stream);
+      if (e == hipErrorNotReady) { hipGetLastError(); continue; }
+      if (e == hipSuccess && *stamp == want) { std::atomic_thread_fence(std::memory_order_acquire); ctx->timer.ready = ctx->timer.mail_mark; return BALM_OK; }
+      if (e != hipSuccess) { ctx->err = std::string("balm_damping_iter: ") + hipGetErrorString(e); return BALM_ERR_HIP; }
+      ctx->err = "balm_damping_iter: the iteration's scalars did not arrive"; return BALM_ERR_HIP;
+    }
+  }
   for (int spin = 0;; spin++) {
     if (*stamp == want) { std::atomic_thread_fence(std::memory_order_acquire); collect_timing_if_idle(ctx); return BALM_OK; }
     if ((spin & 255) == 255 && std::chrono::steady_clock::now() - t0 > std::chrono::microseconds(300)) break;
@@ -215,14 +255,15 @@
   }
 }
 
-int residual_device(balm_ctx *ctx, const double *d_poses, int f0, int f1, int slot, bool defer_sum = false, bool send_mail = false) {
+int residual_device(balm_ctx *ctx, const double *d_poses, int f0, int f1, int slot, bool defer_sum = false, bool send_mail = false,
+                    const GoRule *go_rule = nullptr) {
   if (f1 <= f0) {
     HIP_TRY(hipMemsetAsync(ctx->d_scal + slot, 0, sizeof(double), ctx->stream));
     ctx->nr_tmp = 0;
   } else {
     Span sp(ctx, BALM_T_MOMENTS);
     launch_world_moments(ctx->stream, ctx->d_cl, d_poses, ctx->W, f0, f1, ctx->d_C);
-    const EigenMail mail{ctx->d_scal, ctx->d_hscal, send_mail ? (double)++ctx->mail_seq : 0.0, slot};
+    const EigenMail mail{ctx->d_scal, ctx->d_hscal, send_mail ? (double)++ctx->mail_seq : 0.0, slot, go_rule ? *go_rule : GoRule()};
     ctx->nr_tmp = launch_feature_eigen(ctx->stream, ctx->d_C, ctx->has_fix ? ctx->d_fix : nullptr, ctx->d_coe, f0, f1, ctx->d_feat_tmp,
                                        ctx->d_rpart_tmp, send_mail ? &mail : nullptr);
     if (!defer_sum) launch_sum_scalar(ctx->stream, ctx->d_rpart_tmp, ctx->nr_tmp, ctx->d_scal + slot);
@@ -281,9 +322,55 @@
   return BALM_OK;
 }
 
+struct EvalInputs { const double *poses, *feat, *rpart; int nr; };
+static int enqueue_hessian(balm_ctx *ctx, int form, const double *d_poses, const double *d_feat, const double *d_rpart, int nr, int f0, int f1,
+                           int slot, bool factors, double *zero_from, size_t zero_count, const double *go, const EvalInputs *alt, bool *rowmax_out) {
+  const int W = ctx->W, nf = f1 - f0;
+  const int dacc = form == 0 ? DACC_LEFT : DACC_RIGHT;
+  const bool ahead = go != nullptr;
+  int rc;
+  SyrkPlan plan = plan_syrk(ctx->ntiles, 3L * nf);
+  const int nblk = factors_grid(W, nf, form);
+  hipStream_t s = ctx->stream;
+  const bool sparse = ctx->sparse && f0 == 0 && f1 == ctx->F;
+  bool rowmax_valid = ctx->rowmax_cur_valid;
+  if (factors) {
+    Span sp(ctx, BALM_T_FACTORS, ahead);
+    if (zero_count) HIP_TRY(hipMemsetAsync(zero_from, 0, zero_count * sizeof(double), s));
+    const bool rm = rowmax_valid = launch_factors(s, form, ctx->d_cl, d_poses, d_feat, W, ctx->npad, f0, f1, ctx->d_Gt, ctx->d_dpart, nblk,
+                                   sparse ? ctx->d_slot : nullptr, (!sparse && syrk_int8_for(ctx, 3L * nf)) ? ctx->d_rowmax : nullptr, ctx->d_rowmax_part, go,
+                                                  alt ? alt->poses : nullptr, alt ? alt->feat : nullptr);
+    if (rowmax_out) *rowmax_out = rm;
+  }
+  HIP_TRY(hipGetLastError());
+  const bool int8 = !sparse && syrk_int8_for(ctx, 3L * nf);
+  {
+    Span sp(ctx, BALM_T_SYRK, ahead);
+    if (sparse) launch_syrk_sparse(s, ctx->d_Gt, ctx->npad, ctx->d_jobs, ctx->d_items, ctx->d_chunk_ids, ctx->sp_nsteps, ctx->sp_nitems, ctx->d_part, go);
+    else if (int8) {
+      if (launch_syrk_i8(s, ctx->d_Gt, ctx->npad, ctx->n, 3L * nf, ctx->d_sub, ctx->ntiles, ctx->d_i8, ctx->d_part,
+                         rowmax_valid ? ctx->d_rowmax : nullptr)) { ctx->err = "INT8 SYRK: unsupported size"; return BALM_ERR_ARG; }
+      plan.SG = 1;
+    }
+    else launch_syrk(s, ctx->d_Gt, ctx->npad, ctx->ntiles, ctx->d_jobs, plan, ctx->d_part, go);
+  }
+  {
+    Span sp(ctx, BALM_T_ASSEMBLE, ahead);
+    launch_reduce(s, ctx->d_part, plan.SG, (long)ctx->ntiles * TILE_ELEMS, ctx->d_dpart, nblk, dacc * W,
+                  d_rpart, nr, ctx->d_red, red_dacc_off(ctx), red_r_off(ctx), sparse ? ctx->d_csr : nullptr, go,
+                  alt ? alt->rpart : nullptr, alt ? alt->nr : 0);
+  }
+  if ((rc = hook_allreduce(ctx, ctx->d_red, (long)ctx->red_len))) return rc;
+  {
+    Span sp(ctx, BALM_T_ASSEMBLE, ahead);
+    launch_assemble(s, form, ctx->d_red, red_dacc_off(ctx), ctx->d_sub, ctx->ntiles, W, ctx->d_H, ctx->d_g, ctx->d_red + red_r_off(ctx),
+                    ctx->d_scal + slot, go);
+  }
+  return BALM_OK;
+}
+
 int evaluate_device(balm_ctx *ctx, int form, const double *d_poses, int f0, int f1, int slot) {
   const int W = ctx->W, nf = f1 - f0;
-  const int dacc = form == 0 ? DACC_LEFT : DACC_RIGHT;
   int rc;
   if (nf <= 0) {
     HIP_TRY(hipMemsetAsync(ctx->d_red, 0, ctx->red_len * sizeof(double), ctx->stream));
@@ -293,9 +380,8 @@
                     ctx->d_red + red_r_off(ctx), ctx->d_scal + slot);
     return BALM_OK;
   }
-  SyrkPlan plan = plan_syrk(ctx->ntiles, 3L * nf);
+  const SyrkPlan plan = plan_syrk(ctx->ntiles, 3L * nf);
   if ((rc = prepare_evaluate(ctx, form, nf))) return rc;
-  const int nblk = factors_grid(W, nf, form);
   hipStream_t s = ctx->stream;
   if (!(ctx->feat_cur_valid && f0 == 0 && f1 == ctx->F)) {
     Span sp(ctx, BALM_T_MOMENTS);
@@ -303,45 +389,25 @@
     ctx->nr_cur = launch_feature_eigen(s, ctx->d_C, ctx->has_fix ? ctx->d_fix : nullptr, ctx->d_coe, f0, f1, ctx->d_feat, ctx->d_rpart);
     ctx->feat_cur_valid = (f0 == 0 && f1 == ctx->F);
   }
-  const int nr = ctx->nr_cur;
   const bool sparse = ctx->sparse && f0 == 0 && f1 == ctx->F;
   const size_t kpad = sparse ? (size_t)ctx->sp_nchunks * ctx->sp_nsteps * 4 : (size_t)plan.Kpad;
-  if (!(ctx->gt_cur_valid && ctx->feat_cur_valid && f0 == 0 && f1 == ctx->F)) {
-    Span sp(ctx, BALM_T_FACTORS);
+  const bool factors = !(ctx->gt_cur_valid && ctx->feat_cur_valid && f0 == 0 && f1 == ctx->F);
+  double *zero_from = nullptr;
+  size_t zero_count = 0;
+  if (factors) {
     const size_t k0 = (size_t)3 * nf, k1 = kpad + 64;
     if (ctx->gt_dirty_cols == ~(size_t)0) {
-      HIP_TRY(hipMemsetAsync(ctx->d_Gt, 0, ctx->cap_Gt * sizeof(double), s));
-      ctx->gt_dirty_cols = 0;
+      zero_from = ctx->d_Gt; zero_count = ctx->cap_Gt;
     } else if (ctx->gt_dirty_cols > k0) {
-      HIP_TRY(hipMemsetAsync(ctx->d_Gt + k0 * ctx->npad, 0, (std::max(ctx->gt_dirty_cols, k1) - k0) * ctx->npad * sizeof(double), s));
+      zero_from = ctx->d_Gt + k0 * ctx->npad; zero_count = (std::max(ctx->gt_dirty_cols, k1) - k0) * ctx->npad;
     }
     ctx->gt_dirty_cols = k0;
-    ctx->rowmax_cur_valid = launch_factors(s, form, ctx->d_cl, d_poses, ctx->d_feat, W, ctx->npad, f0, f1, ctx->d_Gt, ctx->d_dpart, nblk,
-                                           sparse ? ctx->d_slot : nullptr, (!sparse && syrk_int8_for(ctx, 3L * nf)) ? ctx->d_rowmax : nullptr, ctx->d_rowmax_part);
+  }
+  bool rowmax = false;
+  if ((rc = enqueue_hessian(ctx, form, d_poses, ctx->d_feat, ctx->d_rpart, ctx->nr_cur, f0, f1, slot, factors, zero_from, zero_count, nullptr, nullptr, &rowmax))) return rc;
+  if (factors) {
+    ctx->rowmax_cur_valid = rowmax;
     ctx->gt_cur_valid = false;
-  }
-  HIP_TRY(hipGetLastError());
-  const bool int8 = !sparse && syrk_int8_for(ctx, 3L * nf);
-  {
-    Span sp(ctx, BALM_T_SYRK);
-    if (sparse) launch_syrk_sparse(s, ctx->d_Gt, ctx->npad, ctx->d_jobs, ctx->d_items, ctx->d_chunk_ids, ctx->sp_nsteps, ctx->sp_nitems, ctx->d_part);
-    else if (int8) {
-      if (launch_syrk_i8(s, ctx->d_Gt, ctx->npad, ctx->n, 3L * nf, ctx->d_sub, ctx->ntiles, ctx->d_i8, ctx->d_part,
-                         ctx->rowmax_cur_valid ? ctx->d_rowmax : nullptr)) { ctx->err = "INT8 SYRK: unsupported size"; return BALM_ERR_ARG; }
-      plan.SG = 1;
-    }
-    else launch_syrk(s, ctx->d_Gt, ctx->npad, ctx->ntiles, ctx->d_jobs, plan, ctx->d_part);
-  }
-  {
-    Span sp(ctx, BALM_T_ASSEMBLE);
-    launch_reduce(s, ctx->d_part, plan.SG, (long)ctx->ntiles * TILE_ELEMS, ctx->d_dpart, nblk, dacc * W,
-                  ctx->d_rpart, nr, ctx->d_red, red_dacc_off(ctx), red_r_off(ctx), sparse ? ctx->d_csr : nullptr);
-  }
-  if ((rc = hook_allreduce(ctx, ctx->d_red, (long)ctx->red_len))) return rc;
-  {
-    Span sp(ctx, BALM_T_ASSEMBLE);
-    launch_assemble(s, form, ctx->d_red, red_dacc_off(ctx), ctx->d_sub, ctx->ntiles, W, ctx->d_H, ctx->d_g, ctx->d_red + red_r_off(ctx),
-                    ctx->d_scal + slot);
   }
   return BALM_OK;
 }
@@ -455,6 +521,7 @@
   ctx->device = device;
   ctx->flags = flags;
   ctx->timer.on = (flags & BALM_FLAG_TIMING) != 0;
+  ctx->lm_ahead = !(flags & BALM_FLAG_NO_LM_AHEAD);
   auto fail = [&]() -> balm_ctx * { one_destroy(ctx); return nullptr; };
   std::vector<int> jobs, sub;
   {
@@ -540,6 +607,7 @@
   if (ctx->amail.host) hipHostFree((void *)ctx->amail.host);
   if (ctx->amail.scan_state) hipFree(ctx->amail.scan_state);
   for (auto &sp : ctx->timer.pending) { hipEventDestroy(sp.a); hipEventDestroy(sp.b); }
+  for (auto &sp : ctx->timer.ahead) { hipEventDestroy(sp.a); hipEventDestroy(sp.b); }
   for (auto e : ctx->timer.pool) hipEventDestroy(e);
   if (ctx->stream) hipStreamDestroy(ctx->stream);
   delete ctx;
@@ -1262,26 +1330,47 @@
   return BALM_OK;
 }
 
-static int lm_enqueue(balm_ctx *ctx, int form, bool evaluated, bool mail) {
+static bool lm_ahead_eligible(const balm_ctx *ctx, int it, bool fused) {
+  return ctx->lm_ahead && !has_transport(ctx) && !ctx->multi && !fused && ctx->F > 0 && it + 1 < ctx->lm_max_iter &&
+         ctx->gt_dirty_cols == (size_t)3 * ctx->F && !(!ctx->sparse && syrk_int8_for(ctx, 3L * ctx->F));
+}
+
+static int lm_enqueue(balm_ctx *ctx, int form, bool evaluated, bool mail, int it = -1) {
   int rc;
-  if (evaluated && (rc = evaluate_device(ctx, form, ctx->d_poses, 0, ctx->F, 0))) return rc;
+  if (evaluated && !ctx->ahead_done && (rc = evaluate_device(ctx, form, ctx->d_poses, 0, ctx->F, 0))) return rc;
+  ctx->ahead_done = false;
   {
     Span sp(ctx, BALM_T_SOLVE);
     launch_solve(ctx, evaluated, form, ctx->d_poses, ctx->d_poses_tmp);
   }
   ctx->gt_trial_valid = false;
   bool sum_in_mail = false;
-  if (fuse_trial(ctx) && ctx->d_Gt2 && ctx->d_dpart2) {
+  const bool fused = fuse_trial(ctx) && ctx->d_Gt2 && ctx->d_dpart2;
+  const bool ahead = mail && it >= 0 && lm_ahead_eligible(ctx, it, fused);
+  GoRule rule = ctx->lm_rule;
+  rule.on = ahead;
+  if (!ctx->feat_cur_valid) rule.force_hess = 0;
+  bool mailed = false;
+  if (fused) {
     if ((rc = trial_device(ctx, form, ctx->d_poses_tmp, 1))) return rc;
   } else {
     sum_in_mail = mail && !has_transport(ctx) && ctx->F > 0;
     const bool eigen_mails = sum_in_mail && ctx->F <= 256;
-    if ((rc = residual_device(ctx, ctx->d_poses_tmp, 0, ctx->F, 1, sum_in_mail, eigen_mails))) return rc;
-    if (eigen_mails) return BALM_OK;
-  }
-  if (mail) launch_scalars_mail(ctx->stream, ctx->d_scal, ctx->d_hscal, (double)++ctx->mail_seq, sum_in_mail ? ctx->d_rpart_tmp : nullptr,
-                                ctx->nr_tmp, 1);
-  else HIP_TRY(hipMemcpyAsync(ctx->h_scal, ctx->d_scal, 16 * sizeof(double), hipMemcpyDeviceToHost, ctx->stream));
+    if ((rc = residual_device(ctx, ctx->d_poses_tmp, 0, ctx->F, 1, sum_in_mail, eigen_mails, &rule))) return rc;
+    mailed = eigen_mails;
+  }
+  if (!mailed) {
+    if (mail) launch_scalars_mail(ctx->stream, ctx->d_scal, ctx->d_hscal, (double)++ctx->mail_seq, sum_in_mail ? ctx->d_rpart_tmp : nullptr,
+                                  ctx->nr_tmp, 1, rule);
+    else HIP_TRY(hipMemcpyAsync(ctx->h_scal, ctx->d_scal, 16 * sizeof(double), hipMemcpyDeviceToHost, ctx->stream));
+  }
+  ctx->timer.mail_mark = ctx->timer.pending.size();
+  if (ahead) {
+    ctx->ahead_queued = true;
+    const EvalInputs cur{ctx->d_poses, ctx->d_feat, ctx->d_rpart, ctx->nr_cur};
+    if ((rc = enqueue_hessian(ctx, form, ctx->d_poses_tmp, ctx->d_feat_tmp, ctx->d_rpart_tmp, ctx->nr_tmp, 0, ctx->F, 0, true, nullptr, 0,
+                              ctx->d_scal + SCAL_GO, &cur, nullptr))) return rc;
+  }
   return BALM_OK;
 }
 
@@ -1324,7 +1413,7 @@
     }
     ctx->u_on_device = false;
   }
-  int rc = lm_enqueue(ctx, form, evaluated, true);
+  int rc = lm_enqueue(ctx, form, evaluated, true, disabled ? it : -1);
   if (rc) return rc;
   return wait_scalars(ctx);
 }
@@ -1368,6 +1457,11 @@
   double u = o->u0, v = 2, r1 = 0, r2 = 0;
   bool calc = true;
   int it = 0;
+  ctx->lm_rule.rel_tol = o->rel_tol; ctx->lm_rule.abs_tol = o->abs_tol; ctx->lm_rule.no_stop = o->no_stop ? 1 : 0;
+  ctx->lm_rule.force_hess = o->force_hess ? 1 : 0;
+  ctx->lm_max_iter = o->max_iter;
+  ctx->ahead_queued = ctx->ahead_done = false;
+  ahead_settle(ctx, false);
   int fault_rank = -1, fault_it = -1, timeout_it = -1;
   if (const char *fi = getenv("BALM_FAULT_INJECT")) {
     if (!strncmp(fi, "timeout,", 8)) timeout_it = atoi(fi + 8);
@@ -1379,6 +1473,9 @@
     if (it == timeout_it) { ctx->inject_solve_timeout = true; timeout_it = -1; }
     if ((rc = set_damping(ctx, u))) return rc;
     if ((rc = lm_iteration(ctx, o->form, evaluated, it))) return rc;
+    const double go = ctx->ahead_queued ? ctx->h_scal[SCAL_GO] : 0.0;
+    const bool ahead_ran = go == 1.0 || go == 2.0;
+    ctx->ahead_queued = false;
     double sc[3] = {ctx->h_scal[0], ctx->h_scal[1], ctx->h_scal[2]};
     if ((rc = multi_share_scalars(ctx, it, sc, 3))) return rc;
     r1 = sc[0]; r2 = sc[1];
@@ -1387,11 +1484,13 @@
     if (!ctx->multi && !ctx->persistent_off && !(std::isfinite(r2) && std::isfinite(q1)) && std::isfinite(r1) && solve_timed_out(ctx)) {
       ctx->persistent_off = true;
       drop_lm_graphs(ctx);
+      ahead_settle(ctx, false);
       ctx->feat_cur_valid = false; ctx->gt_cur_valid = false;
       calc = true;
       continue;
     }
     if (!(std::isfinite(r1) && std::isfinite(r2))) {
+      ahead_settle(ctx, false);
       ctx->err = "balm_damping_iter: non-finite residual";
       return BALM_ERR_NUMERIC;
     }
@@ -1402,6 +1501,10 @@
       printf("iter%d: (%lf %lf) u: %lf v: %.1lf q: %.3lf %lf %lf\n", it, r1, r2, u, v, q / q1, q1, q);
       fflush(stdout);
     }
+    const bool stops = !o->no_stop && (std::fabs(r1 - r2) / r1 < o->rel_tol || (o->abs_tol > 0 && std::fabs(r1 - r2) < o->abs_tol));
+    const bool goes_on = !stops && it + 1 < o->max_iter;
+    const bool ahead_taken = goes_on && (q > 0 ? go == 1.0 : (go == 2.0 && o->force_hess));
+    ahead_settle(ctx, ahead_ran);
     if (q > 0) {
       double *t = ctx->d_poses; ctx->d_poses = ctx->d_poses_tmp; ctx->d_poses_tmp = t;
       t = ctx->d_feat; ctx->d_feat = ctx->d_feat_tmp; ctx->d_feat_tmp = t;
@@ -1422,13 +1525,14 @@
       u *= (q < 1.0 / 3.0 ? 1.0 / 3.0 : q);
       calc = true;
     } else {
-      u = u * v; v = 2 * v; calc = false;
-    }
+      u = u * v; v = 2 * v; calc = go == 1.0;
+    }
+    if (ahead_taken) { ctx->ahead_done = true; ctx->rowmax_cur_valid = false; }
     it++;
     if (!o->no_stop && std::fabs(r1 - r2) / r1 < o->rel_tol) break;
     if (!o->no_stop && o->abs_tol > 0 && std::fabs(r1 - r2) < o->abs_tol) break;
   }
-  ctx->feat_cur_valid = false; ctx->gt_cur_valid = false;
+  ctx->feat_cur_valid = false; ctx->gt_cur_valid = false; ctx->ahead_done = false;
   if (o->reanchor) launch_reanchor(s, W, ctx->d_poses);
   HIP_TRY(hipMemcpyAsync(poses, ctx->d_poses, (size_t)12 * W * sizeof(double), hipMemcpyDeviceToHost, s));
   if ((rc = sync_stream(ctx))) return rc;
diff --git a/balm_amd/csrc/balm_internal.h b/balm_amd/csrc/balm_internal.h
--- a/balm_amd/csrc/balm_internal.h
+++ b/balm_amd/csrc/balm_internal.h
@@ -34,6 +34,9 @@
   bool on = false;
   struct Span { hipEvent_t a, b; int slot; };
   std::vector<Span> pending;
+  size_t mail_mark = 0;
+  size_t ready = 0;
+  std::vector<Span> ahead;
   std::vector<hipEvent_t> pool;
   double ms[BALM_T_COUNT] = {0};
   long cnt[BALM_T_COUNT] = {0};
@@ -48,6 +51,10 @@
   unsigned long long *scan_state = nullptr; unsigned int scan_gen = 0;
 };
 constexpr long SCAN_TILES_CAP = 8192;
+}
+
+namespace balm {
+struct GoRule { double rel_tol = 0, abs_tol = 0; int no_stop = 0, force_hess = 0, on = 0; };
 }
 
 struct balm_ctx {
@@ -116,6 +123,11 @@
   double *h_scal = nullptr;
   double *d_hscal = nullptr;
   unsigned long long mail_seq = 0;
+  bool lm_ahead = true;
+  balm::GoRule lm_rule;
+  int lm_max_iter = 0;
+  bool ahead_queued = false;
+  bool ahead_done = false;
   bool need_minv = false;
   bool solve_tiled = false;
   int chain_refused_P[2] = {-1, -1};
@@ -171,28 +183,29 @@
 hipError_t preload_voxel();
 void launch_transpose_clusters(hipStream_t s, const double *aos, double *soa, int F, int W);
 void launch_world_moments(hipStream_t s, const double *cl, const double *poses, int W, int f0, int f1, double *C);
-struct EigenMail { double *scal; double *host; double stamp; int slot; };
+struct EigenMail { double *scal; double *host; double stamp; int slot; GoRule rule; };
 int launch_feature_eigen(hipStream_t s, const double *C, const double *fix, const double *coe, int f0, int f1,
                          double *feat, double *rpart, const EigenMail *mail = nullptr);
 int factors_grid(int W, int nfeat, int form);
 int factors_chunk(int W);
 bool launch_factors(hipStream_t s, int form, const double *cl, const double *poses, const double *feat, int W,
                     int npad, int f0, int f1, double *Gt, double *dpart, int nblk, const int *slot = nullptr,
-                    unsigned long long *rowmax = nullptr, double *rowmax_part = nullptr);
+                    unsigned long long *rowmax = nullptr, double *rowmax_part = nullptr, const double *go = nullptr,
+                    const double *poses_alt = nullptr, const double *feat_alt = nullptr);
 int launch_moments_factors(hipStream_t s, int form, const double *cl, const double *poses, const double *fix, const double *coe, int W,
                            int npad, int F, double *Gt, double *dpart, int nblk, const int *slot, double *feat, double *rpart,
                            unsigned long long *rowmax = nullptr, double *rowmax_part = nullptr);
 struct SyrkPlan { int SG; int nsteps; int Kpad; long nblocks; };
 SyrkPlan plan_syrk(int ntiles, long K);
 void launch_syrk(hipStream_t s, const double *Gt, int npad, int ntiles, const int *tileIJ, const SyrkPlan &p,
-                 double *part);
+                 double *part, const double *go = nullptr);
 void launch_syrk_sparse(hipStream_t s, const double *Gt, int npad, const int *jobs, const int *items, const int *chunk_ids,
-                        int nsteps, long nitems, double *part);
+                        int nsteps, long nitems, double *part, const double *go = nullptr);
 void launch_reduce(hipStream_t s, const double *part, int SG, long tile_elems_total, const double *dpart, int nblk,
                    int dacc_len, const double *rpart, int nr, double *red, long red_dacc_off, long red_r_off,
-                   const int *csr_ptr = nullptr);
+                   const int *csr_ptr = nullptr, const double *go = nullptr, const double *rpart_alt = nullptr, int nr_alt = 0);
 void launch_assemble(hipStream_t s, int form, const double *red, long red_dacc_off, const int *tileIJ, int ntiles,
-                     int W, double *H, double *g, const double *r_in = nullptr, double *r_out = nullptr);
+                     int W, double *H, double *g, const double *r_in = nullptr, double *r_out = nullptr, const double *go = nullptr);
 void launch_sum_scalar(hipStream_t s, const double *rpart, int nr, double *out);
 struct I8Layout { int T, rows_p, NT, M; long Kp; size_t off_digits, off_rowmax, off_scale, off_part; };
 size_t syrk_i8_scratch_bytes(int n, long K, I8Layout *lay);
@@ -246,6 +259,15 @@
 int multi_host_barrier_rc(balm_ctx *ctx, int rc);
 
 constexpr int SCAL_U = 5;
+constexpr int SCAL_GO = 6;
+__host__ __device__ inline double lm_go(const GoRule &g, double r1, double r2, double q1) {
+  if (!g.on || !(r1 - r1 == 0.0 && r2 - r2 == 0.0 && q1 - q1 == 0.0)) return 0.0;
+  const double taken = r1 - r2 > 0 ? 1.0 : (g.force_hess ? 2.0 : 0.0);
+  if (g.no_stop) return taken;
+  if (fabs(r1 - r2) / r1 < g.rel_tol) return 0.0;
+  if (g.abs_tol > 0 && fabs(r1 - r2) < g.abs_tol) return 0.0;
+  return taken;
+}
 constexpr int SCAL_STAMP = 16 + 64;
 bool chain_macro_plan(int P, int NH, std::vector<int> &tab);
 void context_born(int device);
@@ -255,7 +277,7 @@
 void launch_solve(balm_ctx *c, bool new_hessian, int upd_form = 0, const double *upd_poses = nullptr, double *upd_out = nullptr);
 void launch_update_poses(hipStream_t s, int form, int W, const double *poses, const double *dx, double *out);
 void launch_scalars_mail(hipStream_t s, double *d_scal, double *d_hscal, double stamp, const double *rpart = nullptr, int nr = 0,
-                         int slot = 0);
+                         int slot = 0, const GoRule &rule = GoRule());
 void launch_reanchor(hipStream_t s, int W, double *poses);
 
 struct AssocOpts {
diff --git a/balm_amd/csrc/kernels_accum.hip b/balm_amd/csrc/kernels_accum.hip
--- a/balm_amd/csrc/kernels_accum.hip
+++ b/balm_amd/csrc/kernels_accum.hip
@@ -229,7 +229,12 @@
   if (threadIdx.x == 0) mail.scal[mail.slot] = sred[0];
   __syncthreads();
   volatile double *host = mail.host;
-  if (threadIdx.x < 16) host[threadIdx.x] = ((int)threadIdx.x == mail.slot) ? sred[0] : mail.scal[threadIdx.x];
+  if (threadIdx.x < 16) {
+    auto val = [&](int i) { return i == mail.slot ? sred[0] : mail.scal[i]; };
+    double v = val((int)threadIdx.x);
+    if (threadIdx.x == SCAL_GO) mail.scal[SCAL_GO] = v = lm_go(mail.rule, val(0), val(1), val(2));
+    host[threadIdx.x] = v;
+  }
   __threadfence_system();
   __syncthreads();
   if (threadIdx.x == 0) { host[SCAL_STAMP] = mail.stamp; __threadfence_system(); }
@@ -240,7 +245,7 @@
   int nf = f1 - f0;
   if (nf <= 0) return 0;
   int grid = (nf + 255) / 256;
-  const EigenMail none{nullptr, nullptr, 0.0, 0};
+  const EigenMail none{nullptr, nullptr, 0.0, 0, GoRule()};
   hipLaunchKernelGGL(k_feature_eigen, dim3(grid), dim3(256), 0, s, C, fix, coe, f0, f1, feat, rpart, (mail && grid == 1) ? *mail : none);
   return grid;
 }
@@ -494,8 +499,16 @@
                                                          const double *__restrict__ feat, int W, int Wc, int npad, int f0,
                                                          int f1, double *__restrict__ Gt,
                                                          double *__restrict__ dpart, const int *__restrict__ slot, int staged,
-                                                         double *__restrict__ rowmax_part = nullptr) {
+                                                         double *__restrict__ rowmax_part = nullptr,
+                                                         const double *__restrict__ go = nullptr,
+                                                         const double *__restrict__ poses_alt = nullptr,
+                                                         const double *__restrict__ feat_alt = nullptr) {
   static_assert(!MAXR || REGS, "the row maxima live in the lane that owns the pose");
+  if (go) {
+    const double g = *go;
+    if (g == 0.0) return;
+    if (g == 2.0) { poses = poses_alt; feat = feat_alt; }
+  }
   double rm[6] = {0.0, 0.0, 0.0, 0.0, 0.0, 0.0}, bad = 0.0;
   constexpr int DACC = FORM == 0 ? DACC_LEFT : DACC_RIGHT;
   extern __shared__ __attribute__((aligned(16))) double sm[];
@@ -813,7 +826,8 @@
 }
 
 bool launch_factors(hipStream_t s, int form, const double *cl, const double *poses, const double *feat, int W,
-                    int npad, int f0, int f1, double *Gt, double *dpart, int nblk, const int *slot, unsigned long long *rowmax, double *rowmax_part) {
+                    int npad, int f0, int f1, double *Gt, double *dpart, int nblk, const int *slot, unsigned long long *rowmax, double *rowmax_part,
+                    const double *go, const double *poses_alt, const double *feat_alt) {
   const int Wc = factors_chunk(W), chunks = (W + Wc - 1) / Wc;
   size_t lds = factors_lds(W, form);
   int bs = W <= 64 ? 64 : (W <= 128 ? 128 : 256);
@@ -826,7 +840,7 @@
     hipLaunchKernelGGL(k_rowmax_reduce, dim3((npad + 63) / 64), dim3(1024), 0, s, rowmax_part, nblk, W, npad, rowmax);
     return true;
   }
-#define BALM_FACTORS(F, R) hipLaunchKernelGGL((k_feature_factors<F, R, false>), dim3(nblk, chunks), dim3(bs), lds, s, cl, poses, feat, W, Wc, npad, f0, f1, Gt, dpart, slot, staged, nullptr)
+#define BALM_FACTORS(F, R) hipLaunchKernelGGL((k_feature_factors<F, R, false>), dim3(nblk, chunks), dim3(bs), lds, s, cl, poses, feat, W, Wc, npad, f0, f1, Gt, dpart, slot, staged, nullptr, go, poses_alt, feat_alt)
   if (form == 0) { if (regs) BALM_FACTORS(0, true); else BALM_FACTORS(0, false); }
   else BALM_FACTORS(1, false);
 #undef BALM_FACTORS
@@ -919,7 +933,8 @@
 
 __global__ __launch_bounds__(64) void k_hessian_syrk(const double *__restrict__ Gt, int npad, int njobs,
                                                      const int *__restrict__ jobs, int nsteps, long nblocks,
-                                                     double *__restrict__ part) {
+                                                     double *__restrict__ part, const double *__restrict__ go) {
+  if (go && *go == 0.0) return;
   const long bid = xcd_remap(blockIdx.x, nblocks);
   const int tile = (int)(bid % njobs);
   const int sg = (int)(bid / njobs);
@@ -931,7 +946,8 @@
 __global__ __launch_bounds__(64) void k_hessian_syrk_sparse(const double *__restrict__ Gt, int npad,
                                                             const int *__restrict__ jobs, const int *__restrict__ items,
                                                             const int *__restrict__ chunk_ids, int nsteps, long nitems,
-                                                            double *__restrict__ part) {
+                                                            double *__restrict__ part, const double *__restrict__ go) {
+  if (go && *go == 0.0) return;
   const long bid = xcd_remap(blockIdx.x, nitems);
   const int tile = items[4 * bid], first = items[4 * bid + 1], count = items[4 * bid + 2], slot = items[4 * bid + 3];
   const int type = jobs[4 * tile], I = jobs[4 * tile + 1], J = jobs[4 * tile + 2];
@@ -983,15 +999,15 @@
 }
 
 void launch_syrk_sparse(hipStream_t s, const double *Gt, int npad, const int *jobs, const int *items, const int *chunk_ids,
-                        int nsteps, long nitems, double *part) {
+                        int nsteps, long nitems, double *part, const double *go) {
   hipLaunchKernelGGL(k_hessian_syrk_sparse, dim3((unsigned)nitems), dim3(64), 0, s, Gt, npad, jobs, items, chunk_ids, nsteps,
-                     nitems, part);
+                     nitems, part, go);
 }
 
 void launch_syrk(hipStream_t s, const double *Gt, int npad, int ntiles, const int *tileIJ, const SyrkPlan &p,
-                 double *part) {
+                 double *part, const double *go) {
   hipLaunchKernelGGL(k_hessian_syrk, dim3((unsigned)p.nblocks), dim3(64), 0, s, Gt, npad, ntiles, tileIJ,
-                     p.nsteps, p.nblocks, part);
+                     p.nsteps, p.nblocks, part, go);
 }
 
 template <class Sink>
@@ -1098,7 +1114,13 @@
 
 __global__ __launch_bounds__(256) void k_reduce_all(const double *__restrict__ part, int SG, const int *__restrict__ csr_ptr, long tile_total,
                                                     int tile_blocks, const double *__restrict__ dpart, int nblk, int dacc_len, int dacc_cap,
-                                                    const double *__restrict__ rpart, int nr, double *__restrict__ red, long dacc_off, long r_off, int quads) {
+                                                    const double *__restrict__ rpart, int nr, double *__restrict__ red, long dacc_off, long r_off, int quads,
+                                                    const double *__restrict__ go, const double *__restrict__ rpart_alt, int nr_alt) {
+  if (go) {
+    const double g = *go;
+    if (g == 0.0) return;
+    if (g == 2.0) { rpart = rpart_alt; nr = nr_alt; }
+  }
   if ((int)blockIdx.x < tile_blocks) {
     auto to_payload = [&](long t, double v) { red[t] = v; };
     if (csr_ptr) reduce_tiles_csr(part, csr_ptr, tile_total, to_payload, blockIdx.x, tile_blocks);
@@ -1110,14 +1132,15 @@
 }
 
 void launch_reduce(hipStream_t s, const double *part, int SG, long tile_total, const double *dpart, int nblk,
-                   int dacc_len, const double *rpart, int nr, double *red, long dacc_off, long r_off, const int *csr_ptr) {
+                   int dacc_len, const double *rpart, int nr, double *red, long dacc_off, long r_off, const int *csr_ptr, const double *go,
+                   const double *rpart_alt, int nr_alt) {
   const int dacc_cap = (int)(r_off - dacc_off);
   static const bool no_quads = getenv("BALM_REDUCE_QUADS") && getenv("BALM_REDUCE_QUADS")[0] == '0';
   const int quads = !csr_ptr && !no_quads && tile_total <= 32768 && SG >= 8;
   int grid = (int)(((quads ? 4 : 1) * tile_total + 255) / 256);
   if (grid > 8192) grid = 8192;
   hipLaunchKernelGGL(k_reduce_all, dim3(grid + (dacc_cap + 63) / 64), dim3(256), 0, s, part, SG, csr_ptr, tile_total, grid, dpart, nblk, dacc_len,
-                     dacc_cap, rpart, nr, red, dacc_off, r_off, quads);
+                     dacc_cap, rpart, nr, red, dacc_off, r_off, quads, go, rpart_alt, nr_alt);
 }
 
 __device__ __forceinline__ int sym3(int r, int c) {
@@ -1145,7 +1168,8 @@
 __global__ __launch_bounds__(256) void k_assemble(const double *__restrict__ red, long dacc_off,
                                                   const int *__restrict__ tileIJ, int ntiles, int W,
                                                   double *__restrict__ H, double *__restrict__ g, const double *__restrict__ r_in,
-                                                  double *__restrict__ r_out) {
+                                                  double *__restrict__ r_out, const double *__restrict__ go) {
+  if (go && *go == 0.0) return;
   const int n = 6 * W;
   if (r_out && blockIdx.x == 0 && threadIdx.x == 0) *r_out = *r_in;
   const long total = (long)ntiles * TILE_ELEMS;
@@ -1180,15 +1204,15 @@
 }
 
 void launch_assemble(hipStream_t s, int form, const double *red, long dacc_off, const int *tileIJ, int ntiles, int W,
-                     double *H, double *g, const double *r_in, double *r_out) {
+                     double *H, double *g, const double *r_in, double *r_out, const double *go) {
   long total = (long)ntiles * TILE_ELEMS;
   int grid = (int)((total + 255) / 256);
   if (grid > 4096) grid = 4096;
   if (form == 0)
-    hipLaunchKernelGGL(k_assemble<0>, dim3(grid), dim3(256), 0, s, red, dacc_off, tileIJ, ntiles, W, H, g, r_in, r_out);
+    hipLaunchKernelGGL(k_assemble<0>, dim3(grid), dim3(256), 0, s, red, dacc_off, tileIJ, ntiles, W, H, g, r_in, r_out, go);
   else
-    hipLaunchKernelGGL(k_assemble<1>, dim3(grid), dim3(256), 0, s, red, dacc_off, tileIJ, ntiles, W, H, g, r_in, r_out);
-}
-
-
-}
+    hipLaunchKernelGGL(k_assemble<1>, dim3(grid), dim3(256), 0, s, red, dacc_off, tileIJ, ntiles, W, H, g, r_in, r_out, go);
+}
+
+
+}
diff --git a/balm_amd/csrc/kernels_solve.hip b/balm_amd/csrc/kernels_solve.hip
--- a/balm_amd/csrc/kernels_solve.hip
+++ b/balm_amd/csrc/kernels_solve.hip
@@ -883,7 +883,7 @@
 }
 
 __global__ __launch_bounds__(256) void k_scalars_mail(double *__restrict__ scal, volatile double *__restrict__ host, double stamp,
-                                                      const double *__restrict__ rpart, int nr, int slot) {
+                                                      const double *__restrict__ rpart, int nr, int slot, GoRule rule) {
   __shared__ double sred[256];
   if (rpart) {
     double s = 0.0;
@@ -897,14 +897,19 @@
     if (threadIdx.x == 0) scal[slot] = sred[0];
     __syncthreads();
   }
-  if (threadIdx.x < 16) host[threadIdx.x] = (rpart && (int)threadIdx.x == slot) ? sred[0] : scal[threadIdx.x];
+  if (threadIdx.x < 16) {
+    auto val = [&](int i) { return (rpart && i == slot) ? sred[0] : scal[i]; };
+    double v = val((int)threadIdx.x);
+    if (threadIdx.x == SCAL_GO) scal[SCAL_GO] = v = lm_go(rule, val(0), val(1), val(2));
+    host[threadIdx.x] = v;
+  }
   __threadfence_system();
   __syncthreads();
   if (threadIdx.x == 0) { host[SCAL_STAMP] = stamp; __threadfence_system(); }
 }
 
-void launch_scalars_mail(hipStream_t s, double *d_scal, double *d_hscal, double stamp, const double *rpart, int nr, int slot) {
-  hipLaunchKernelGGL(k_scalars_mail, dim3(1), dim3(256), 0, s, d_scal, d_hscal, stamp, rpart, nr, slot);
+void launch_scalars_mail(hipStream_t s, double *d_scal, double *d_hscal, double stamp, const double *rpart, int nr, int slot, const GoRule &rule) {
+  hipLaunchKernelGGL(k_scalars_mail, dim3(1), dim3(256), 0, s, d_scal, d_hscal, stamp, rpart, nr, slot, rule);
 }
 
 hipError_t preload_solve() {
diff --git a/include/balm_hip.h b/include/balm_hip.h
--- a/include/balm_hip.h
+++ b/include/balm_hip.h
@@ -23,7 +23,8 @@
 enum {
   BALM_FLAG_TIMING = 1,
   BALM_FLAG_LOOPBACK_SHARDS = 2,
-  BALM_FLAG_SYRK_INT8 = 4
+  BALM_FLAG_SYRK_INT8 = 4,
+  BALM_FLAG_NO_LM_AHEAD = 8
 };
 
 typedef struct balm_iter_log {
```
